# Nightmare-n/GD-MAE

Measured on AMD Instinct MI355X. Metric: MAE pre-train frames/sec (Waymo-shape, 180k pts, 75% mask), higher is better.
Workload: dtype bf16

## Files before the change

gd-mae_amd/csrc/conv_tiles.hip:

```cpp
#include "conv_tiles.h"

typedef float f32x16 __attribute__((ext_vector_type(16)));
typedef __bf16 bf16x8 __attribute__((ext_vector_type(8)));
typedef _Float16 f16x8 __attribute__((ext_vector_type(8)));
union CtFrag {
  uint4 q;
  bf16x8 v;
  f16x8 h;
};

#define CT_C 128
#define CT_SITE_PITCH 272
#ifndef CT_CH
#define CT_CH 128
#endif
#ifndef CT_RING
#define CT_RING 8
#endif
#define CT_HALVES (CT_C / CT_CH)
#define CT_KS (CT_CH / 16)
#define CT_NSTEP (9 * CT_KS)
#define CT_CPS (CT_CH / 8)
#define CT_PSITE (CT_CH * 2 + 16)
#define CT_ROW_PITCH (CT_CH == 128 ? 2944 : 1664)
#define CT_TILE_PITCH (10 * CT_ROW_PITCH)
#ifndef CT_TPW
#define CT_TPW 2
#endif
#define CT_THREADS (CT_TPW * 128)
#define CT_NWAVES (CT_TPW * 2)
#define CT_STAGE_PITCH 17408
#define CT_RED_OFF (CT_TPW * CT_STAGE_PITCH)
#define CT_EPI_BYTES (CT_RED_OFF + CT_TPW * CT_NWAVES * 2 * CT_C * 4)
#define CT_PATCH_BYTES (CT_TPW * CT_TILE_PITCH)
#define CT_LDS_BYTES (CT_PATCH_BYTES > CT_EPI_BYTES ? CT_PATCH_BYTES : CT_EPI_BYTES)
#define CT_SPP (CT_THREADS / CT_CPS)
#define CT_NPASS ((100 * CT_TPW + CT_SPP - 1) / CT_SPP)
#define CT_ESPP (CT_THREADS / 16)
#define CT_MAX_SRC 3
#define CT_NRED 256

__device__ inline float ct_bf2f(unsigned short h) { return __uint_as_float(((unsigned)h) << 16); }
__device__ inline unsigned short ct_f2bf(float f) { return gd_to_bf16(f); }
__device__ inline unsigned ct_pack2(float lo, float hi) { return gd_pack_bf16(lo, hi); }
__device__ inline float ct_f16r(float f) {
  const unsigned p = gd_pack_f16(f, 0.f);
  return (float)__builtin_bit_cast(_Float16, (unsigned short)(p & 0xFFFFu));
}
__device__ inline void ct_unpack8(const uint4& u, float (&f)[8]) {
  const unsigned w[4] = {u.x, u.y, u.z, u.w};
#pragma unroll
  for (int k = 0; k < 4; ++k) {
    f[2 * k] = __uint_as_float(w[k] << 16);
    f[2 * k + 1] = __uint_as_float(w[k] & 0xFFFF0000u);
  }
}

struct CtMaps {
  const int* map[CT_MAX_SRC];
  int ls[CT_MAX_SRC];
  int k;
};

__global__ __launch_bounds__(256) void k_ct_tile_flags(CtMaps Mp, int B, int H, int W, int TH, int TW, int* __restrict__ flag) {
  const int lane = threadIdx.x & 63;
  const int t = blockIdx.x * 4 + (threadIdx.x >> 6);
  if (t >= B * TH * TW) return;
  const int tx = t % TW, r = t / TW, ty = r % TH, b = r / TH;
  bool act = false;
  for (int e = lane; e < 100; e += 64) {
    const int y = ty * 8 - 1 + e / 10, x = tx * 8 - 1 + e % 10;
    if (y < 0 || y >= H || x < 0 || x >= W) continue;
    for (int g = 0; g < Mp.k; ++g) {
      const int ls = Mp.ls[g];
      act |= Mp.map[g][(b * (H >> ls) + (y >> ls)) * (W >> ls) + (x >> ls)] >= 0;
    }
  }
  const unsigned long long m = __ballot(act);
  if (lane == 0) flag[t] = m != 0ull;
}

struct CtFlagLoad {
  const int* flag;
  __device__ int operator()(long long i) const { return flag[i]; }
};
struct CtSlotStore {
  int* slot;
  int* list;
  __device__ void operator()(long long i, int ex, int v) const {
    slot[i] = v ? ex : -1;
    if (v) list[ex] = (int)i;
  }
};

extern "C" size_t gdmae_decoder_tiles_workspace_bytes(int B, int H, int W) {
  const long long nt = (long long)B * ((H + 7) / 8) * ((W + 7) / 8);
  return gd_align(sizeof(int) * nt) + gd_align(sizeof(int) * (gd_scan_ws_elems(nt) + 2)) + 256;
}

extern "C" int gdmae_decoder_tiles(const int* const* maps, const int* strides, int k, int B, int H, int W, int* tile_slot,
                                   int* tile_list, int* n_act, void* workspace, void* stream) {
  GD_REQUIRE(k >= 1 && k <= CT_MAX_SRC, "decoder_tiles: 1..3 source stages");
  GD_REQUIRE(H >= 2 && W >= 2 && B >= 1, "decoder_tiles: map too small");
  hipStream_t st = (hipStream_t)stream;
  CtMaps Mp;
  Mp.k = k;
  for (int g = 0; g < k; ++g) {
    const int s = strides[g];
    GD_REQUIRE(s == 1 || s == 2 || s == 4 || s == 8, "decoder_tiles: stride must be 1, 2, 4 or 8");
    GD_REQUIRE(H % s == 0 && W % s == 0, "decoder_tiles: stride must divide the map");
    Mp.map[g] = maps[g];
    Mp.ls[g] = s == 1 ? 0 : (s == 2 ? 1 : (s == 4 ? 2 : 3));
  }
  const int TH = (H + 7) / 8, TW = (W + 7) / 8;
  const long long nt = (long long)B * TH * TW;
  GdArena A(workspace, gdmae_decoder_tiles_workspace_bytes(B, H, W));
  int* flag = A.take<int>(nt);
  int* scan_ws = A.take<int>(gd_scan_ws_elems(nt) + 2);
  hipLaunchKernelGGL(k_ct_tile_flags, dim3(gd_div_up(nt, 4)), dim3(256), 0, st, Mp, B, H, W, TH, TW, flag);
  GD_LAUNCH_CHECK();
  return gd_device_scan<int>(nt, CtFlagLoad{flag}, CtSlotStore{tile_slot, tile_list}, n_act, scan_ws, st);
}

size_t gd_decoder_tiles_lb_state_bytes(long long nt) { return gd_scan_lb_state_bytes<int>(nt); }
int gd_decoder_tiles_lb(const int* const* maps, const int* strides, int k, int B, int H, int W, int* tile_slot, int* tile_list, int* n_act,
                        int* flag, void* lb_state, hipStream_t st) {
  GD_REQUIRE(k >= 1 && k <= CT_MAX_SRC, "decoder_tiles: 1..3 source stages");
  CtMaps Mp;
  Mp.k = k;
  for (int g = 0; g < k; ++g) {
    const int s = strides[g];
    GD_REQUIRE((s == 1 || s == 2 || s == 4 || s == 8) && H % s == 0 && W % s == 0, "decoder_tiles: stride must be 1, 2, 4 or 8 and divide the map");
    Mp.map[g] = maps[g];
    Mp.ls[g] = s == 1 ? 0 : (s == 2 ? 1 : (s == 4 ? 2 : 3));
  }
  const int TH = (H + 7) / 8, TW = (W + 7) / 8;
  const long long nt = (long long)B * TH * TW;
  hipLaunchKernelGGL(k_ct_tile_flags, dim3(gd_div_up(nt, 4)), dim3(256), 0, st, Mp, B, H, W, TH, TW, flag);
  GD_LAUNCH_CHECK();
  return gd_device_scan_lb<int>(nt, CtFlagLoad{flag}, CtSlotStore{tile_slot, tile_list}, GdNoTotal{}, n_act, lb_state, st);
}

__global__ __launch_bounds__(256) void k_ct_pack_weights(const float* __restrict__ w, int Cin, int nsteps, uint4* __restrict__ Wp) {
  const int i = blockIdx.x * blockDim.x + threadIdx.x;
  if (i >= nsteps * 4 * 64) return;
  const int lane = i & 63, wv = (i >> 6) & 3, st = i >> 8;
  const int ks = st & 7, tap = (st >> 3) % 9, g = (st >> 3) / 9;
  const int o = 32 * wv + (lane & 31);
  const int ci = g * CT_C + ks * 16 + (lane >> 5) * 8;
  float f[8];
#pragma unroll
  for (int j = 0; j < 8; ++j) f[j] = w[((long long)o * Cin + ci + j) * 9 + tap];
  uint4 q;
  q.x = gd_pack_f16(f[0], f[1]);
  q.y = gd_pack_f16(f[2], f[3]);
  q.z = gd_pack_f16(f[4], f[5]);
  q.w = gd_pack_f16(f[6], f[7]);
  Wp[i] = q;
}

struct CtBPtrs {
  const float* b[CT_MAX_SRC];
};

__global__ __launch_bounds__(256) void k_ct_class_consts(const float* __restrict__ w, CtBPtrs Bp, int Cin, int C2,
                                                         unsigned short* __restrict__ bgz, unsigned short* __restrict__ ybg) {
  __shared__ double sh[9][256];
  const int o = blockIdx.x;
  double t[9];
#pragma unroll
  for (int k = 0; k < 9; ++k) t[k] = 0.0;
  for (int c = threadIdx.x; c < Cin; c += 256) {
    const float bv = Bp.b[c / CT_C][c % CT_C];
    if (o == 0) bgz[c] = ct_f2bf(bv > 0.f ? bv : 0.f);
    const double bg = (double)ct_f16r(bv > 0.f ? bv : 0.f);
#pragma unroll
    for (int k = 0; k < 9; ++k) t[k] += (double)ct_f16r(w[((long long)o * Cin + c) * 9 + k]) * bg;
  }
#pragma unroll
  for (int k = 0; k < 9; ++k) sh[k][threadIdx.x] = t[k];
  __syncthreads();
  if (threadIdx.x < 9) {
    double s = 0.0;
    for (int i = 0; i < 256; ++i) s += sh[threadIdx.x][i];
    sh[threadIdx.x][0] = s;
  }
  __syncthreads();
  if (threadIdx.x < 9) {
    const int cy = threadIdx.x / 3, cx = threadIdx.x % 3;
    double s = 0.0;
    for (int ky = 0; ky < 3; ++ky) {
      if ((cy == 0 && ky == 0) || (cy == 2 && ky == 2)) continue;
      for (int kx = 0; kx < 3; ++kx) {
        if ((cx == 0 && kx == 0) || (cx == 2 && kx == 2)) continue;
        s += sh[ky * 3 + kx][0];
      }
    }
    ybg[threadIdx.x * C2 + o] = ct_f2bf((float)s);
  }
}

extern "C" size_t gdmae_conv3x3_tiles_packed_bytes(int k) { return (size_t)k * 72 * 4 * 64 * 16; }

extern "C" int gdmae_conv3x3_tiles_pack(const float* conv_w, int C2, int Cin, const float* const* b, int k, void* Wp, void* bgz,
                                        void* ybg, void* stream) {
  GD_REQUIRE(C2 == CT_C && k >= 1 && k <= CT_MAX_SRC && Cin == CT_C * k, "conv3x3_tiles: 128 output channels, 128 per source");
  hipStream_t st = (hipStream_t)stream;
  const int nsteps = k * 72;
  hipLaunchKernelGGL(k_ct_pack_weights, dim3(nsteps), dim3(256), 0, st, conv_w, Cin, nsteps, (uint4*)Wp);
  GD_LAUNCH_CHECK();
  CtBPtrs Bp;
  for (int g = 0; g < CT_MAX_SRC; ++g) Bp.b[g] = g < k ? b[g] : nullptr;
  hipLaunchKernelGGL(k_ct_class_consts, dim3(C2), dim3(256), 0, st, conv_w, Bp, Cin, C2, (unsigned short*)bgz, (unsigned short*)ybg);
  GD_LAUNCH_CHECK();
  return 0;
}

struct CtSrc {
  const unsigned short* P;
  const int* map;
  const float* a;
  const float* b;
  int ls;
};
struct CtArgs {
  CtSrc src[CT_MAX_SRC];
  int k;
  const uint4* Wp;
  const int* tile_list;
  int n_act, H, W, TH, TW;
  unsigned short* Yc;
  float* part;
};

#define CT_MFMA(a, b, c) __builtin_amdgcn_mfma_f32_32x32x16_f16((a), (b), (c), 0, 0, 0)

#define CT_OFF(st) ((((st) / CT_KS) / 3) * CT_ROW_PITCH + (((st) / CT_KS) % 3) * CT_PSITE + ((st) % CT_KS) * 32)
#define CT_WSTEP(st, hf) ((((st) / CT_KS) * 8 + (hf) * CT_KS + ((st) % CT_KS)) * 256)

__global__ __launch_bounds__(CT_THREADS, CT_TPW == 2 ? (CT_CH == 64 ? 3 : 2) : 1) void k_conv3x3_tiles(CtArgs A) {
  extern __shared__ __align__(16) unsigned char lds[];
  const int tid = threadIdx.x, lane = tid & 63, wvg = tid >> 6;
  const int wv = wvg & 3;
  const int tg = wvg >> 2;
  const int slot0 = blockIdx.x * CT_TPW;
  int tb[CT_TPW], ty0[CT_TPW], tx0[CT_TPW];
  bool have[CT_TPW];
#pragma unroll
  for (int t = 0; t < CT_TPW; ++t) {
    have[t] = slot0 + t < A.n_act;
    const int tile = have[t] ? A.tile_list[slot0 + t] : 0;
    tx0[t] = (tile % A.TW) * 8;
    const int r = tile / A.TW;
    ty0[t] = (r % A.TH) * 8;
    tb[t] = r / A.TH;
  }
  const int lc = tid % CT_CPS;
  const int lsg = tid / CT_CPS;
  const unsigned char* lb = lds + tg * 2 * CT_TILE_PITCH + ((lane & 31) >> 3) * CT_ROW_PITCH + (lane & 7) * CT_PSITE + (lane >> 5) * 16;
  f32x16 acc0, acc1, acc2, acc3;
#pragma unroll
  for (int i = 0; i < 16; ++i) acc0[i] = acc1[i] = acc2[i] = acc3[i] = 0.f;

  for (int g = 0; g < A.k; ++g) {
    const CtSrc S = A.src[g];
    const int ls = S.ls, sm = (1 << ls) - 1;
    const int Hs = A.H >> ls, Ws = A.W >> ls;
    int code[CT_NPASS];
    {
      int tokv[CT_NPASS];
#pragma unroll
      for (int p = 0; p < CT_NPASS; ++p) {
        const int e = p * CT_SPP + lsg;
        const int t = e / 100 < CT_TPW ? e / 100 : CT_TPW - 1;
        const int r = e - 100 * (e / 100);
        const int py = r / 10, px = r - py * 10;
        const int y = ty0[t] + py - 1, x = tx0[t] + px - 1;
        const bool inb = e < 100 * CT_TPW && have[t] && y >= 0 && y < A.H && x >= 0 && x < A.W;
        tokv[p] = S.map[inb ? (tb[t] * Hs + (y >> ls)) * Ws + (x >> ls) : 0];
      }
#pragma unroll
      for (int p = 0; p < CT_NPASS; ++p) {
        const int e = p * CT_SPP + lsg;
        int c = -3;
        if (e < 100 * CT_TPW) {
          const int t = e / 100;
          const int r = e - 100 * t;
          const int py = r / 10, px = r - py * 10;
          if (have[t]) {
            const int y = ty0[t] + py - 1, x = tx0[t] + px - 1;
            c = -2;
            if (y >= 0 && y < A.H && x >= 0 && x < A.W) {
              const int tok = tokv[p];
              c = tok < 0 ? -1 : (((tok << ls) + (y & sm)) << ls) + (x & sm);
            }
          }
        }
        code[p] = c;
      }
    }
    const unsigned short* __restrict__ Prows = S.P ? S.P : (const unsigned short*)S.a;
#pragma unroll 1
    for (int hf = 0; hf < CT_HALVES; ++hf) {
      {
        const int c0 = hf * CT_CH + lc * 8;
        float av[8], bv[8];
        {
          const float4 a0 = *(const float4*)(S.a + c0), a1 = *(const float4*)(S.a + c0 + 4);
          const float4 b0 = *(const float4*)(S.b + c0), b1 = *(const float4*)(S.b + c0 + 4);
          av[0] = a0.x; av[1] = a0.y; av[2] = a0.z; av[3] = a0.w; av[4] = a1.x; av[5] = a1.y; av[6] = a1.z; av[7] = a1.w;
          bv[0] = b0.x; bv[1] = b0.y; bv[2] = b0.z; bv[3] = b0.w; bv[4] = b1.x; bv[5] = b1.y; bv[6] = b1.z; bv[7] = b1.w;
        }
        uint4 bgq;
        {
          float r[8];
#pragma unroll
          for (int j = 0; j < 8; ++j) r[j] = bv[j];
          bgq.x = gd_pack_f16_relu(r[0], r[1]); bgq.y = gd_pack_f16_relu(r[2], r[3]); bgq.z = gd_pack_f16_relu(r[4], r[5]); bgq.w = gd_pack_f16_relu(r[6], r[7]);
        }
        uint4 q[CT_NPASS];
#pragma unroll
        for (int p = 0; p < CT_NPASS; ++p) q[p] = *(const uint4*)(Prows + (long long)(code[p] >= 0 ? code[p] : 0) * CT_C + c0);
#pragma unroll
        for (int p = 0; p < CT_NPASS; ++p) {
          if (code[p] == -3) continue;
          const int e = p * CT_SPP + lsg;
          const int t = e / 100;
          const int r = e - 100 * t;
          const int py = r / 10, px = r - py * 10;
          uint4 o;
          if (code[p] >= 0) {
            float f[8];
            ct_unpack8(q[p], f);
#pragma unroll
            for (int j = 0; j < 8; ++j) f[j] = fmaf(av[j], f[j], bv[j]);
            o.x = gd_pack_f16_relu(f[0], f[1]); o.y = gd_pack_f16_relu(f[2], f[3]); o.z = gd_pack_f16_relu(f[4], f[5]); o.w = gd_pack_f16_relu(f[6], f[7]);
          } else if (code[p] == -1) {
            o = bgq;
          } else {
            o = make_uint4(0u, 0u, 0u, 0u);
          }
          *(uint4*)(lds + t * CT_TILE_PITCH + py * CT_ROW_PITCH + px * CT_PSITE + lc * 16) = o;
        }
      }
      __syncthreads();
      {
        const uint4* __restrict__ wp = A.Wp + ((size_t)g * 72 * 4 + wv) * 64 + lane + (size_t)hf * CT_KS * 256;
        CtFrag wr[CT_RING + 1], sf[2][4];
#pragma unroll
        for (int st = 0; st < CT_RING; ++st) wr[st].q = wp[CT_WSTEP(st, 0)];
        sf[0][0].q = *(const uint4*)(lb);
        sf[0][1].q = *(const uint4*)(lb + 4 * CT_ROW_PITCH);
        sf[0][2].q = *(const uint4*)(lb + CT_TILE_PITCH);
        sf[0][3].q = *(const uint4*)(lb + CT_TILE_PITCH + 4 * CT_ROW_PITCH);
#pragma unroll
        for (int st = 0; st < CT_NSTEP; ++st) {
          if (st + CT_RING < CT_NSTEP) wr[(st + CT_RING) % (CT_RING + 1)].q = wp[CT_WSTEP(st + CT_RING, 0)];
          if (st + 1 < CT_NSTEP) {
            sf[(st + 1) & 1][0].q = *(const uint4*)(lb + CT_OFF(st + 1));
            sf[(st + 1) & 1][1].q = *(const uint4*)(lb + 4 * CT_ROW_PITCH + CT_OFF(st + 1));
            sf[(st + 1) & 1][2].q = *(const uint4*)(lb + CT_TILE_PITCH + CT_OFF(st + 1));
            sf[(st + 1) & 1][3].q = *(const uint4*)(lb + CT_TILE_PITCH + 4 * CT_ROW_PITCH + CT_OFF(st + 1));
          }
          acc0 = CT_MFMA(wr[st % (CT_RING + 1)].h, sf[st & 1][0].h, acc0);
          acc1 = CT_MFMA(wr[st % (CT_RING + 1)].h, sf[st & 1][1].h, acc1);
          acc2 = CT_MFMA(wr[st % (CT_RING + 1)].h, sf[st & 1][2].h, acc2);
          acc3 = CT_MFMA(wr[st % (CT_RING + 1)].h, sf[st & 1][3].h, acc3);
          __builtin_amdgcn_sched_barrier(0);
        }
      }
      __syncthreads();
    }
  }

  {
    const int n = lane & 31;
    const int cb = wv * 32 + 4 * (lane >> 5);
#define CT_STAGE(acc, sb)                                                                                              \
  _Pragma("unroll") for (int j = 0; j < 4; ++j) {                                                                      \
    uint2 o;                                                                                                           \
    o.x = ct_pack2(acc[4 * j], acc[4 * j + 1]);                                                                        \
    o.y = ct_pack2(acc[4 * j + 2], acc[4 * j + 3]);                                                                    \
    *(uint2*)(lds + (tg * 2 + ((sb) >> 1)) * CT_STAGE_PITCH + (((sb) & 1) * 32 + n) * CT_SITE_PITCH + (cb + 8 * j) * 2) = o; \
  }
    CT_STAGE(acc0, 0)
    CT_STAGE(acc1, 1)
    CT_STAGE(acc2, 2)
    CT_STAGE(acc3, 3)
#undef CT_STAGE
  }
  __syncthreads();
  float* red = (float*)(lds + CT_RED_OFF);
  const int elc = tid & 15, elsg = tid >> 4;
#pragma unroll
  for (int t = 0; t < CT_TPW; ++t) {
    if (!have[t]) continue;
    float s[8], q2[8];
#pragma unroll
    for (int j = 0; j < 8; ++j) s[j] = q2[j] = 0.f;
#pragma unroll
    for (int p = 0; p < 64 / CT_ESPP; ++p) {
      const int site = p * CT_ESPP + elsg;
      const uint4 v = *(const uint4*)(lds + t * CT_STAGE_PITCH + site * CT_SITE_PITCH + elc * 16);
      *(uint4*)(A.Yc + ((long long)(slot0 + t) * GD_TILE_SITES + site) * CT_C + elc * 8) = v;
      if (ty0[t] + (site >> 3) < A.H && tx0[t] + (site & 7) < A.W) {
        float f[8];
        ct_unpack8(v, f);
#pragma unroll
        for (int j = 0; j < 8; ++j) {
          s[j] += f[j];
          q2[j] = fmaf(f[j], f[j], q2[j]);
        }
      }
    }
#pragma unroll
    for (int j = 0; j < 8; ++j) {
      s[j] += __shfl_xor(s[j], 16, 64);
      s[j] += __shfl_xor(s[j], 32, 64);
      q2[j] += __shfl_xor(q2[j], 16, 64);
      q2[j] += __shfl_xor(q2[j], 32, 64);
    }
    if (lane < 16) {
#pragma unroll
      for (int j = 0; j < 8; ++j) {
        red[((t * CT_NWAVES + wvg) * 2 + 0) * CT_C + elc * 8 + j] = s[j];
        red[((t * CT_NWAVES + wvg) * 2 + 1) * CT_C + elc * 8 + j] = q2[j];
      }
    }
  }
  __syncthreads();
#pragma unroll
  for (int t = 0; t < CT_TPW; ++t) {
    if (!have[t] || tid >= 256) continue;
    const int stat = tid >> 7, ch = tid & 127;
    float v = 0.f;
#pragma unroll
    for (int w = 0; w < CT_NWAVES; ++w) v += red[((t * CT_NWAVES + w) * 2 + stat) * CT_C + ch];
    A.part[(long long)(slot0 + t) * 256 + tid] = v;
  }
}

__global__ __launch_bounds__(256) void k_ct_stats_reduce(const float* __restrict__ part, int n_act, const int* __restrict__ tile_list,
                                                         const unsigned short* __restrict__ ybg, int B, int H, int W, int TH, int TW,
                                                         float* __restrict__ red) {
  const int tid = threadIdx.x;
  if ((int)blockIdx.x < CT_NRED) {
    const int chunk = (n_act + CT_NRED - 1) / CT_NRED;
    const int r0 = blockIdx.x * chunk, r1 = r0 + chunk < n_act ? r0 + chunk : n_act;
    float a0 = 0.f, a1 = 0.f, a2 = 0.f, a3 = 0.f;
    int r = r0;
    for (; r + 15 < r1; r += 16) {
      float v[16];
#pragma unroll
      for (int u = 0; u < 16; ++u) v[u] = part[(long long)(r + u) * 256 + tid];
#pragma unroll
      for (int u = 0; u < 16; u += 4) {
        a0 += v[u];
        a1 += v[u + 1];
        a2 += v[u + 2];
        a3 += v[u + 3];
      }
    }
    for (; r + 3 < r1; r += 4) {
      a0 += part[(long long)r * 256 + tid];
      a1 += part[(long long)(r + 1) * 256 + tid];
      a2 += part[(long long)(r + 2) * 256 + tid];
      a3 += part[(long long)(r + 3) * 256 + tid];
    }
    for (; r < r1; ++r) a0 += part[(long long)r * 256 + tid];
    red[(long long)blockIdx.x * 256 + tid] = (a0 + a1) + (a2 + a3);
    return;
  }
  __shared__ int cnt[9];
  if (tid < 9) cnt[tid] = 0;
  __syncthreads();
  int c[9];
#pragma unroll
  for (int k = 0; k < 9; ++k) c[k] = 0;
  for (int i0 = tid; i0 < n_act; i0 += 8 * 256) {
   int tl[8];
#pragma unroll
   for (int u = 0; u < 8; ++u) tl[u] = tile_list[i0 + u * 256 < n_act ? i0 + u * 256 : n_act - 1];
#pragma unroll
   for (int u = 0; u < 8; ++u) {
    if (i0 + u * 256 >= n_act) continue;
    const int tile = tl[u];
    const int tx = tile % TW, ty = (tile / TW) % TH;
    const int y0 = ty * 8, y1 = y0 + 8 < H ? y0 + 8 : H, x0 = tx * 8, x1 = x0 + 8 < W ? x0 + 8 : W;
    const int ry[3] = {y0 == 0 ? 1 : 0, 0, y1 == H ? 1 : 0};
    const int rx[3] = {x0 == 0 ? 1 : 0, 0, x1 == W ? 1 : 0};
    const int my = (y1 - y0) - ry[0] - ry[2], mx = (x1 - x0) - rx[0] - rx[2];
#pragma unroll
    for (int cy = 0; cy < 3; ++cy)
#pragma unroll
      for (int cx = 0; cx < 3; ++cx) c[cy * 3 + cx] += (cy == 1 ? my : ry[cy]) * (cx == 1 ? mx : rx[cx]);
   }
  }
#pragma unroll
  for (int k = 0; k < 9; ++k)
    if (c[k]) atomicAdd(&cnt[k], c[k]);
  __syncthreads();
  const int stat = tid >> 7, ch = tid & 127;
  double acc = 0.0;
#pragma unroll
  for (int cy = 0; cy < 3; ++cy)
#pragma unroll
    for (int cx = 0; cx < 3; ++cx) {
      const long long total = (long long)B * (cy == 1 ? H - 2 : 1) * (cx == 1 ? W - 2 : 1);
      const double n = (double)(total - cnt[cy * 3 + cx]);
      const double v = (double)ct_bf2f(ybg[(cy * 3 + cx) * CT_C + ch]);
      acc += n * (stat ? v * v : v);
    }
  const float hi = (float)acc;
  red[(long long)CT_NRED * 256 + tid] = hi;
  red[(long long)(CT_NRED + 1) * 256 + tid] = (float)(acc - (double)hi);
}

int gd_bn_fold_from_partials(hipStream_t st, const float* part, int nblk, int C, double count, const float* gamma,
                             const float* beta, double eps, double momentum, float* running_mean, float* running_var,
                             long long* num_batches, double* stats, float* ab, float* mv);

extern "C" size_t gdmae_conv3x3_tiles_workspace_bytes(int n_act) {
  return gd_align((size_t)(n_act > 0 ? n_act : 1) * 256 * sizeof(float)) + gd_align((size_t)(CT_NRED + 2) * 256 * sizeof(float));
}

extern "C" int gdmae_conv3x3_tiles_fwd(const void* const* P, const int* const* maps, const float* const* a, const float* const* b,
                                       const int* strides, int k, const void* Wp, const void* ybg, const int* tile_list, int n_act,
                                       int B, int H, int W, void* Yc, const float* gamma, const float* beta, double eps,
                                       double momentum, float* running_mean, float* running_var, long long* num_batches,
                                       double* stats, float* ab, float* mv, void* workspace, void* stream) {
  GD_REQUIRE(k >= 1 && k <= CT_MAX_SRC, "conv3x3_tiles: 1..3 source stages");
  GD_REQUIRE(H >= 2 && W >= 2, "conv3x3_tiles: map too small");
  hipStream_t st = (hipStream_t)stream;
  CtArgs A;
  A.k = k;
  for (int g = 0; g < CT_MAX_SRC; ++g) {
    if (g < k) {
      const int s = strides[g];
      GD_REQUIRE((s == 1 || s == 2 || s == 4 || s == 8) && H % s == 0 && W % s == 0, "conv3x3_tiles: stride");
      A.src[g].P = (const unsigned short*)P[g];
      A.src[g].map = maps[g];
      A.src[g].a = a[g];
      A.src[g].b = b[g];
      A.src[g].ls = s == 1 ? 0 : (s == 2 ? 1 : (s == 4 ? 2 : 3));
    } else {
      A.src[g].P = nullptr; A.src[g].map = nullptr; A.src[g].a = nullptr; A.src[g].b = nullptr; A.src[g].ls = 0;
    }
  }
  A.Wp = (const uint4*)Wp;
  A.tile_list = tile_list;
  A.n_act = n_act;
  A.H = H; A.W = W; A.TH = (H + 7) / 8; A.TW = (W + 7) / 8;
  A.Yc = (unsigned short*)Yc;
  GdArena ar(workspace, gdmae_conv3x3_tiles_workspace_bytes(n_act));
  float* part = ar.take<float>((size_t)(n_act > 0 ? n_act : 1) * 256);
  float* red = ar.take<float>((size_t)(CT_NRED + 2) * 256);
  A.part = part;
  if (n_act > 0) {
    static bool once = false;
    if (!once) {
      GD_CHECK(hipFuncSetAttribute((const void*)k_conv3x3_tiles, hipFuncAttributeMaxDynamicSharedMemorySize, CT_LDS_BYTES));
      once = true;
    }
    hipLaunchKernelGGL(k_conv3x3_tiles, dim3((n_act + CT_TPW - 1) / CT_TPW), dim3(CT_THREADS), CT_LDS_BYTES, st, A);
    GD_LAUNCH_CHECK();
  }
  hipLaunchKernelGGL(k_ct_stats_reduce, dim3(CT_NRED + 1), dim3(256), 0, st, (const float*)part, n_act, tile_list,
                     (const unsigned short*)ybg, B, H, W, A.TH, A.TW, red);
  GD_LAUNCH_CHECK();
  return gd_bn_fold_from_partials(st, red, CT_NRED + 2, CT_C, (double)B * H * W, gamma, beta, eps, momentum, running_mean,
                                  running_var, num_batches, stats, ab, mv);
}

template <int ES>
__global__ __launch_bounds__(256) void k_tiles_gather_rows(const void* __restrict__ Yc, GdTiles T, const int* __restrict__ cell,
                                                           long long n, int H, int W, int C, uint4* __restrict__ out) {
  const int cv = C * ES / 16;
  const long long total = n * cv;
  for (long long i = blockIdx.x * (long long)blockDim.x + threadIdx.x; i < total; i += (long long)gridDim.x * blockDim.x) {
    const long long r = total < (1ll << 31) ? (long long)((unsigned)i / (unsigned)cv) : i / cv;
    const int v = (int)(i - r * cv);
    const int s = cell[r];
    const int x = s % W, q = s / W, y = q % H, b = q / H;
    out[i] = ((const uint4*)gd_y_row<ES>(Yc, T, b, y, x, H, W, C))[v];
  }
}

extern "C" int gdmae_tiles_gather_rows(const void* Yc, const int* tile_slot, const void* ybg, const int* cell, long long n, int H,
                                       int W, int C, int elem_bytes, void* out, void* stream) {
  GD_REQUIRE(tile_slot != nullptr && (elem_bytes == 2 || elem_bytes == 4) && (C * elem_bytes) % 16 == 0, "tiles_gather_rows");
  if (n <= 0) return 0;
  GdTiles T{tile_slot, ybg, (H + 7) / 8, (W + 7) / 8};
  long long g = (n * (C * elem_bytes / 16) + 255) / 256;
  if (g > 16384) g = 16384;
  if (elem_bytes == 2) hipLaunchKernelGGL(k_tiles_gather_rows<2>, dim3((int)g), dim3(256), 0, (hipStream_t)stream, Yc, T, cell, n, H, W, C, (uint4*)out);
  else hipLaunchKernelGGL(k_tiles_gather_rows<4>, dim3((int)g), dim3(256), 0, (hipStream_t)stream, Yc, T, cell, n, H, W, C, (uint4*)out);
  GD_LAUNCH_CHECK();
  return 0;
}

__global__ __launch_bounds__(256) void k_tiles_gather_rows_affine_relu(const void* __restrict__ Yc, GdTiles T, const int* __restrict__ cell,
                                                                       long long n, int H, int W, int C, const float* __restrict__ a,
                                                                       const float* __restrict__ b, uint4* __restrict__ yrows,
                                                                       float4* __restrict__ out) {
  const int cv = C / 8;
  const long long total = n * cv;
  for (long long i = blockIdx.x * (long long)blockDim.x + threadIdx.x; i < total; i += (long long)gridDim.x * blockDim.x) {
    const long long r = total < (1ll << 31) ? (long long)((unsigned)i / (unsigned)cv) : i / cv;
    const int v = (int)(i - r * cv);
    const int s = cell[r];
    const int x = s % W, q = s / W, y = q % H, bb = q / H;
    const uint4 yq = ((const uint4*)gd_y_row<2>(Yc, T, bb, y, x, H, W, C))[v];
    const float4 a0 = ((const float4*)a)[2 * v], a1 = ((const float4*)a)[2 * v + 1];
    const float4 b0 = ((const float4*)b)[2 * v], b1 = ((const float4*)b)[2 * v + 1];
    const unsigned w4[4] = {yq.x, yq.y, yq.z, yq.w};
    const float av[8] = {a0.x, a0.y, a0.z, a0.w, a1.x, a1.y, a1.z, a1.w};
    const float bv[8] = {b0.x, b0.y, b0.z, b0.w, b1.x, b1.y, b1.z, b1.w};
    float o[8];
#pragma unroll
    for (int j = 0; j < 4; ++j) {
      const float h0 = fmaf(av[2 * j], __uint_as_float(w4[j] << 16), bv[2 * j]);
      const float h1 = fmaf(av[2 * j + 1], __uint_as_float(w4[j] & 0xFFFF0000u), bv[2 * j + 1]);
      o[2 * j] = h0 > 0.f ? h0 : 0.f;
      o[2 * j + 1] = h1 > 0.f ? h1 : 0.f;
    }
    yrows[i] = yq;
    out[2 * i] = make_float4(o[0], o[1], o[2], o[3]);
    out[2 * i + 1] = make_float4(o[4], o[5], o[6], o[7]);
  }
}

extern "C" int gdmae_tiles_gather_rows_affine_relu(const void* Yc, const int* tile_slot, const void* ybg, const int* cell, long long n,
                                                   int H, int W, int C, const float* a, const float* b, void* yrows, float* out,
                                                   void* stream) {
  GD_REQUIRE(tile_slot != nullptr && C % 8 == 0 && a != nullptr && b != nullptr, "tiles_gather_rows_affine_relu: bf16 rows, C % 8 == 0");
  if (n <= 0) return 0;
  GdTiles T{tile_slot, ybg, (H + 7) / 8, (W + 7) / 8};
  long long g = (n * (C / 8) + 255) / 256;
  if (g > 16384) g = 16384;
  hipLaunchKernelGGL(k_tiles_gather_rows_affine_relu, dim3((int)g), dim3(256), 0, (hipStream_t)stream, Yc, T, cell, n, H, W, C, a, b,
                     (uint4*)yrows, (float4*)out);
  GD_LAUNCH_CHECK();
  return 0;
}

template <int ES>
__global__ __launch_bounds__(256) void k_tiles_to_dense(const void* __restrict__ Yc, GdTiles T, int B, int H, int W, int C,
                                                        uint4* __restrict__ out) {
  const int cv = C * ES / 16;
  const long long total = (long long)B * H * W * cv;
  for (long long i = blockIdx.x * (long long)blockDim.x + threadIdx.x; i < total; i += (long long)gridDim.x * blockDim.x) {
    const long long s = i / cv;
    const int v = (int)(i % cv);
    const int x = (int)(s % W);
    const long long q = s / W;
    const int y = (int)(q % H), b = (int)(q / H);
    out[i] = ((const uint4*)gd_y_row<ES>(Yc, T, b, y, x, H, W, C))[v];
  }
}

__global__ __launch_bounds__(256) void k_tiles_to_dense_affine_relu(const void* __restrict__ Yc, GdTiles T, int B, int H, int W, int C,
                                                                    const float* __restrict__ a, const float* __restrict__ bsh,
                                                                    float* __restrict__ out) {
  const int cv = C / 8;
  const long long total = (long long)B * H * W * cv;
  const unsigned total32 = (unsigned)total, ucv = (unsigned)cv, uW = (unsigned)W, uH = (unsigned)H;
  for (unsigned i = blockIdx.x * blockDim.x + threadIdx.x; i < total32; i += gridDim.x * blockDim.x) {
    const unsigned s32 = i / ucv;
    const int v = (int)(i - s32 * ucv);
    const unsigned q32 = s32 / uW;
    const int x = (int)(s32 - q32 * uW);
    const unsigned b32 = q32 / uH;
    const int y = (int)(q32 - b32 * uH), b = (int)b32;
    const long long s = s32;
    const uint4 u = ((const uint4*)gd_y_row<2>(Yc, T, b, y, x, H, W, C))[v];
    float f[8];
    ct_unpack8(u, f);
    const float4 a0 = *(const float4*)(a + 8 * v), a1 = *(const float4*)(a + 8 * v + 4);
    const float4 b0 = *(const float4*)(bsh + 8 * v), b1 = *(const float4*)(bsh + 8 * v + 4);
    float4 o0, o1;
    o0.x = fmaxf(fmaf(a0.x, f[0], b0.x), 0.f); o0.y = fmaxf(fmaf(a0.y, f[1], b0.y), 0.f);
    o0.z = fmaxf(fmaf(a0.z, f[2], b0.z), 0.f); o0.w = fmaxf(fmaf(a0.w, f[3], b0.w), 0.f);
    o1.x = fmaxf(fmaf(a1.x, f[4], b1.x), 0.f); o1.y = fmaxf(fmaf(a1.y, f[5], b1.y), 0.f);
    o1.z = fmaxf(fmaf(a1.z, f[6], b1.z), 0.f); o1.w = fmaxf(fmaf(a1.w, f[7], b1.w), 0.f);
    typedef float f4v __attribute__((ext_vector_type(4)));
    __builtin_nontemporal_store(f4v{o0.x, o0.y, o0.z, o0.w}, (f4v*)(out + s * C + 8 * v));
    __builtin_nontemporal_store(f4v{o1.x, o1.y, o1.z, o1.w}, (f4v*)(out + s * C + 8 * v + 4));
  }
}

extern "C" int gdmae_tiles_to_dense_affine_relu(const void* Yc, const int* tile_slot, const void* ybg, int B, int H, int W, int C, const float* a,
                                                const float* b, float* out, void* stream) {
  GD_REQUIRE(tile_slot != nullptr && C % 8 == 0 && a != nullptr && b != nullptr, "tiles_to_dense_affine_relu");
  GD_REQUIRE((long long)B * H * W * (C / 8) < (1ll << 31), "tiles_to_dense_affine_relu: B H W C / 8 must fit 31 bits");
  GdTiles T{tile_slot, ybg, (H + 7) / 8, (W + 7) / 8};
  hipLaunchKernelGGL(k_tiles_to_dense_affine_relu, dim3(16384), dim3(256), 0, (hipStream_t)stream, Yc, T, B, H, W, C, a, b, out);
  GD_LAUNCH_CHECK();
  return 0;
}

extern "C" int gdmae_tiles_to_dense(const void* Yc, const int* tile_slot, const void* ybg, int B, int H, int W, int C, int elem_bytes,
                                    void* out, void* stream) {
  GD_REQUIRE(tile_slot != nullptr && (elem_bytes == 2 || elem_bytes == 4) && (C * elem_bytes) % 16 == 0, "tiles_to_dense");
  GdTiles T{tile_slot, ybg, (H + 7) / 8, (W + 7) / 8};
  if (elem_bytes == 2) hipLaunchKernelGGL(k_tiles_to_dense<2>, dim3(16384), dim3(256), 0, (hipStream_t)stream, Yc, T, B, H, W, C, (uint4*)out);
  else hipLaunchKernelGGL(k_tiles_to_dense<4>, dim3(16384), dim3(256), 0, (hipStream_t)stream, Yc, T, B, H, W, C, (uint4*)out);
  GD_LAUNCH_CHECK();
  return 0;
}
```

gd-mae_amd/csrc/plan.hip:

```cpp
#include "../../include/gdmae_hip.h"
#include "common.h"
#include <string.h>

int gd_voxelize_impl(const float* points, long long n_points, int n_cols, const float* lo, const float* vs, const int* grid_xyz,
                     int batch_size, float* points_out, long long* point_coords, long long* inverse, int* inverse32,
                     long long* voxel_coords, int* pillar_cell, int* pillar_pt_off, int* pillar_pts, int* point_rank,
                     int* sample_pillar_off, float* pillar_mean, int* cell2pillar_out, int* counts, void* workspace, size_t workspace_bytes,
                     void* lb_state, float* points_pm, int* row_pillar, hipStream_t st);
size_t gd_voxelize_lb_state_bytes(long long n_points, long long cells);
size_t gd_plan_scan_state_bytes(long long n);
size_t gd_plan_win_state_bytes(long long n);
int gd_plan_visible_tokens(const float* mask, const int* cell2pillar, long long n_cells, int* tok_pillar, int* tok_cell, int* map,
                           int* n_tok, void* lb_state, hipStream_t st);
int gd_plan_downsample(const int* map_in, int B, int Yi, int Xi, int* tok_cell_out, int* map_out, int* n_out, void* lb_state,
                       hipStream_t st);
struct Dims {
  int B, Y, X;
};
struct PlanJob {
  const int* n_tok;
  const int* tok_cell;
  Dims dt, dm;
  const int* map;
  int mode, s;
  int* nbr;
  int* nbr_rev;
};
constexpr int kPlanMaxJobs = 16;
struct PlanJobs {
  PlanJob j[kPlanMaxJobs];
  int count;
};
int gd_plan_jobs(const PlanJobs& J, long long cap_max, hipStream_t st);
size_t gd_plan_windows_ws_bytes(int B, int Y, int X, int wx, int wy);
long long gd_plan_n_windows(int B, int Y, int X, int wx, int wy);
struct GdWinStage {
  const int* map;
  int B, Y, X, wx, wy, nlev;
  const int *drop_lo, *drop_hi, *max_tokens;
  int* out[2][7];
  int* counts[2];
  void* workspace;
  void* lb_state;
};
int gd_plan_windows_all(const GdWinStage* stages, int n_stages, hipStream_t st);
size_t gd_decoder_tiles_lb_state_bytes(long long nt);
int gd_decoder_tiles_lb(const int* const* maps, const int* strides, int k, int B, int H, int W, int* tile_slot, int* tile_list, int* n_act,
                        int* flag, void* lb_state, hipStream_t st);
int gd_decoder_site_rulebook(const int* site, const int* n_dev, int sites_per_tok, long long cap_sites, const int* tile_slot, int H, int W,
                             int* nbr, hipStream_t st);

namespace {

struct StageGeo {
  int Y, X;
  long long cap;
  long long cap_in;
  int up_s;
  long long n_win;
};

struct Layout {
  gdmae_plan_buffer* table;
  int max_entries, n;
  size_t off;
  bool ok;
  long long add(const char* name, size_t bytes) {
    const size_t o = off;
    if (table) {
      if (n >= max_entries) {
        ok = false;
        return -1;
      }
      strncpy(table[n].name, name, sizeof(table[n].name) - 1);
      table[n].name[sizeof(table[n].name) - 1] = 0;
      table[n].offset = (long long)o;
      table[n].bytes = (long long)bytes;
    }
    ++n;
    off += gd_align(bytes);
    return (long long)o;
  }
};

struct Offsets {
  long long lb_state, counts, points, point_coords, inverse, inverse32, voxel_coords, pillar_cell, pt_off, pillar_pts, point_rank,
      sample_off, pillar_mean, cell2pillar, points_pm, row_pillar, vox_ws, mask, len_keep, tok_pillar;
  long long vis_tok_cell, vis_map;
  long long vfe_row_tok, vfe_vis_rows, vfe_vis_tok, vfe_tok_row_off;
  struct {
    long long tok_cell, map, nbr_subm, nbr_subm_t, nbr_down, nbr_down_t, up_sites, win_ws;
    long long w[2][7];
  } s[GDMAE_PLAN_MAX_STAGES];
  long long dec_slot, dec_list, dec_flag, dec_nbr[3];
  size_t lb_bytes, vox_ws_bytes;
  int n_counts;
  bool dec;
  StageGeo geo[GDMAE_PLAN_MAX_STAGES];
  long long cap_pts, m_cap, cells;
};

constexpr int kTokScanThreads = 1024, kTokScanItems = 4;
__global__ __launch_bounds__(kTokScanThreads) void k_vfe_tok_row_off(const int* __restrict__ n_tok_p, const int* __restrict__ tok_pillar,
                                                                     const int* __restrict__ pt_off, int* __restrict__ tok_row_off,
                                                                     int* __restrict__ n_rows) {
  __shared__ int s_wave[kTokScanThreads / 64];
  const int n = *n_tok_p, lane = threadIdx.x & 63, wave = threadIdx.x >> 6;
  int base = 0;
  for (int t0 = 0; t0 < n; t0 += kTokScanThreads * kTokScanItems) {
    const int t = t0 + (int)threadIdx.x * kTokScanItems;
    int c[kTokScanItems], sum = 0;
#pragma unroll
    for (int k = 0; k < kTokScanItems; ++k) {
      c[k] = 0;
      if (t + k < n) {
        const int p = tok_pillar[t + k];
        c[k] = pt_off[p + 1] - pt_off[p];
      }
      sum += c[k];
    }
    int incl = sum;
#pragma unroll
    for (int d = 1; d < 64; d <<= 1) {
      const int o = __shfl_up(incl, d, 64);
      if (lane >= d) incl += o;
    }
    if (lane == 63) s_wave[wave] = incl;
    __syncthreads();
    int before = 0, all = 0;
#pragma unroll
    for (int w = 0; w < kTokScanThreads / 64; ++w) {
      before += w < wave ? s_wave[w] : 0;
      all += s_wave[w];
    }
    int run = base + before + incl - sum;
#pragma unroll
    for (int k = 0; k < kTokScanItems; ++k) {
      if (t + k < n) tok_row_off[t + k] = run;
      run += c[k];
    }
    base += all;
    __syncthreads();
  }
  if (threadIdx.x == 0) {
    tok_row_off[n] = base;
    *n_rows = base;
  }
}
__global__ __launch_bounds__(256) void k_vfe_vis_rows(const int* __restrict__ counts, const int* __restrict__ row_pillar,
                                                      const int* __restrict__ pillar_cell, const int* __restrict__ map,
                                                      const int* __restrict__ pt_off, const int* __restrict__ tok_row_off,
                                                      int* __restrict__ row_tok, int* __restrict__ vis_rows, int* __restrict__ vis_tok) {
  const int N = counts[0];
  for (int r = blockIdx.x * 256 + threadIdx.x; r < N; r += gridDim.x * 256) {
    const int p = row_pillar[r];
    const int t = map[pillar_cell[p]];
    row_tok[r] = t;
    if (t >= 0) {
      const int rc = tok_row_off[t] + (r - pt_off[p]);
      vis_rows[rc] = r;
      vis_tok[rc] = t;
    }
  }
}

int check(const gdmae_plan_params* p) {
  GD_REQUIRE(p != nullptr, "geometry plan: null parameters");
  GD_REQUIRE(p->n_points >= 0 && p->n_points < (1ll << 31) && p->n_cols >= 4 && p->n_cols <= 65 && p->batch_size >= 1,
             "geometry plan: bad point buffer");
  GD_REQUIRE(p->grid[0] >= 1 && p->grid[1] >= 1 && p->grid[2] == 1, "geometry plan: single-layer pillar grids (spt_backbone_mae.py:94)");
  GD_REQUIRE(p->n_stages >= 1 && p->n_stages <= GDMAE_PLAN_MAX_STAGES, "geometry plan: 1..4 stages");
  for (int i = 0; i < p->n_stages; ++i) {
    GD_REQUIRE(p->stride[i] == 1 || p->stride[i] == 2, "geometry plan: conv_down stride 1 or 2 (k3 s2 p1)");
    GD_REQUIRE(i == 0 || p->stride[i] == 2, "geometry plan: only the first stage may keep the resolution");
    GD_REQUIRE(p->win_x[i] >= 1 && p->win_y[i] >= 1 && p->win_x[i] * p->win_y[i] <= 64, "geometry plan: window must fit one wavefront");
    GD_REQUIRE(p->n_levels[i] >= 1 && p->n_levels[i] <= 3, "geometry plan: 1..3 drop levels");
  }
  GD_REQUIRE(p->n_dec >= 0 && p->n_dec <= 3, "geometry plan: at most 3 decoder source stages");
  for (int g = 0; g < p->n_dec; ++g) GD_REQUIRE(p->dec_sources[g] >= 0 && p->dec_sources[g] < p->n_stages, "geometry plan: decoder source");
  return 0;
}

int layout(const gdmae_plan_params* p, gdmae_plan_buffer* table, int max_entries, Offsets& O, size_t* total, int* n_entries) {
  if (int rc = check(p)) return rc;
  Layout L{table, max_entries, 0, 0, true};
  const int B = p->batch_size, gx = p->grid[0], gy = p->grid[1], F = p->n_cols - 1;
  const long long n0 = p->cap_points > p->n_points ? p->cap_points : p->n_points;
  O.cells = (long long)B * gx * gy;
  GD_REQUIRE(O.cells < (1ll << 31), "geometry plan: B*Y*X must fit int32");
  O.cap_pts = n0 > 0 ? n0 : 1;
  O.m_cap = n0 < O.cells ? n0 : O.cells;
  if (O.m_cap < 1) O.m_cap = 1;
  const long long cap = O.cap_pts;
  int Y = gy, X = gx;
  long long c = O.m_cap;
  for (int i = 0; i < p->n_stages; ++i) {
    StageGeo& g = O.geo[i];
    g.cap_in = c;
    if (p->stride[i] == 2) {
      Y = (Y - 1) / 2 + 1;
      X = (X - 1) / 2 + 1;
      c = 4 * c < (long long)B * Y * X ? 4 * c : (long long)B * Y * X;
    }
    g.Y = Y; g.X = X; g.cap = c;
    const int us = gy / Y;
    g.up_s = (us >= 1 && us * Y == gy && us * X == gx) ? us : 0;
    g.n_win = gd_plan_n_windows(B, Y, X, p->win_x[i], p->win_y[i]);
    GD_REQUIRE(g.n_win < (1 << 21), "geometry plan: window grid too large for the packed scan");
    GD_REQUIRE(g.cap < (1 << 21), "geometry plan: stage token capacity must stay below 2^21 (21-bit fields of the packed window scan)");
  }
  O.dec = p->n_dec > 0;
  for (int g = 0; g < p->n_dec; ++g) {
    const int us = O.geo[p->dec_sources[g]].up_s;
    O.dec = O.dec && (us == 1 || us == 2 || us == 4 || us == 8);
  }
  const long long nt = (long long)B * ((gy + 7) / 8) * ((gx + 7) / 8);
  size_t lb = gd_voxelize_lb_state_bytes(n0, O.cells) + gd_plan_scan_state_bytes(O.cells);
  for (int i = 0; i < p->n_stages; ++i) {
    if (p->stride[i] == 2) lb += gd_plan_scan_state_bytes((long long)B * O.geo[i].Y * O.geo[i].X);
    lb += 2 * gd_plan_win_state_bytes(O.geo[i].n_win);
  }
  if (O.dec) lb += gd_decoder_tiles_lb_state_bytes(nt);
  O.lb_bytes = lb;
  O.lb_state = L.add("lb_state", lb);
  O.n_counts = 2 + p->n_stages + 16 * p->n_stages + 1 + 1 + 1;
  O.counts = L.add("counts", sizeof(int) * O.n_counts);
  O.points = L.add("points", sizeof(float) * cap * p->n_cols);
  O.point_coords = L.add("point_coords", sizeof(long long) * cap * 4);
  O.inverse = L.add("inverse", sizeof(long long) * cap);
  O.inverse32 = L.add("inverse32", sizeof(int) * cap);
  O.voxel_coords = L.add("voxel_coords", sizeof(long long) * cap * 4);
  O.pillar_cell = L.add("pillar_cell", sizeof(int) * cap);
  O.pt_off = L.add("pt_off", sizeof(int) * (cap + 1));
  O.pillar_pts = L.add("pillar_pts", sizeof(int) * cap);
  O.point_rank = L.add("point_rank", sizeof(int) * cap);
  O.sample_off = L.add("sample_off", sizeof(int) * (B + 1));
  O.pillar_mean = L.add("pillar_mean", sizeof(float) * cap * F);
  O.cell2pillar = L.add("cell2pillar", sizeof(int) * O.cells);
  O.points_pm = L.add("points_pm", sizeof(float) * cap * p->n_cols);
  O.row_pillar = L.add("row_pillar", sizeof(int) * cap);
  O.vox_ws_bytes = gdmae_voxelize_workspace_bytes(n0, B, gx, gy, 1);
  O.vox_ws = L.add("vox_ws", O.vox_ws_bytes);
  O.mask = L.add("mask", sizeof(float) * O.m_cap);
  O.len_keep = L.add("len_keep", sizeof(int) * B);
  O.tok_pillar = L.add("tok_pillar", sizeof(int) * O.m_cap);
  O.vis_tok_cell = O.vis_map = -1;
  if (p->stride[0] == 2) {
    O.vis_tok_cell = L.add("vis.tok_cell", sizeof(int) * O.m_cap);
    O.vis_map = L.add("vis.map", sizeof(int) * O.cells);
  }
  O.vfe_row_tok = O.vfe_vis_rows = O.vfe_vis_tok = O.vfe_tok_row_off = -1;
  if (p->masked && p->want_pm) {
    O.vfe_row_tok = L.add("vfe.row_tok", sizeof(int) * cap);
    O.vfe_vis_rows = L.add("vfe.vis_rows", sizeof(int) * cap);
    O.vfe_vis_tok = L.add("vfe.vis_tok", sizeof(int) * cap);
    O.vfe_tok_row_off = L.add("vfe.tok_row_off", sizeof(int) * (O.m_cap + 1));
  }
  char nm[40];
  static const char* const kWin[7] = {"tok_win", "tok_level", "tok_slot", "tok_pos", "csr_tok", "win_start", "win_len"};
  for (int i = 0; i < p->n_stages; ++i) {
    const StageGeo& g = O.geo[i];
    auto name = [&](const char* s) { snprintf(nm, sizeof(nm), "s%d.%s", i, s); return (const char*)nm; };
    O.s[i].tok_cell = L.add(name("tok_cell"), sizeof(int) * g.cap);
    O.s[i].map = L.add(name("map"), sizeof(int) * (long long)B * g.Y * g.X);
    O.s[i].nbr_subm = L.add(name("nbr_subm"), sizeof(int) * g.cap * 9);
    O.s[i].nbr_subm_t = L.add(name("nbr_subm_t"), sizeof(int) * g.cap * 9);
    O.s[i].nbr_down = O.s[i].nbr_down_t = O.s[i].up_sites = -1;
    if (p->stride[i] == 2) {
      O.s[i].nbr_down = L.add(name("nbr_down"), sizeof(int) * g.cap * 9);
      O.s[i].nbr_down_t = L.add(name("nbr_down_t"), sizeof(int) * g.cap_in * 9);
    }
    if (g.up_s > 1) O.s[i].up_sites = L.add(name("up_sites"), sizeof(int) * g.cap * g.up_s * g.up_s);
    O.s[i].win_ws = L.add(name("win_ws"), gd_plan_windows_ws_bytes(B, g.Y, g.X, p->win_x[i], p->win_y[i]));
    const long long wcap = g.n_win < g.cap ? g.n_win : g.cap;
    for (int sh = 0; sh < 2; ++sh)
      for (int k = 0; k < 7; ++k) {
        snprintf(nm, sizeof(nm), "s%d.w%d.%s", i, sh, kWin[k]);
        O.s[i].w[sh][k] = L.add(nm, sizeof(int) * (k < 5 ? g.cap : wcap));
      }
  }
  O.dec_slot = O.dec_list = O.dec_flag = -1;
  if (O.dec) {
    O.dec_slot = L.add("dec.tile_slot", sizeof(int) * nt);
    O.dec_list = L.add("dec.tile_list", sizeof(int) * nt);
    O.dec_flag = L.add("dec.flag", sizeof(int) * nt);
    for (int g = 0; g < p->n_dec; ++g) {
      const StageGeo& sg = O.geo[p->dec_sources[g]];
      snprintf(nm, sizeof(nm), "dec.nbr%d", g);
      O.dec_nbr[g] = L.add(nm, sizeof(int) * sg.cap * sg.up_s * sg.up_s * 9);
    }
  }
  GD_REQUIRE(L.ok, "geometry plan: buffer table too small");
  if (total) *total = L.off;
  if (n_entries) *n_entries = L.n;
  return 0;
}

}

extern "C" int gdmae_geometry_plan_layout(const gdmae_plan_params* p, gdmae_plan_buffer* table, int max_entries, int* n_entries,
                                          size_t* total_bytes) {
  Offsets O;
  return layout(p, table, max_entries, O, total_bytes, n_entries);
}

extern "C" int gdmae_geometry_plan(const gdmae_plan_params* p, const float* points, const float* noise, void* arena, size_t arena_bytes,
                                   void* stream) {
  Offsets O;
  size_t total = 0;
  if (int rc = layout(p, nullptr, 0, O, &total, nullptr)) return rc;
  GD_REQUIRE(arena != nullptr && arena_bytes >= total, "geometry plan: arena too small (gdmae_geometry_plan_layout)");
  GD_REQUIRE(!p->masked || noise != nullptr, "geometry plan: masking needs one noise value per pillar (capacity min(points, cells))");
  hipStream_t st = (hipStream_t)stream;
  char* A = (char*)arena;
  auto I = [&](long long off) { return off < 0 ? (int*)nullptr : (int*)(A + off); };
  const int B = p->batch_size, gx = p->grid[0], gy = p->grid[1], ns = p->n_stages;
  int* counts = I(O.counts);
  int* n_tok = counts + 2;
  int* win_counts = counts + 2 + ns;
  int* n_act = counts + 2 + ns + 16 * ns;
  int* n_vis = n_act + 1;
  GD_CHECK(hipMemsetAsync(A + O.lb_state, 0, (size_t)(O.counts - O.lb_state) + gd_align(sizeof(int) * O.n_counts), st));
  char* lb = A + O.lb_state;
  {
    int rc = gd_voxelize_impl(points, p->n_points, p->n_cols, p->lo, p->vs, p->grid, B, (float*)(A + O.points), (long long*)(A + O.point_coords),
                              (long long*)(A + O.inverse), I(O.inverse32), (long long*)(A + O.voxel_coords), I(O.pillar_cell), I(O.pt_off),
                              I(O.pillar_pts), I(O.point_rank), I(O.sample_off), (float*)(A + O.pillar_mean), I(O.cell2pillar), counts,
                              A + O.vox_ws, O.vox_ws_bytes, lb, p->want_pm ? (float*)(A + O.points_pm) : nullptr,
                              p->want_pm ? I(O.row_pillar) : nullptr, st);
    if (rc) return rc;
    lb += gd_voxelize_lb_state_bytes(p->n_points, O.cells);
  }
  float* mask = (float*)(A + O.mask);
  if (p->masked) {
    int rc = gdmae_random_mask(noise, I(O.sample_off), B, p->keep_frac, mask, I(O.len_keep), stream);
    if (rc) return rc;
  } else {
    GD_CHECK(hipMemsetAsync(mask, 0, sizeof(float) * O.m_cap, st));
  }
  const bool first_strided = p->stride[0] == 2;
  int* cur_cell = first_strided ? I(O.vis_tok_cell) : I(O.s[0].tok_cell);
  int* cur_map = first_strided ? I(O.vis_map) : I(O.s[0].map);
  int* cur_n = first_strided ? n_vis : n_tok;
  {
    int rc = gd_plan_visible_tokens(mask, I(O.cell2pillar), O.cells, I(O.tok_pillar), cur_cell, cur_map, cur_n, lb, st);
    if (rc) return rc;
    lb += gd_plan_scan_state_bytes(O.cells);
  }
  if (O.vfe_row_tok >= 0) {
    hipLaunchKernelGGL(k_vfe_tok_row_off, dim3(1), dim3(kTokScanThreads), 0, st, (const int*)cur_n, (const int*)I(O.tok_pillar),
                       (const int*)I(O.pt_off), I(O.vfe_tok_row_off), n_vis + 1);
    GD_LAUNCH_CHECK();
    const long long blocks = (O.cap_pts + 255) / 256;
    hipLaunchKernelGGL(k_vfe_vis_rows, dim3((unsigned)(blocks < 2048 ? blocks : 2048)), dim3(256), 0, st, (const int*)counts,
                       (const int*)I(O.row_pillar), (const int*)I(O.pillar_cell), (const int*)cur_map, (const int*)I(O.pt_off),
                       (const int*)I(O.vfe_tok_row_off), I(O.vfe_row_tok), I(O.vfe_vis_rows), I(O.vfe_vis_tok));
    GD_LAUNCH_CHECK();
  }
  int Yp = gy, Xp = gx;
  PlanJobs J;
  J.count = 0;
  long long cap_max = 1;
  GdWinStage W[4];
  GD_REQUIRE(ns <= 4, "geometry plan: at most four stages");
  for (int i = 0; i < ns; ++i) {
    const StageGeo& g = O.geo[i];
    GD_REQUIRE(J.count + 4 <= kPlanMaxJobs, "geometry plan: job table full");
    if (g.cap > cap_max) cap_max = g.cap;
    if (p->stride[i] == 2) {
      int rc = gd_plan_downsample(cur_map, B, Yp, Xp, I(O.s[i].tok_cell), I(O.s[i].map), n_tok + i, lb, st);
      if (rc) return rc;
      lb += gd_plan_scan_state_bytes((long long)B * g.Y * g.X);
      J.j[J.count++] = PlanJob{n_tok + i, I(O.s[i].tok_cell), Dims{B, g.Y, g.X}, Dims{B, Yp, Xp}, cur_map, 1, 0, I(O.s[i].nbr_down), nullptr};
      J.j[J.count++] = PlanJob{cur_n, cur_cell, Dims{B, Yp, Xp}, Dims{B, g.Y, g.X}, I(O.s[i].map), 2, 0, I(O.s[i].nbr_down_t), nullptr};
      if (g.cap_in > cap_max) cap_max = g.cap_in;
      cur_cell = I(O.s[i].tok_cell);
      cur_map = I(O.s[i].map);
      cur_n = n_tok + i;
      Yp = g.Y;
      Xp = g.X;
    }
    J.j[J.count++] = PlanJob{cur_n, cur_cell, Dims{B, g.Y, g.X}, Dims{B, g.Y, g.X}, cur_map, 0, 0, I(O.s[i].nbr_subm), I(O.s[i].nbr_subm_t)};
    if (g.up_s > 1) {
      J.j[J.count++] = PlanJob{cur_n, cur_cell, Dims{B, g.Y, g.X}, Dims{B, g.Y, g.X}, nullptr, 3, g.up_s, I(O.s[i].up_sites), nullptr};
      if (g.cap * g.up_s * g.up_s / 9 + 1 > cap_max) cap_max = g.cap * g.up_s * g.up_s / 9 + 1;
    }
    GdWinStage& w = W[i];
    w.map = cur_map;
    w.B = B; w.Y = g.Y; w.X = g.X; w.wx = p->win_x[i]; w.wy = p->win_y[i]; w.nlev = p->n_levels[i];
    w.drop_lo = p->drop_lo[i]; w.drop_hi = p->drop_hi[i]; w.max_tokens = p->max_tokens[i];
    w.counts[0] = win_counts + 16 * i;
    w.counts[1] = win_counts + 16 * i + 8;
    for (int sh = 0; sh < 2; ++sh)
      for (int k = 0; k < 7; ++k) w.out[sh][k] = I(O.s[i].w[sh][k]);
    w.workspace = A + O.s[i].win_ws;
    w.lb_state = lb;
    lb += 2 * gd_plan_win_state_bytes(g.n_win);
  }
  {
    int rc = gd_plan_jobs(J, cap_max, st);
    if (rc) return rc;
    rc = gd_plan_windows_all(W, ns, st);
    if (rc) return rc;
  }
  if (O.dec) {
    const int* maps[3];
    int ups[3];
    for (int g = 0; g < p->n_dec; ++g) {
      maps[g] = I(O.s[p->dec_sources[g]].map);
      ups[g] = O.geo[p->dec_sources[g]].up_s;
    }
    int rc = gd_decoder_tiles_lb(maps, ups, p->n_dec, B, gy, gx, I(O.dec_slot), I(O.dec_list), n_act, I(O.dec_flag), lb, st);
    if (rc) return rc;
    for (int g = 0; g < p->n_dec; ++g) {
      const int si = p->dec_sources[g];
      const StageGeo& sg = O.geo[si];
      const int* sites = sg.up_s > 1 ? I(O.s[si].up_sites) : I(O.s[si].tok_cell);
      rc = gd_decoder_site_rulebook(sites, n_tok + si, sg.up_s * sg.up_s, sg.cap * sg.up_s * sg.up_s, I(O.dec_slot), gy, gx, I(O.dec_nbr[g]), st);
      if (rc) return rc;
    }
  }
  return 0;
}
```

gd-mae_amd/gdmae_hip/decoder.py:

```python
from __future__ import annotations

import os
from collections import namedtuple
from dataclasses import dataclass
from types import SimpleNamespace
from typing import Optional

import torch
import torch.nn.functional as F

from . import bn as gbn
from . import lib as L
from . import ops, packing
from . import plan as gplan
from . import timing

CONV_BWD = os.environ.get("GDMAE_DEC_BWD", "implicit")
BLOCK_BWD = os.environ.get("GDMAE_DEC_BLOCK", "1")
DY_ROWS = os.environ.get("GDMAE_DEC_DY_ROWS", "1") != "0"
GATHER_FUSED = os.environ.get("GDMAE_DEC_GATHER_FUSED", "1") != "0"



def colstats(x2d: torch.Tensor):
    R, C = x2d.shape
    assert x2d.is_contiguous() and x2d.dtype in (torch.float32, torch.bfloat16)
    out = torch.empty(2 * C, dtype=torch.float64, device=x2d.device)
    ws = torch.empty(L.load().gdmae_colstats_workspace_bytes(C), dtype=torch.uint8, device=x2d.device)
    L.call("gdmae_colstats", L.ptr(x2d), R, C, int(x2d.dtype == torch.bfloat16), L.ptr(out), L.ptr(ws), L.stream())
    return out[:C], out[C:]


def _gather_slice(table2d, idx, col0, ncol):
    es = table2d.element_size()
    out = torch.empty(idx.numel(), ncol, dtype=table2d.dtype, device=table2d.device)
    L.call("gdmae_gather_rows_strided", L.ptr(table2d), L.ptr(idx), idx.numel(), ncol * es, table2d.shape[1] * es,
           col0 * es, L.ptr(out), L.stream())
    return out


def _scatter_slice(src2d, idx, table2d, col0):
    es = table2d.element_size()
    src2d = src2d.contiguous()
    assert src2d.dtype == table2d.dtype
    L.call("gdmae_scatter_rows_strided", L.ptr(src2d), L.ptr(idx), idx.numel(), src2d.shape[1] * es,
           table2d.shape[1] * es, col0 * es, L.ptr(table2d), L.stream())


def _bf(t):
    return int(t.dtype == torch.bfloat16)


_TAP_REGION = torch.zeros(9, 9, dtype=torch.float64)
for _ky in (-1, 0, 1):
    for _kx in (-1, 0, 1):
        _k = (_ky + 1) * 3 + (_kx + 1)
        _TAP_REGION[_k, 0] = 1
        if _ky:
            _TAP_REGION[_k, 1 if _ky < 0 else 2] = -1
        if _kx:
            _TAP_REGION[_k, 3 if _kx < 0 else 4] = -1
        if _ky and _kx:
            _TAP_REGION[_k, 5 + (0 if _ky < 0 else 2) + (0 if _kx < 0 else 1)] = 1


_REGION_CONSTS = {}


def _region_consts(dev, B, H, W):
    key = (dev, B, H, W)
    if key not in _REGION_CONSTS:
        R = B * H * W
        cnt = torch.tensor([R, B * W, B * W, B * H, B * H, B, B, B, B], dtype=torch.float64)
        _REGION_CONSTS[key] = (_TAP_REGION.to(dev), cnt.to(dev))
    return _REGION_CONSTS[key]


@dataclass(frozen=True, eq=False)
class TileConv:
    tiles: gplan.DecoderTiles
    maps: list
    ups: list


@dataclass(frozen=True, eq=False)
class DecoderGeom:
    B: int
    H: int
    W: int
    eps1: float
    eps2: float
    cdt: torch.dtype
    tile_conv: Optional[TileConv] = None


_Forward = namedtuple("_Forward", "y2 yrows stats2 ab2 mv2 Z tile_slot ybg bgz out", defaults=(None,))


def _forward_tiles(geom, pre_conv_hook, conv_w, gamma2, beta2, pillar_cell, Ps, widths, ab_l, bn2):
    B, H, W, cdt, tc = geom.B, geom.H, geom.W, geom.cdt, geom.tile_conv
    dt, k, dev = tc.tiles, len(Ps), Ps[0].device
    lib = L.load()
    Cin = sum(widths)
    C2 = 128
    Wp = torch.empty(lib.gdmae_conv3x3_tiles_packed_bytes(k), dtype=torch.uint8, device=dev)
    bgz = torch.empty(Cin, dtype=cdt, device=dev)
    ybg = torch.empty(9, C2, dtype=cdt, device=dev)
    a_l, b_l = [ab[:w] for ab, w in zip(ab_l, widths)], [ab[w:] for ab, w in zip(ab_l, widths)]
    L.call("gdmae_conv3x3_tiles_pack", L.ptr(conv_w), C2, Cin, L.host_ptrs(b_l), k, L.ptr(Wp), L.ptr(bgz), L.ptr(ybg),
           L.stream())
    y2 = torch.empty(max(dt.n_act, 1) * 64, C2, dtype=cdt, device=dev)
    stats2 = torch.empty(2 * C2, dtype=torch.float64, device=dev)
    ab2 = torch.empty(2 * C2, dtype=torch.float32, device=dev)
    mv2 = torch.empty(2 * C2, dtype=torch.float32, device=dev)
    ws = torch.empty(lib.gdmae_conv3x3_tiles_workspace_bytes(dt.n_act), dtype=torch.uint8, device=dev)
    rm, rv, nb, mom = gbn.running_stats(bn2)
    flops = 2.0 * dt.n_act * 64 * C2 * 9 * Cin
    if pre_conv_hook is not None:
        pre_conv_hook()
    with timing.kernel("k_conv3x3_tiles", dt.n_act * 64 * (Cin + C2) * 2, flops,
                       {"dense_equivalent_TFLOPs_per_launch": round(2.0 * B * H * W * C2 * 9 * Cin / 1e12, 4), "active_tiles": dt.n_act}):
        L.call("gdmae_conv3x3_tiles_fwd", L.host_ptrs([P.contiguous() for P in Ps]), L.host_ptrs(tc.maps), L.host_ptrs(a_l),
               L.host_ptrs(b_l), L.host_i32(tc.ups), k, L.ptr(Wp), L.ptr(ybg), L.ptr(dt.tile_list), dt.n_act, B, H, W,
               L.ptr(y2), L.ptr(gamma2), L.ptr(beta2), float(geom.eps2), mom, L.ptr(rm), L.ptr(rv), L.ptr(nb), L.ptr(stats2),
               L.ptr(ab2), L.ptr(mv2), L.ptr(ws), L.stream())
    M = pillar_cell.numel()
    yrows = torch.empty(M, C2, dtype=cdt, device=dev)
    out = None
    if GATHER_FUSED:
        out = torch.empty(M, C2, dtype=torch.float32, device=dev)
        L.call("gdmae_tiles_gather_rows_affine_relu", L.ptr(y2), L.ptr(dt.tile_slot), L.ptr(ybg), L.ptr(pillar_cell), M, H, W, C2,
               L.ptr(ab2), L.ptr(ab2[C2:]), L.ptr(yrows), L.ptr(out), L.stream())
    else:
        L.call("gdmae_tiles_gather_rows", L.ptr(y2), L.ptr(dt.tile_slot), L.ptr(ybg), L.ptr(pillar_cell), M, H, W, C2, 2,
               L.ptr(yrows), L.stream())
    return _Forward(y2, yrows, stats2, ab2, mv2, None, dt.tile_slot, ybg, bgz, out)


def _forward_dense_map(geom, conv_w, gamma2, beta2, pillar_cell, sites, Ps, widths, ab_l, bn2):
    B, H, W, cdt = geom.B, geom.H, geom.W, geom.cdt
    R = B * H * W
    bgz = torch.relu(torch.cat([ab[w:] for ab, w in zip(ab_l, widths)])).to(cdt)
    Z = torch.empty(R, sum(widths), dtype=cdt, device=Ps[0].device)
    L.call("gdmae_fill_rows", L.ptr(bgz), R, Z.shape[1], Z.element_size(), L.ptr(Z), L.stream())
    col = 0
    for P, st, ab, w in zip(Ps, sites, ab_l, widths):
        L.call("gdmae_rows_affine_relu_scatter", L.ptr(P), _bf(P), L.ptr(st), P.shape[0], w, L.ptr(ab), L.ptr(ab[w:]), L.ptr(Z), _bf(Z),
               Z.shape[1], col, L.stream())
        col += w
    from . import dense as gdense
    C2o = conv_w.shape[0]
    if cdt == torch.bfloat16 and Z.shape[1] % 64 == 0 and conv_w.dtype == torch.float32:
        y2 = gdense.Conv3x3Dense.apply(Z.view(B, H, W, -1).permute(0, 3, 1, 2), conv_w.detach(), None, 1, None).permute(0, 2, 3, 1)
    elif cdt == torch.float32 and Z.shape[1] % 64 == 0:
        y2 = gdense.conv3x3_f32_rows(Z.view(B, H, W, -1), conv_w.detach().float().contiguous(), None, 1)[..., :C2o]
    else:
        wc = ops.shadow(conv_w, cdt)
        with torch.autocast("cuda", enabled=False):
            y2 = F.conv2d(Z.view(B, H, W, -1).permute(0, 3, 1, 2), wc, None, 1, 1).permute(0, 2, 3, 1)
    if not y2.is_contiguous():
        y2 = y2.contiguous()
    y2 = y2.view(R, -1)
    stats2, ab2, mv2 = gbn.fold(y2, R, gamma2, beta2, geom.eps2, bn2)
    yrows = ops.gather_rows_raw(y2, pillar_cell)
    return _Forward(y2, yrows, stats2, ab2, mv2, Z, None, None, bgz)


def _backward_schedule(geom, conv_w, sites, Ps, widths, fwd):
    C2 = fwd.y2.shape[1]
    native = conv_w.dtype == torch.float32 and conv_w.is_contiguous() and C2 % 8 == 0
    tc = geom.tile_conv
    if not (CONV_BWD == "implicit" and fwd.tile_slot is not None and fwd.y2.dtype == torch.bfloat16 and native and C2 == 128
            and all(w == 128 for w in widths) and tc is not None):
        return native, ["taps"] * len(widths)
    stage_bwd = []
    for P, st, u in zip(Ps, sites, tc.ups):
        n, u = P.shape[0], int(u)
        block = (BLOCK_BWD != "0" and u in (2, 4) and P.dtype == torch.bfloat16 and P.is_contiguous() and st.numel() >= n
                 and int(L.load().gdmae_decoder_block_dw_workspace_bytes(n, u)) > 0)
        stage_bwd.append("block" if block else "rulebook")
    return native, stage_bwd


def _save(ctx, **named):
    ctx.saved_names = [(name, len(v) if isinstance(v, (list, tuple)) else None) for name, v in named.items()]
    ctx.save_for_backward(*[t for v in named.values() for t in (v if isinstance(v, (list, tuple)) else (v,))])


def _saved(ctx) -> SimpleNamespace:
    sv, out, j = ctx.saved_tensors, SimpleNamespace(), 0
    for name, n in ctx.saved_names:
        setattr(out, name, sv[j] if n is None else sv[j:j + n])
        j += 1 if n is None else n
    return out


def _bn2_backward(s, dout, R, direct):
    yrows, ab2 = s.yrows, s.ab2
    M, C2 = yrows.shape
    dev = yrows.device
    dout = dout.float().contiguous()
    st2 = torch.empty(3 * C2, dtype=torch.float64, device=dev)
    ws = torch.empty(L.load().gdmae_rows_bwd_stats_workspace_bytes(C2), dtype=torch.uint8, device=dev)
    L.call("gdmae_rows_bwd_stats", L.ptr(yrows), _bf(yrows), None, M, C2, L.ptr(ab2), L.ptr(ab2[C2:]), L.ptr(dout), 0, C2, 0,
           L.ptr(st2), L.ptr(ws), L.stream())
    dgamma2, dbeta2, k01 = gbn.bwd_coeffs(st2, 3, s.stats2, ab2, s.gamma2, R, None, direct)
    return dout, st2, k01, dgamma2, dbeta2


def _pillar_rows(s, dout):
    yrows, ab2 = s.yrows, s.ab2
    M, C2 = yrows.shape
    zero = torch.zeros(2 * C2, dtype=torch.float32, device=yrows.device)
    rows = torch.empty(M, C2, dtype=torch.float32, device=yrows.device)
    L.call("gdmae_rows_bwd", L.ptr(yrows), _bf(yrows), None, M, C2, L.ptr(ab2), L.ptr(ab2[C2:]), L.ptr(zero), L.ptr(zero[C2:]),
           L.ptr(dout), 0, C2, 0, L.ptr(rows), 0, L.stream())
    return rows


def _region_sums(s, rows, dout, B, H, W):
    y2 = s.y2
    C2 = y2.shape[1]
    reg = torch.empty(16, C2, dtype=torch.float64, device=y2.device)
    ws = torch.empty(L.load().gdmae_border_sums_workspace_bytes(B, C2), dtype=torch.uint8, device=y2.device)
    if rows is None:
        L.call("gdmae_border_sums_rows", L.ptr(y2), _bf(y2), L.ptr(s.tile_slot), L.ptr(s.ybg), L.ptr(dout), L.ptr(s.yrows), L.ptr(s.ab2),
               L.ptr(s.ab2[C2:]), L.ptr(s.pillar_cell), dout.shape[0], B, H, W, C2, L.ptr(reg), L.ptr(ws), L.stream())
    else:
        L.call("gdmae_border_sums", L.ptr(y2), _bf(y2), L.ptr(s.tile_slot), L.ptr(s.ybg), L.ptr(rows), L.ptr(s.pillar_cell),
               rows.shape[0], B, H, W, C2, L.ptr(reg), L.ptr(ws), L.stream())
    return reg



def region_algebra_native(stats2, ab2, st2, k01, reg, tap_region, cnt, R, conv_w, bgz, cdt):
    C2, Cin, dev = conv_w.shape[0], bgz.numel(), conv_w.device
    S = torch.empty(9, C2, dtype=torch.float64, device=dev)
    tot = torch.empty(Cin, dtype=torch.float64, device=dev)
    dWk = torch.empty(9, C2, Cin, dtype=torch.float32, device=dev)
    Wd = torch.empty(9, C2, Cin, dtype=cdt, device=dev)
    ws = torch.empty(L.load().gdmae_decoder_region_workspace_bytes(C2, Cin), dtype=torch.uint8, device=dev)
    L.call("gdmae_decoder_region_algebra", L.ptr(stats2), L.ptr(ab2), L.ptr(st2), L.ptr(k01), L.ptr(reg),
           L.ptr(tap_region), L.ptr(cnt), float(R), C2, Cin, L.ptr(conv_w), L.ptr(bgz), _bf(Wd), L.ptr(S), L.ptr(tot),
           L.ptr(dWk), L.ptr(Wd), L.ptr(ws), L.stream())
    return S, tot, dWk, Wd


def region_algebra_torch(stats2, ab2, st2, k01, reg, tap_region, cnt, R, conv_w, bgz, cdt):
    C2, Cin = conv_w.shape[0], bgz.numel()
    k0, k1 = k01[:C2].double(), k01[C2:].double()
    regY = torch.cat([(stats2[:C2] * R)[None], reg[:8]])
    regR = torch.cat([(ab2[:C2].double() * st2[:C2])[None], reg[8:]])
    regD = cnt[:, None] * k0[None, :] + regY * k1[None, :] + regR
    S = tap_region @ regD
    Wk = conv_w.permute(2, 3, 0, 1).reshape(9, C2, Cin)
    tot = torch.einsum('ko,koi->i', S, Wk.double()).contiguous()
    dWk = (S[:, :, None] * bgz.double()[None, None, :]).to(torch.promote_types(torch.float32, conv_w.dtype))
    Wd = Wk.to(cdt)
    return S, tot, dWk, Wd


def _stage_dx_spconv(b, i, col):
    n, w, C2 = b.Ps[i].shape[0], b.widths[i], b.y2.shape[1]
    nbr = b.tiles.nbr[i]
    assert nbr.shape[0] == n, (nbr.shape, n)
    dX = torch.empty(n, w, dtype=b.cdt, device=b.y2.device)
    L.call("gdmae_spconv", L.ptr(b.dYc), 0, L.ptr(nbr), b.packed.data_ptr() + i * 9 * w * C2 * 2, n, C2, w, L.ptr(dX), 8, L.stream())
    return dX


def _stage_grads_block(b, i, col):
    dX = _stage_dx_spconv(b, i, col)
    P, ab, w, u = b.Ps[i], b.ab_l[i], b.widths[i], int(b.ups[i])
    n = P.shape[0]
    ws = torch.empty(int(L.load().gdmae_decoder_block_dw_workspace_bytes(n, u)), dtype=torch.uint8, device=P.device)
    L.call("gdmae_decoder_block_dw", L.ptr(P), L.ptr(ab), L.ptr(ab[w:]), L.ptr(b.bgz[col:col + w]), L.ptr(b.sites[i]), n, u, L.ptr(b.dYc),
           L.ptr(b.tile_slot), b.H, b.W, L.ptr(b.dWk), b.bgz.numel(), col, L.ptr(ws), L.stream())
    return dX, None
# ... 130 lines not shown
            col += w
        dWk = b.dWk
        if dW_rows:
            dWk = dWk + torch.cat(dW_rows, dim=1).view(dWk.shape)
        dW = dWk.permute(1, 2, 0).reshape(b.conv_w.shape[0], b.conv_w.shape[1], 3, 3)
        if ctx.direct_w is not None:
            ctx.direct_w.add_(dW)
        else:
            grads[2] = dW.to(b.conv_w.dtype)
        grads[3], grads[4] = dgamma2, dbeta2
        return tuple(grads)


class DeconvRowsFn(torch.autograd.Function):

    @staticmethod
    def forward(ctx, x, weight, direct):
        cin, cout, s, _ = weight.shape
        n = x.shape[0]
        dev = x.device
        x = x.contiguous()
        nb = L.load().gdmae_deconv_rows_packed_bytes(cin, cout, s)
        pf = torch.empty(nb, dtype=torch.uint8, device=dev)
        pb = torch.empty(nb, dtype=torch.uint8, device=dev)
        L.call("gdmae_deconv_rows_pack", L.ptr(weight), cin, cout, s, L.ptr(pf), L.ptr(pb), L.stream())
        P = torch.empty(n * s * s, cout, dtype=torch.bfloat16, device=dev)
        L.call("gdmae_deconv_rows_fwd", L.ptr(x), n, cin, cout, s, L.ptr(pf), L.ptr(P), L.stream())
        ctx.save_for_backward(x, pb)
        ctx.meta = (cin, cout, s, direct)
        return P

    @staticmethod
    def backward(ctx, dP):
        x, pb = ctx.saved_tensors
        cin, cout, s, direct = ctx.meta
        n = x.shape[0]
        dP = dP.contiguous()
        if dP.dtype != torch.bfloat16:
            dP = dP.to(torch.bfloat16)
        dx = None
        if ctx.needs_input_grad[0]:
            dx = torch.empty(n, cin, dtype=torch.bfloat16, device=x.device)
            L.call("gdmae_deconv_rows_bwd_input", L.ptr(dP), n, cin, cout, s, L.ptr(pb), L.ptr(dx), L.stream())
        ws = torch.empty(L.load().gdmae_deconv_rows_dw_workspace_bytes(n, cin, cout, s), dtype=torch.uint8, device=x.device)
        L.call("gdmae_deconv_rows_bwd_weight", L.ptr(x), L.ptr(dP), n, cin, cout, s, L.ptr(direct), L.ptr(ws), L.stream())
        return dx, None, None


DECONV_ROWS = os.environ.get("GDMAE_DECONV_ROWS", "1") != "0"


def deconv_rows(x, deconv):
    w = deconv.weight
    s = int(deconv.stride[0])
    cin, cout = w.shape[0], w.shape[1]
    direct = ops.direct_grad(w)
    if (DECONV_ROWS and x.is_cuda and torch.is_autocast_enabled() and x.dtype == torch.bfloat16 and direct is not None and w.dtype == torch.float32
            and w.is_contiguous() and cin in (128, 256) and cout == 128 and s in (1, 2, 4) and x.shape[0] > 0):
        return DeconvRowsFn.apply(x, w, direct)
    wmat = w.permute(0, 2, 3, 1).reshape(cin, s * s * cout)
    return ops.linear(x, wmat.t()).view(-1, cout)


class PredHeadFn(torch.autograd.Function):

    @staticmethod
    def forward(ctx, x, weight, bias, direct):
        n, n_out = x.shape[0], weight.shape[0]
        x = x.contiguous()
        packed = torch.empty(L.load().gdmae_pred_head_packed_bytes(), dtype=torch.uint8, device=x.device)
        L.call("gdmae_pred_head_pack", L.ptr(weight), None if bias is None else L.ptr(bias), weight.shape[1], n_out, L.ptr(packed), L.stream())
        xb = torch.empty(n, x.shape[1], dtype=torch.bfloat16, device=x.device)
        y = torch.empty(n, n_out, dtype=torch.float32, device=x.device)
        L.call("gdmae_pred_head_fwd", L.ptr(x), n, n_out, L.ptr(packed), None, L.ptr(xb), L.ptr(y), L.stream())
        ctx.save_for_backward(xb, packed)
        ctx.meta = (n_out, direct, weight.shape, None if bias is None else bias.shape)
        return y

    @staticmethod
    def backward(ctx, dy):
        x, packed = ctx.saved_tensors
        n_out, direct, wshape, bshape = ctx.meta
        n = x.shape[0]
        dy = dy.contiguous()
        if dy.dtype not in (torch.bfloat16, torch.float32):
            dy = dy.float()
        f32 = dy.dtype == torch.float32
        dyb = torch.empty(dy.shape, dtype=torch.bfloat16, device=x.device) if f32 else None
        dx = torch.empty(x.shape, dtype=torch.float32, device=x.device) if ctx.needs_input_grad[0] else None
        if direct is not None:
            dW, db = direct
            ret = (None, None)
        else:
            dW = torch.zeros(wshape, dtype=torch.float32, device=x.device)
            db = None if bshape is None else torch.zeros(bshape, dtype=torch.float32, device=x.device)
            ret = (dW, db)
        ws = torch.empty(L.load().gdmae_pred_head_bwd_workspace_bytes(n), dtype=torch.uint8, device=x.device)
        scale = ops.LAZY_SCALE.pop(dy.data_ptr(), None) if f32 else None
        if scale is None and ops.LAZY_SCALE:
            raise RuntimeError("an unscaled Chamfer gradient was handed over (ops.LAZY_SCALE) but did not arrive here as the same tensor")
        L.call("gdmae_pred_head_bwd", L.ptr(dy), int(f32), None if dyb is None else L.ptr(dyb), None if scale is None else L.ptr(scale[0]),
               None if scale is None else L.ptr(scale[1]), L.ptr(x), n, n_out, L.ptr(packed),
               None if dx is None else L.ptr(dx), L.ptr(dW), None if db is None else L.ptr(db), L.ptr(ws), L.stream())
        return (dx, *ret, None)


def pred_head(x, linear):
    w, b = linear.weight, linear.bias
    if (DECONV_ROWS and x.is_cuda and torch.is_autocast_enabled() and x.dtype == torch.float32 and w.dtype == torch.float32 and w.is_contiguous()
            and w.shape[1] == 128 and 8 <= w.shape[0] <= 64 and w.shape[0] % 8 == 0 and x.shape[0] > 0):
        dw, db = ops.direct_grad(w), (ops.direct_grad(b) if b is not None else None)
        direct = (dw, db) if (dw is not None and (b is None or db is not None)) else None
        y = PredHeadFn.apply(x, w, b, direct)
        y._gd_pred_head = True
        return y
    return ops.linear(x, w, b)


def upsampled_sites(stage_plan, s: int, Y: int, X: int) -> torch.Tensor:
    if s == 1:
        return stage_plan.tok_cell
    pre = getattr(stage_plan, "_up_sites", None)
    if pre is not None and pre[0] == s and stage_plan.Y * s == Y and stage_plan.X * s == X:
        return pre[1]
    return gplan.upsample_cells(stage_plan.tok_cell, stage_plan.Y, stage_plan.X, s).reshape(-1).contiguous()


def expand_dense(y2, ybg, tiles, a2, b2, B, Y, X):
    R = B * Y * X
    C2 = y2.shape[1]
    compact = ybg is not None
    assert y2.shape[0] == (max(tiles.n_act, 1) * 64 if compact else R), (y2.shape, R, compact)
    if compact and y2.dtype == torch.bfloat16 and C2 % 8 == 0:
        dmap = torch.empty(R, C2, dtype=torch.float32, device=y2.device)
        L.call("gdmae_tiles_to_dense_affine_relu", L.ptr(y2), L.ptr(tiles.tile_slot), L.ptr(ybg), B, Y, X, C2,
               L.ptr(a2), L.ptr(b2), L.ptr(dmap), L.stream())
        return dmap.view(B, Y, X, -1).permute(0, 3, 1, 2)
    if compact:
        yd = torch.empty(R, C2, dtype=y2.dtype, device=y2.device)
        L.call("gdmae_tiles_to_dense", L.ptr(y2), L.ptr(tiles.tile_slot), L.ptr(ybg), B, Y, X, C2, y2.element_size(),
               L.ptr(yd), L.stream())
        y2 = yd
    return torch.relu(y2.float() * a2 + b2).view(B, Y, X, -1).permute(0, 3, 1, 2)


def sparse_decoder(model_cfg, deblocks, conv_out, hidden, pillar_cell, cell2pillar, B, Y, X, want_dense=False, conv_impl='tiles', pre_conv_hook=None):
    args, bns = [], []
    cdt = torch.bfloat16 if torch.is_autocast_enabled() else torch.float32
    src_idx = [int(src[-1]) - 1 for src in model_cfg.FEATURES_SOURCE]
    tile_conv = None
    if cdt == torch.bfloat16 and conv_impl == 'tiles':
        ep = hidden[0]._plan
        tile_conv = TileConv(gplan.decoder_tiles(ep, src_idx, Y, X), [hidden[i].stage_plan.map for i in src_idx],
                             [Y // hidden[i].stage_plan.Y for i in src_idx])
    for i, src in enumerate(model_cfg.FEATURES_SOURCE):
        h = hidden[int(src[-1]) - 1]
        sp = h.stage_plan
        deconv, bn = deblocks[i][0], deblocks[i][1]
        s = int(deconv.stride[0])
        assert deconv.kernel_size == (s, s) and sp.Y * s == Y and sp.X * s == X and deconv.bias is None
        P = deconv_rows(h.features, deconv)
        args += [upsampled_sites(sp, s, Y, X), P, bn.weight, bn.bias]
        bns.append(bn)
    conv, bn2 = conv_out[0], conv_out[1]
    outs = DecoderHead.apply(DecoderGeom(B, Y, X, bns[0].eps, bn2.eps, cdt, tile_conv), pre_conv_hook, conv.weight, bn2.weight, bn2.bias,
                             pillar_cell, cell2pillar, tuple(bns) + (bn2,), *args)
    out, y2, mean2, var2 = outs[:4]
    dense = None
    if want_dense:
        with torch.no_grad():
            a2 = (bn2.weight * torch.rsqrt(var2 + bn2.eps)).float().contiguous()
            b2 = (bn2.bias - a2 * mean2).float().contiguous()
            dense = expand_dense(y2, outs[-1], None if tile_conv is None else tile_conv.tiles, a2, b2, B, Y, X)
    return out, dense
```

gd-mae_amd/gdmae_hip/lib.py:

```python
from __future__ import annotations

import ctypes as C
import os

import torch

_HERE = os.path.dirname(os.path.abspath(__file__))
LIB_PATH = os.path.abspath(os.path.join(_HERE, "..", "csrc", "libgdmae_hip.so"))
if os.environ.get("GDMAE_LIB"):
    LIB_PATH = os.path.abspath(os.environ["GDMAE_LIB"])


class GdmaeHipError(RuntimeError):
    pass


_P, _I, _L, _F, _D, _Z = C.c_void_p, C.c_int, C.c_longlong, C.c_float, C.c_double, C.c_size_t

SIGNATURES = {
    "gdmae_abi_version": (_I, []),
    "gdmae_target_arch": (C.c_char_p, []),
    "gdmae_last_error": (C.c_char_p, []),
    "gdmae_voxelize_workspace_bytes": (_Z, [_L, _I, _I, _I, _I]),
    "gdmae_voxelize": (_I, [_P, _L, _I, _P, _P, _P, _I, _P, _P, _P, _P, _P, _P, _P, _P, _P, _P, _P, _P, _P, _P, _Z, _P]),
    "gdmae_decorate_points": (_I, [_P, _P, _P, _P, _L, _I, _P, _P, _P, _P]),
    "gdmae_vfe_infer": (_I, [_P, _P, _P, _P, _L, _L, _I, _P, _P, _P, _P, _I, _P, _P, _I, _P, _P]),
    "gdmae_vfe_point_layer_workspace_bytes": (_Z, [_I]),
    "gdmae_pillar_major_rows": (_I, [_P, _I, _P, _P, _P, _L, _P, _P, _P]),
    "gdmae_vfe_point_layer_fwd": (_I, [_P, _P, _P, _P, _I, _L, _I, _P, _P, _P, _I, _P, _P, _D, _D, _P, _P, _P, _P, _P, _P, _P, _I, _P, _P]),
    "gdmae_vfe_point_layer_bwd": (_I, [_P, _P, _P, _P, _I, _L, _I, _P, _P, _P, _I, _P, _P, _P, _P, _I, _P, _P, _P, _I, _P, _P]),
    "gdmae_vfe_max_layer_workspace_bytes": (_Z, []),
    "gdmae_vfe_max_layer_fwd": (_I, [_P, _L, _P, _P, _P, _I, _P, _P, _D, _D, _P, _P, _P, _P, _P, _P, _P, _P, _P, _P]),
    "gdmae_vfe_max_layer_bwd": (_I, [_P, _L, _P, _P, _I, _P, _P, _P, _P, _P, _P, _P, _P, _P, _P, _P, _I, _P, _P]),
    "gdmae_vfe_max_layer_fwd_f16": (_I, [_P, _L, _P, _P, _P, _I, _P, _P, _D, _D, _P, _P, _P, _P, _P, _P, _P, _P, _P, _P]),
    "gdmae_vfe_max_layer_bwd_f16": (_I, [_P, _L, _P, _P, _I, _P, _P, _P, _P, _P, _P, _P, _P, _P, _P, _P, _I, _P, _P]),
    "gdmae_vfe_max_layer_vis_fwd": (_I, [_P, _L, _P, _P, _P, _L, _I, _P, _P, _D, _D, _P, _P, _P, _P, _P, _P, _P, _P, _P, _P]),
    "gdmae_vfe_max_layer_vis_fwd_f16": (_I, [_P, _L, _P, _P, _P, _L, _I, _P, _P, _D, _D, _P, _P, _P, _P, _P, _P, _P, _P, _P, _P]),
    "gdmae_vfe_max_layer_vis_bwd": (_I, [_P, _L, _P, _P, _P, _I, _I, _P, _P, _P, _P, _P, _P, _P, _P, _P, _P, _P, _I, _P, _P]),
    "gdmae_vfe_max_layer_vis_bwd_f16": (_I, [_P, _L, _P, _P, _P, _I, _I, _P, _P, _P, _P, _P, _P, _P, _P, _P, _P, _P, _I, _P, _P]),
    "gdmae_fill_rows": (_I, [_P, _L, _I, _I, _P, _P]),
    "gdmae_weighted_mean_finish": (_I, [_P, _P, _L, _P, _P]),
    "gdmae_decoder_region_workspace_bytes": (_Z, [_I, _I]),
    "gdmae_decoder_region_algebra": (_I, [_P, _P, _P, _P, _P, _P, _P, _D, _I, _I, _P, _P, _I, _P, _P, _P, _P, _P, _P]),
    "gdmae_segment_max": (_I, [_P, _P, _P, _I, _I, _P, _P, _P]),
    "gdmae_segment_max_bwd": (_I, [_P, _P, _P, _L, _I, _P, _P]),
    "gdmae_random_mask": (_I, [_P, _P, _I, _D, _P, _P, _P]),
    "gdmae_visible_tokens": (_I, [_P, _P, _P, _L, _L, _P, _P, _P, _P, _P, _P]),
    "gdmae_downsample_tokens": (_I, [_P, _P, _L, _I, _I, _I, _P, _P, _P, _P, _P, _P]),
    "gdmae_rulebook": (_I, [_P, _P, _L, _I, _I, _I, _I, _I, _P, _I, _P, _P]),
    "gdmae_window_workspace_bytes": (_Z, [_I, _I, _I, _I, _I]),
    "gdmae_window_partition": (_I, [_P, _I, _I, _I, _I, _I, _I, _I, _P, _P, _P, _P, _P, _P, _P, _P, _P, _P, _P, _P, _Z, _P]),
    "gdmae_gather_rows": (_I, [_P, _P, _L, _I, _P, _P]),
    "gdmae_scatter_rows": (_I, [_P, _P, _L, _I, _P, _P]),
    "gdmae_gather_rows_strided": (_I, [_P, _P, _L, _I, _I, _I, _P, _P]),
    "gdmae_scatter_rows_strided": (_I, [_P, _P, _L, _I, _I, _I, _P, _P]),
    "gdmae_colstats_workspace_bytes": (_Z, [_I]),
    "gdmae_colstats": (_I, [_P, _L, _I, _I, _P, _P, _P]),
    "gdmae_rows_affine_relu_scatter": (_I, [_P, _I, _P, _L, _I, _P, _P, _P, _I, _I, _I, _P]),
    "gdmae_rows_affine_relu_sub": (_I, [_P, _I, _P, _L, _I, _P, _P, _P, _P, _I, _I, _I, _P]),
    "gdmae_rows_affine_relu_add": (_I, [_P, _I, _L, _I, _P, _P, _P, _P, _I, _P]),
    "gdmae_rows_bwd_stats_workspace_bytes": (_Z, [_I]),
    "gdmae_rows_bwd_stats": (_I, [_P, _I, _P, _L, _I, _P, _P, _P, _I, _I, _I, _P, _P, _P]),
    "gdmae_bn_fold": (_I, [_P, _L, _I, _I, _D, _P, _P, _D, _D, _P, _P, _P, _P, _P, _P, _P, _P]),
    "gdmae_bn_bwd_coeffs": (_I, [_P, _I, _P, _P, _P, _I, _D, _P, _P, _P, _I, _P, _P]),
    "gdmae_rows_bwd_stats_rows": (_I, [_L]),
    "gdmae_bn_bwd_coeffs_rows": (_I, [_P, _I, _I, _P, _P, _P, _I, _D, _P, _P, _P, _I, _P, _P]),
    "gdmae_border_sums_workspace_bytes": (_Z, [_I, _I]),
    "gdmae_border_sums": (_I, [_P, _I, _P, _P, _P, _P, _I, _I, _I, _I, _I, _P, _P, _P]),
    "gdmae_border_sums_rows": (_I, [_P, _I, _P, _P, _P, _P, _P, _P, _P, _I, _I, _I, _I, _I, _P, _P, _P]),
    "gdmae_conv3x3_grad_taps": (_I, [_P, _I, _P, _P, _P, _P, _P, _P, _P, _L, _I, _I, _I, _P, _P]),
    "gdmae_decoder_tiles_workspace_bytes": (_Z, [_I, _I, _I]),
    "gdmae_decoder_tiles": (_I, [_P, _P, _I, _I, _I, _I, _P, _P, _P, _P, _P]),
    "gdmae_conv3x3_tiles_packed_bytes": (_Z, [_I]),
    "gdmae_conv3x3_tiles_pack": (_I, [_P, _I, _I, _P, _I, _P, _P, _P, _P]),
    "gdmae_conv3x3_tiles_workspace_bytes": (_Z, [_I]),
    "gdmae_conv3x3_tiles_fwd": (_I, [_P, _P, _P, _P, _P, _I, _P, _P, _P, _I, _I, _I, _I, _P, _P, _P, _D, _D, _P, _P, _P, _P, _P, _P,
                                     _P, _P]),
    "gdmae_tiles_gather_rows": (_I, [_P, _P, _P, _P, _L, _I, _I, _I, _I, _P, _P]),
    "gdmae_tiles_gather_rows_affine_relu": (_I, [_P, _P, _P, _P, _L, _I, _I, _I, _P, _P, _P, _P, _P]),
    "gdmae_tiles_to_dense": (_I, [_P, _P, _P, _I, _I, _I, _I, _I, _P, _P]),
    "gdmae_tiles_to_dense_affine_relu": (_I, [_P, _P, _P, _I, _I, _I, _I, _P, _P, _P, _P]),
    "gdmae_rows_bwd": (_I, [_P, _I, _P, _L, _I, _P, _P, _P, _P, _P, _I, _I, _I, _P, _I, _P]),
    "gdmae_segment_max_affine": (_I, [_P, _I, _P, _P, _I, _I, _P, _P, _P, _P, _P]),
    "gdmae_segmax_bwd_stats": (_I, [_P, _I, _P, _P, _P, _L, _I, _P, _P, _P, _P, _P]),
    "gdmae_segmax_bn_bwd": (_I, [_P, _I, _P, _P, _P, _P, _L, _I, _P, _P, _P, _P, _I, _P]),
    "gdmae_window_attention_fwd": (_I, [_P, _P, _P, _I, _P, _P, _P, _I, _I, _I, _I, _P, _F, _P]),
    "gdmae_window_attention_bwd": (_I, [_P, _P, _P, _P, _P, _I, _P, _P, _P, _P, _I, _I, _I, _I, _P, _F, _P]),
    "gdmae_window_attention_levels_writes_lse": (_I, [_I, _I, _P, _I, _I]),
    "gdmae_window_attention_levels_fwd": (_I, [_P, _P, _P, _I, _P, _P, _P, _I, _P, _P, _I, _I, _P, _F, _P, _P]),
    "gdmae_window_attention_levels_bwd": (_I, [_P, _P, _P, _P, _P, _I, _P, _P, _P, _P, _I, _P, _P, _I, _I, _P, _F, _P, _P, _P]),
    "gdmae_conv3x3_dense_packed_bytes": (_Z, [_I, _I]),
    "gdmae_conv3x3_dense_pack": (_I, [_P, _I, _I, _I, _I, _P, _P]),
    "gdmae_conv3x3_dense": (_I, [_P, _I, _I, _I, _I, _I, _I, _P, _P, _P, _P]),
    "gdmae_conv3x3_dense_add": (_I, [_P, _I, _I, _I, _I, _I, _I, _P, _P, _P, _P, _P]),
    "gdmae_conv3x3_dense_relu": (_I, [_P, _I, _I, _I, _I, _I, _I, _P, _P, _P, _P, _P]),
    "gdmae_conv3x3_dense_stats_workspace_bytes": (_Z, [_I, _I, _I, _I]),
    "gdmae_conv3x3_dense_stat_rows": (_I, []),
    "gdmae_conv3x3_dense_stats": (_I, [_P, _I, _I, _I, _I, _I, _I, _P, _P, _P, _P, _P, _P]),
    "gdmae_bn_fold_partials": (_I, [_P, _I, _I, _D, _P, _P, _D, _D, _P, _P, _P, _P, _P, _P, _P]),
    "gdmae_conv3x3_dense_f32out": (_I, [_P, _I, _I, _I, _I, _I, _I, _P, _P, _P, _I, _P]),
    "gdmae_conv3x3_dense_dw_workspace_bytes": (_Z, [_I, _I, _I, _I, _I]),
    "gdmae_conv3x3_dense_bwd_weight": (_I, [_P, _P, _I, _I, _I, _I, _I, _I, _I, _I, _P, _P, _P]),
    "gdmae_attention_timing": (_I, [_I]),
    "gdmae_attention_timing_read": (_I, [_I, _P, _P]),
    "gdmae_kernel_timing": (_I, [_I]),
    "gdmae_kernel_timing_slots": (_I, []),
    "gdmae_kernel_timing_name": (C.c_char_p, [_I]),
    "gdmae_kernel_timing_read": (_I, [_I, _P, _P, _P, _P]),
    "gdmae_kernel_timing_read_side": (_I, [_I, _P]),
    "gdmae_add_layernorm_workspace_bytes": (_Z, [_I]),
    "gdmae_add_layernorm_fwd": (_I, [_P, _P, _I, _P, _P, _L, _I, _F, _P, _P, _P, _P]),
    "gdmae_add_layernorm_bwd": (_I, [_P, _P, _I, _P, _P, _P, _P, _I, _L, _I, _P, _P, _P, _P, _P]),
    "gdmae_prep_tokens": (_I, [_P, _P, _P, _L, _I, _P, _P, _I, _P]),
    "gdmae_sum_bf16": (_I, [_P, _I, _L, _P, _P]),
    "gdmae_add3": (_I, [_P, _P, _I, _P, _I, _L, _P, _P]),
    "gdmae_add3_to": (_I, [_P, _P, _I, _P, _I, _L, _P, _I, _P]),
    "gdmae_set_attention_impl": (_I, [_I]),
    "gdmae_sum_partials": (_I, [_P, _L, _F, _P, _I, _P]),
    "gdmae_sum_partials_gated": (_I, [_P, _L, _F, _P, _P, _F, _P]),
    "gdmae_gemm_workspace_bytes": (_Z, []),
    "gdmae_gemm_stats": (_I, [_P]),
    "gdmae_gemm_tuning": (_I, [_I]),
    "gdmae_gemm": (_I, [_P, _P, _P, _L, _L, _L, _I, _I, _I, _I, _P, _P, _P]),
    "gdmae_gemm_tn_splitk_workspace_bytes": (_Z, [_L, _I, _I]),
    "gdmae_gemm_tn_splitk": (_I, [_P, _P, _P, _L, _I, _I, _I, _I, _P, _P]),
    "gdmae_conv_block_scratch_bytes": (_Z, [_L, _L, _I, _I, _I]),
    "gdmae_spconv_packed_bytes": (_Z, [_I, _I]),
    "gdmae_spconv_pack_jobs": (_I, [_P, _I, _I, _I, _P, _P]),
    "gdmae_spconv": (_I, [_P, _I, _P, _P, _L, _I, _I, _P, _I, _P]),
    "gdmae_spconv_bias_relu": (_I, [_P, _I, _P, _P, _P, _L, _I, _I, _P, _P]),
    "gdmae_spconv_stat_rows": (_I, [_I, _I, _I]),
    "gdmae_spconv_stats": (_I, [_P, _I, _P, _P, _L, _I, _I, _P, _P, _P]),
    "gdmae_decoder_dy": (_I, [_P, _P, _I, _P, _P, _P, _P, _I, _I, _I, _P, _P]),
    "gdmae_decoder_dy_rows": (_I, [_P, _P, _I, _P, _P, _P, _P, _P, _P, _I, _I, _I, _P, _P]),
    "gdmae_decoder_site_rulebook": (_I, [_P, _P, _I, _L, _P, _I, _I, _P, _P]),
    "gdmae_tap_dw_rows": (_L, [_L, _I, _I]),
    "gdmae_tap_dw_workspace_bytes": (_Z, [_L, _I, _I]),
    "gdmae_tap_dw": (_I, [_P, _L, _L, _I, _P, _P, _I, _P, _I, _I, _P, _P]),
    "gdmae_decoder_block_dw_workspace_bytes": (_Z, [_L, _I]),
    "gdmae_decoder_block_dw": (_I, [_P, _P, _P, _P, _P, _L, _I, _P, _P, _I, _I, _P, _I, _I, _P, _P]),
    "gdmae_conv_block_fwd": (_I, [_P, _P]),
    "gdmae_conv_block_bwd": (_I, [_P, _P]),
    "gdmae_encoder_layer_bytes": (_I, [_L, _I, _I, _I, _I, _P, _P, _P]),
    "gdmae_dw_gemm_workspace_bytes": (_Z, [_L, _I, _I]),
    "gdmae_dw_gemm": (_I, [_P, _P, _L, _I, _I, _P, _P, _P, _P]),
    "gdmae_layer_packed_bytes": (_Z, [_I, _I]),
    "gdmae_layer_pack_jobs": (_I, [_P, _P, _P, _P, _I, _I, _P, _P]),
    "gdmae_layer_pack_job_count": (_I, [_I, _I]),
    "gdmae_tok_gemm_pack": (_I, [_P, _I, _P]),
    "gdmae_tok_gemm": (_I, [_P, _P, _P, _L, _L, _I, _I, _I, _P, _P, _P, _P, _P, _P, _F, _P, _P, _P, _P, _P, _P, _P]),
    "gdmae_tok_gemm_qkv": (_I, [_P, _P, _P, _P, _P, _L, _I, _P, _P, _P]),
    "gdmae_tok_gemm_ffn": (_I, [_P, _P, _P, _P, _P, _L, _L, _I, _P, _P, _P, _P, _F, _P, _P, _P, _P, _P, _P, _P, _P]),
    "gdmae_tok_gemm_ln_bwd_rows": (_I, [_I]),
    "gdmae_tok_gemm_ln_bwd": (_I, [_P, _P, _L, _L, _I, _I, _P, _P, _P, _P, _P, _P, _P, _P, _P, _P]),
    "gdmae_encoder_layer_fwd": (_I, [_P, _P]),
    "gdmae_encoder_layer_bwd": (_I, [_P, _P]),
    "gdmae_encoder_stage_fwd": (_I, [_P, _I, _P]),
    "gdmae_encoder_stage_bwd": (_I, [_P, _I, _P]),
    "gdmae_deconv_rows_packed_bytes": (_Z, [_I, _I, _I]),
    "gdmae_deconv_rows_pack": (_I, [_P, _I, _I, _I, _P, _P, _P]),
    "gdmae_deconv_rows_fwd": (_I, [_P, _L, _I, _I, _I, _P, _P, _P]),
    "gdmae_deconv_rows_bwd_input": (_I, [_P, _L, _I, _I, _I, _P, _P, _P]),
    "gdmae_deconv_rows_dw_workspace_bytes": (_Z, [_L, _I, _I, _I]),
    "gdmae_deconv_rows_bwd_weight": (_I, [_P, _P, _L, _I, _I, _I, _P, _P, _P]),
    "gdmae_pred_head_packed_bytes": (_Z, []),
    "gdmae_pred_head_pack": (_I, [_P, _P, _I, _I, _P, _P]),
    "gdmae_pred_head_fwd": (_I, [_P, _L, _I, _P, _P, _P, _P, _P]),
    "gdmae_pred_head_bwd_workspace_bytes": (_Z, [_L]),
    "gdmae_pred_head_bwd": (_I, [_P, _I, _P, _P, _P, _P, _L, _I, _P, _P, _P, _P, _P, _P]),
    "gdmae_encoder_set_layer_path": (_I, [_I]),
    "gdmae_encoder_stage_fused": (_I, [_P, _I]),
    "gdmae_group_gt_points": (_I, [_P, _I, _P, _P, _P, _I, _I, _P, _P, _P, _P, _P]),
    "gdmae_chamfer": (_I, [_P, _P, _P, _I, _I, _I, _P, _P, _P]),
    "gdmae_chamfer_points": (_I, [_P, _P, _I, _P, _P, _P, _P, _P, _P, _I, _I, _I, _P, _P, _P]),
    "gdmae_augment_collate_workspace_bytes": (_Z, [_L]),
    "gdmae_augment_collate": (_I, [_P, _L, _I, _P, _I, _P, _P, _P, _P, _P, _P]),
    "gdmae_gt_sample_workspace_bytes": (_Z, [_L]),
    "gdmae_gt_sample_select": (_I, [_P, _P, _P, _P, _I, _I, _P, _P, _P, _I, _I, _P, _P, _P, _P, _P, _P]),
    "gdmae_gt_sample_collate": (_I, [_P, _P, _I, _P, _I, _L, _I, _P, _P, _P, _P, _P, _P, _P, _P, _P, _P]),
    "gdmae_group_workspace_bytes": (_Z, [_L, _L]),
    "gdmae_ingroup_inds": (_I, [_P, _L, _L, _P, _P, _Z, _P]),
    "gdmae_group_inner_inds": (_I, [_P, _L, _L, _I, _P, _P, _Z, _P]),
    "gdmae_center_head_targets_workspace_bytes": (_Z, [_I, _I]),
    "gdmae_center_head_targets": (_I, [_P, _I, _I, _I, _P, _I, _I, _P, _P, _F, _I, _I, _I, _D, _I, _P, _P, _P, _P, _P, _P]),
    "gdmae_center_head_targets_iou": (_I, [_P, _I, _I, _I, _P, _I, _I, _P, _P, _F, _I, _I, _I, _D, _I, _P, _P, _P, _P, _P, _P, _P]),
    "gdmae_focal_loss_rows": (_I, []),
    "gdmae_focal_loss_fwd": (_I, [_P, _I, _P, _P, _I, _I, _I, _I, _P, _P, _P, _P]),
    "gdmae_focal_loss_bwd": (_I, [_P, _I, _P, _P, _I, _I, _I, _I, _P, _P, _P, _I, _P]),
    "gdmae_center_head_decode": (_I, [_P, _P, _P, _P, _P, _P, _P, _P, _I, _I, _I, _I, _P, _P, _F, _P, _F, _I, _P, _P, _P, _P, _P]),
    "gdmae_center_head_detect_workspace_bytes": (_Z, [_I, _I, _I]),
    "gdmae_center_head_detect": (_I, [_P] * 8 + [_I] * 4 + [_P, _P, _F, _P, _F, _I, _I, _P, _P, _P, _P, _P, _I, _I] + [_P] * 6),
    "gdmae_anchor_targets_workspace_bytes": (_Z, [_I, _I, _I]),
    "gdmae_anchor_targets": (_I, [_P, _I, _I, _I, _I, _I, _I, _I, _I, _P, _P, _P, _P, _P, _P, _P, _P, _P, _F, _I, _P, _P, _P, _P, _P, _P, _P]),
    "gdmae_anchor_loss_rows": (_I, []),
    "gdmae_anchor_loss_fwd": (_I, [_P, _I, _I, _I, _I, _I, _I, _I, _P, _P, _P, _P, _P, _P, _P, _P, _P]),
    "gdmae_anchor_loss_bwd": (_I, [_P, _I, _I, _I, _I, _I, _I, _I, _P, _P, _P, _P, _P, _P, _P, _P, _P]),
    "gdmae_anchor_decode": (_I, [_P, _I, _I, _I, _I, _I, _I, _I, _I, _P, _P, _P, _F, _F, _P, _P, _P]),
    "gdmae_anchor_select": (_I, [_P, _I, _I, _I, _I, _F, _P, _P, _P, _P, _P]),
    "gdmae_anchor_head_infer_packed_bytes": (_Z, [_I]),
    "gdmae_anchor_head_infer_pack": (_I, [_P, _P, _P, _P, _P, _P, _I, _I, _I, _I, _P, _P]),
    "gdmae_anchor_head_infer_workspace_bytes": (_Z, [_I, _I, _I, _I]),
    "gdmae_anchor_head_infer": (_I, [_P, _I, _I, _I, _I, _I, _I, _I, _P, _P, _P, _P, _F, _F, _F, _P, _P, _P, _P, _P, _P, _P, _P]),
    "gdmae_anchor_detect_workspace_bytes": (_Z, [_I, _I]),
    "gdmae_anchor_detect": (_I, [_P, _P, _P, _P, _I, _I, _I, _I, _F, _I, _P, _P, _P, _P, _P, _P]),
    "gdmae_boxes_bev_pairs": (_I, [_P, _I, _P, _I, _I, _P, _P]),
    "gdmae_nms_workspace_bytes": (_Z, [_I]),
    "gdmae_nms_bev": (_I, [_P, _I, _F, _I, _P, _P, _P, _P]),
    "gdmae_geometry_plan_layout": (_I, [_P, _P, _I, _P, _P]),
    "gdmae_geometry_plan": (_I, [_P, _P, _P, _P, _Z, _P]),
    "gdmae_grad_sq_norm": (_I, [_P, _L, _P, _P, _P]),
    "gdmae_adam_step": (_I, [_P, _P, _P, _P, _P, _I, _F, _F, _F, _F, _F, _I, _F, _F, _P, _P]),
    "gdmae_adam_step_shadow": (_I, [_P, _P, _P, _P, _P, _I, _F, _F, _F, _F, _F, _I, _F, _F, _P, _P, _P]),
    "gdmae_roi_dfvs_pool_workspace_bytes": (_Z, [_L, _I, _I, _I, _I]),
    "gdmae_roi_dfvs_pool": (_I, [_P, _L, _I, _P, _I, _I, _I, _P, _P, _I, _I, _P, _I, _I, _I, _F, _F, _I, _I, _P, _P, _P, _P, _P, _Z, _P]),
    "gdmae_roi_targets_workspace_bytes": (_Z, [_I, _I]),
    "gdmae_roi_targets": (_I, [_P, _P, _P, _I, _I, _I, _P, _I, _P, _P, _P, _I, _I, _F, _F, _F, _F, _I, _I, _P, _P, _P, _P, _P, _P, _P, _P, _P, _P, _Z, _P]),
    "gdmae_recall_record": (_I, [_P, _P, _I, _I, _I, _P, _P, _I, _I, _P, _I, _I, _P, _I, _P, _P, _P]),
    "gdmae_kitti_eval_frames_per_chunk": (_I, []),
    "gdmae_kitti_eval_workspace_bytes": (_Z, [_I, _I]),
    "gdmae_kitti_eval": (_I, [_I, _I, _I] + [_P] * 21 + [_I] + [_P] * 9 + [_Z, _P]),
    "gdmae_kitti_annos": (_I, [_P, _I, _P, _P, _P, _P, _P, _I, _I, _I, _P, _I, _P, _I, _P, _P, _P, _P, _P, _P, _P, _P]),
    "gdmae_once_eval_frames_per_chunk": (_I, []),
    "gdmae_once_eval_workspace_bytes": (_Z, [_I, _I]),
    "gdmae_once_eval": (_I, [_I] * 6 + [_P] * 22 + [_Z, _P]),
    "gdmae_roi_graph_folded_floats": (_Z, []),
    "gdmae_roi_graph_packed_bytes": (_Z, []),
    "gdmae_roi_graph_workspace_bytes": (_Z, [_L]),
    "gdmae_roi_graph_pack": (_I, [_P, _P, _P]),
    "gdmae_roi_graph_forward": (_I, [_P, _P, _P, _I, _P, _I, _I, _I, _P, _P, _P, _P, _P, _P, _P, _Z, _P]),
}
# ... 95 lines not shown
```

gd-mae_amd/gdmae_hip/plan.py:

```python
from __future__ import annotations

from dataclasses import dataclass, field
from typing import List, Optional

import torch

from . import lib as L

I32 = torch.int32


def _empty(n, dtype, dev):
    return torch.empty(int(n), dtype=dtype, device=dev)


@dataclass
class VoxelPlan:
    batch_size: int
    grid: tuple
    lo: tuple
    vs: tuple
    n_cols: int
    N: int
    M: int
    points: torch.Tensor
    point_coords: torch.Tensor
    inverse: torch.Tensor
    inverse32: torch.Tensor
    voxel_coords: torch.Tensor
    pillar_cell: torch.Tensor
    pt_off: torch.Tensor
    pillar_pts: torch.Tensor
    point_rank: torch.Tensor
    sample_off: torch.Tensor
    pillar_mean: torch.Tensor
    cell2pillar: torch.Tensor
    counts: torch.Tensor
    points_pm: torch.Tensor = None
    row_pillar: torch.Tensor = None


def _voxelize_launch(points: torch.Tensor, point_cloud_range, voxel_size, grid_size, batch_size: int) -> dict:
    assert points.is_cuda and points.dtype == torch.float32 and points.dim() == 2
    points = points.contiguous()
    dev = points.device
    n0, ncols = points.shape
    gx, gy, gz = (int(g) for g in grid_size)
    cells = batch_size * gx * gy * gz
    lo = tuple(float(v) for v in point_cloud_range[:3])
    vs = tuple(float(v) for v in voxel_size)
    F = ncols - 1
    cap = max(n0, 1)
    r = dict(batch_size=batch_size, grid=(gx, gy, gz), lo=lo, vs=vs, ncols=ncols, n0=n0, src=points,
             pts_out=_empty(cap * ncols, torch.float32, dev), pcoords=_empty(cap * 4, torch.int64, dev),
             inverse=_empty(cap, torch.int64, dev), inverse32=_empty(cap, I32, dev), vcoords=_empty(cap * 4, torch.int64, dev),
             pillar_cell=_empty(cap, I32, dev), pt_off=_empty(cap + 1, I32, dev), pillar_pts=_empty(cap, I32, dev),
             prank=_empty(cap, I32, dev), sample_off=_empty(batch_size + 1, I32, dev), mean=_empty(cap * F, torch.float32, dev),
             cell2pillar=_empty(cells, I32, dev), counts=_empty(2, I32, dev))
    wsb = L.load().gdmae_voxelize_workspace_bytes(n0, batch_size, gx, gy, gz)
    r["ws"] = _empty(wsb, torch.uint8, dev)
    L.call("gdmae_voxelize", L.ptr(points), n0, ncols, L.host_f32(lo), L.host_f32(vs), L.host_i32((gx, gy, gz)),
           batch_size, L.ptr(r["pts_out"]), L.ptr(r["pcoords"]), L.ptr(r["inverse"]), L.ptr(r["inverse32"]), L.ptr(r["vcoords"]),
           L.ptr(r["pillar_cell"]), L.ptr(r["pt_off"]), L.ptr(r["pillar_pts"]), L.ptr(r["prank"]), L.ptr(r["sample_off"]),
           L.ptr(r["mean"]), L.ptr(r["cell2pillar"]), L.ptr(r["counts"]), L.ptr(r["ws"]), wsb, L.stream())
    r["pts_pm"] = _empty(cap * ncols, torch.float32, dev)
    r["row_pillar"] = _empty(cap, I32, dev)
    L.call("gdmae_pillar_major_rows", L.ptr(r["pts_out"]), ncols, L.ptr(r["pillar_pts"]), L.ptr(r["inverse32"]), L.ptr(r["counts"]),
           cap, L.ptr(r["pts_pm"]), L.ptr(r["row_pillar"]), L.stream())
    return r


def _voxelize_finalize(r: dict, N: int, M: int) -> VoxelPlan:
    ncols = r["ncols"]
    F = ncols - 1
    return VoxelPlan(r["batch_size"], r["grid"], r["lo"], r["vs"], ncols, N, M,
                     r["pts_out"][:N * ncols].view(N, ncols), r["pcoords"][:N * 4].view(N, 4), r["inverse"][:N],
                     r["inverse32"][:N], r["vcoords"][:M * 4].view(M, 4), r["pillar_cell"][:M], r["pt_off"][:M + 1],
                     r["pillar_pts"][:N], r["prank"][:N], r["sample_off"], r["mean"][:M * F].view(M, F), r["cell2pillar"],
                     r["counts"], r["pts_pm"][:N * ncols].view(N, ncols), r["row_pillar"][:N])


def voxelize(points: torch.Tensor, point_cloud_range, voxel_size, grid_size, batch_size: int) -> VoxelPlan:
    r = _voxelize_launch(points, point_cloud_range, voxel_size, grid_size, batch_size)
    N, M = (int(v) for v in r["counts"].tolist())
    return _voxelize_finalize(r, N, M)


@dataclass
class WindowPlan:
    tok_win: torch.Tensor
    tok_level: torch.Tensor
    tok_slot: torch.Tensor
    tok_pos: torch.Tensor
    csr_tok: torch.Tensor
    win_start: torch.Tensor
    win_len: torch.Tensor
    n_win: List[int] = field(default_factory=list)
    n_tok: List[int] = field(default_factory=list)
    max_tokens: List[int] = field(default_factory=list)


@dataclass
class StagePlan:
    B: int
    Y: int
    X: int
    n_tok: int
    tok_cell: torch.Tensor
    map: torch.Tensor
    nbr_subm: torch.Tensor
    nbr_down: Optional[torch.Tensor]
    nbr_down_t: Optional[torch.Tensor]
    windows: List[WindowPlan] = field(default_factory=list)

    def indices_byx(self) -> torch.Tensor:
        c = self.tok_cell.long()
        x = c % self.X
        r = c // self.X
        return torch.stack([r // self.Y, r % self.Y, x], dim=-1).int()


@dataclass
class DecoderTiles:
    sources: tuple
    B: int
    H: int
    W: int
    n_act: int
    tile_slot: torch.Tensor
    tile_list: torch.Tensor
    nbr: Optional[list] = None


@dataclass
class VfeVisible:
    n_rows: int
    row_tok: torch.Tensor
    vis_rows: torch.Tensor
    vis_tok: torch.Tensor
    tok_row_off: torch.Tensor
    tok_pillar: torch.Tensor
    n_pillars: int


@dataclass
class EncoderPlan:
    mask: Optional[torch.Tensor]
    tok_pillar: torch.Tensor
    stages: List[StagePlan]
    dec_tiles: Optional[DecoderTiles] = None
    vfe_vis: Optional[VfeVisible] = None


def upsample_cells(c: torch.Tensor, Ys: int, Xs: int, s: int) -> torch.Tensor:
    x = c % Xs
    r = torch.div(c, Xs, rounding_mode='floor')
    y = r % Ys
    b = torch.div(r, Ys, rounding_mode='floor')
    d = torch.arange(s, device=c.device, dtype=c.dtype)
    yy = (y * s).view(-1, 1, 1) + d.view(1, s, 1)
    xx = (x * s).view(-1, 1, 1) + d.view(1, 1, s)
    return ((b.view(-1, 1, 1) * (Ys * s) + yy) * (Xs * s) + xx).reshape(c.numel(), s * s)


def _drop_arrays(drop_info):
    d = {int(k): v for k, v in drop_info.items()}
    keys = sorted(d)
    assert keys == list(range(len(keys))) and len(keys) <= 3
    lo = [int(d[k]["drop_range"][0]) for k in keys]
    hi = [int(d[k]["drop_range"][1]) for k in keys]
    T = [int(d[k]["max_tokens"]) for k in keys]
    return lo, hi, T


def _decoder_tiles_launch(maps, ups, B, H, W, dev) -> dict:
    nt = B * ((H + 7) // 8) * ((W + 7) // 8)
    r = dict(tile_slot=_empty(nt, I32, dev), tile_list=_empty(nt, I32, dev), n_act=_empty(1, I32, dev), B=B, H=H, W=W)
    ws = _empty(L.load().gdmae_decoder_tiles_workspace_bytes(B, H, W), torch.uint8, dev)
    L.call("gdmae_decoder_tiles", L.host_ptrs(maps), L.host_i32(ups), len(maps), B, H, W, L.ptr(r["tile_slot"]),
           L.ptr(r["tile_list"]), L.ptr(r["n_act"]), L.ptr(ws), L.stream())
    r["_ws"] = ws
    return r


def decoder_tiles(ep: "EncoderPlan", sources, H: int, W: int) -> DecoderTiles:
    sources = tuple(int(v) for v in sources)
    dt = ep.dec_tiles
    if dt is not None and dt.sources == sources and dt.H == H and dt.W == W:
        return dt
    st = [ep.stages[i] for i in sources]
    B = st[0].B
    ups = [H // sp.Y for sp in st]
    assert all(sp.Y * u == H and sp.X * u == W for sp, u in zip(st, ups))
    r = _decoder_tiles_launch([sp.map for sp in st], ups, B, H, W, st[0].map.device)
    n = int(r["n_act"].item())
    ep.dec_tiles = DecoderTiles(sources, B, H, W, n, r["tile_slot"], r["tile_list"][:n])
    ep.dec_tiles.nbr = _site_rulebooks(ep.dec_tiles, st, ups)
    return ep.dec_tiles


def decoder_site_rulebooks(dt: "DecoderTiles", sites, ups, n_tok=None):
    out = []
    for g, (st, u) in enumerate(zip(sites, ups)):
        n_dev = torch.tensor([st.numel() // (u * u) if n_tok is None else n_tok[g]], dtype=I32, device=st.device)
        nbr = _empty(st.numel() * 9, I32, st.device)
        L.call("gdmae_decoder_site_rulebook", L.ptr(st.contiguous()), L.ptr(n_dev), u * u, st.numel(), L.ptr(dt.tile_slot), dt.H, dt.W,
               L.ptr(nbr), L.stream())
        out.append(nbr.view(-1, 9))
    return out


def _site_rulebooks(dt: "DecoderTiles", stages, ups):
    sites = (sp.tok_cell if u == 1 else (sp._up_sites[1] if getattr(sp, "_up_sites", None) is not None and sp._up_sites[0] == u
                                         else upsample_cells(sp.tok_cell, sp.Y, sp.X, u).reshape(-1).contiguous())
             for sp, u in zip(stages, ups))
    return decoder_site_rulebooks(dt, sites, ups, [sp.n_tok for sp in stages])


def _encoder_launch(vox, m_cap: int, strides, window_shapes, drop_infos, keep_frac, noise, dec_sources=None) -> dict:
    if isinstance(vox, dict):
        dev, grid, B = vox["src"].device, vox["grid"], vox["batch_size"]
        sample_off, pillar_cell, vcounts = vox["sample_off"], vox["pillar_cell"], vox["counts"]
    else:
        dev, grid, B = vox.points.device, vox.grid, vox.batch_size
        sample_off, pillar_cell, vcounts = vox.sample_off, vox.pillar_cell, vox.counts
    gx, gy, gz = grid
    assert gz == 1, "the SST backbone works on single-layer pillar grids (spt_backbone_mae.py:94)"
    lib = L.load()
    st = L.stream()
    M = m_cap
    scan_ws = _empty(8 * (max(B * gx * gy, M) // 4096 + 4), torch.int64, dev)

    if keep_frac is not None:
        if noise is None:
            noise = torch.rand(max(M, 1), device=dev, dtype=torch.float32)
        assert noise.numel() >= 1 and noise.dtype == torch.float32
        mask = _empty(max(M, 1), torch.float32, dev)
        len_keep = _empty(B, I32, dev)
        L.call("gdmae_random_mask", L.ptr(noise.contiguous()), L.ptr(sample_off), B, float(keep_frac), L.ptr(mask),
               L.ptr(len_keep), st)
    else:
        mask = torch.zeros(max(M, 1), dtype=torch.float32, device=dev)

    cap = max(M, 1)
    Y, X = gy, gx
    tok_pillar = _empty(cap, I32, dev)
    tok_cell = _empty(cap, I32, dev)
    smap = _empty(B * Y * X, I32, dev)
    n_tok = _empty(1, I32, dev)
    L.call("gdmae_visible_tokens", L.ptr(mask), L.ptr(pillar_cell), L.ptr(vcounts), M, B * Y * X,
           L.ptr(tok_pillar), L.ptr(tok_cell), L.ptr(smap), L.ptr(n_tok), L.ptr(scan_ws), st)

    raw = []
    for si, stride in enumerate(strides):
        if stride > 1:
            assert stride == 2, "only the k3 s2 p1 strided sparse conv of the shipped configs is implemented"
            Yi, Xi = Y, X
            Y, X = (Yi - 1) // 2 + 1, (Xi - 1) // 2 + 1
            cap_in = cap
            cap = min(4 * cap_in, B * Y * X)
            tok_cell_n = _empty(cap, I32, dev)
            smap_n = _empty(B * Y * X, I32, dev)
            n_tok_n = _empty(1, I32, dev)
            flag = _empty(B * Y * X, I32, dev)
            L.call("gdmae_downsample_tokens", L.ptr(n_tok), L.ptr(tok_cell), cap_in, B, Yi, Xi, L.ptr(tok_cell_n),
                   L.ptr(smap_n), L.ptr(n_tok_n), L.ptr(flag), L.ptr(scan_ws), st)
            nbr_down = _empty(cap * 9, I32, dev)
            L.call("gdmae_rulebook", L.ptr(n_tok_n), L.ptr(tok_cell_n), cap, B, Y, X, Yi, Xi, L.ptr(smap), 1,
                   L.ptr(nbr_down), st)
            nbr_down_t = _empty(cap_in * 9, I32, dev)
            L.call("gdmae_rulebook", L.ptr(n_tok), L.ptr(tok_cell), cap_in, B, Yi, Xi, Y, X, L.ptr(smap_n), 2,
                   L.ptr(nbr_down_t), st)
            tok_cell, smap, n_tok = tok_cell_n, smap_n, n_tok_n
        else:
            nbr_down = nbr_down_t = None
        nbr_subm = _empty(cap * 9, I32, dev)
        L.call("gdmae_rulebook", L.ptr(n_tok), L.ptr(tok_cell), cap, B, Y, X, Y, X, L.ptr(smap), 0, L.ptr(nbr_subm), st)
        wx, wy, wz = (int(v) for v in window_shapes[si])
        assert wz == 1
        dlo, dhi, dT = _drop_arrays(drop_infos[si])
        assert wx * wy <= max(dT), "token drop would not be the identity: unsupported (SURVEY header item 5)"
        wsb = lib.gdmae_window_workspace_bytes(B, Y, X, wx, wy)
        wins = []
        for shifted in (0, 1):
            nwin_cap = B * ((X + wx - 1) // wx + 1) * ((Y + wy - 1) // wy + 1)
            w = dict(tok_win=_empty(cap, I32, dev), tok_level=_empty(cap, I32, dev), tok_slot=_empty(cap, I32, dev),
                     tok_pos=_empty(cap, I32, dev), csr_tok=_empty(cap, I32, dev),
                     win_start=_empty(min(nwin_cap, cap), I32, dev), win_len=_empty(min(nwin_cap, cap), I32, dev),
                     counts=_empty(8, I32, dev), T=dT)
            ws = _empty(wsb, torch.uint8, dev)
            L.call("gdmae_window_partition", L.ptr(smap), B, Y, X, wx, wy, shifted, len(dT), L.host_i32(dlo),
                   L.host_i32(dhi), L.host_i32(dT), L.ptr(w["tok_win"]), L.ptr(w["tok_level"]), L.ptr(w["tok_slot"]),
                   L.ptr(w["tok_pos"]), L.ptr(w["csr_tok"]), L.ptr(w["win_start"]), L.ptr(w["win_len"]),
                   L.ptr(w["counts"]), L.ptr(ws), wsb, st)
            w["_ws"] = ws
            wins.append(w)
        nbr_subm_t = torch.flip(nbr_subm.view(cap, 9), dims=[1]).contiguous().view(-1)
        up_s = gy // Y
        up_sites = upsample_cells(tok_cell, Y, X, up_s) if (up_s > 1 and up_s * Y == gy and up_s * X == gx) else None
        raw.append(dict(B=B, Y=Y, X=X, cap=cap, tok_cell=tok_cell, map=smap, n_tok=n_tok, nbr_subm=nbr_subm,
                        nbr_subm_t=nbr_subm_t, up_s=up_s, up_sites=up_sites, nbr_down=nbr_down, nbr_down_t=nbr_down_t, wins=wins))
    dec = None
    if dec_sources is not None:
        srcs = [raw[int(i)] for i in dec_sources]
        if all(r["up_s"] * r["Y"] == gy and r["up_s"] * r["X"] == gx and r["up_s"] in (1, 2, 4, 8) for r in srcs):
            dec = _decoder_tiles_launch([r["map"] for r in srcs], [r["up_s"] for r in srcs], B, gy, gx, dev)
            dec["sources"] = tuple(int(i) for i in dec_sources)
    counts = torch.cat([r["n_tok"] for r in raw] + [w["counts"] for r in raw for w in r["wins"]]
                       + ([dec["n_act"]] if dec is not None else []))
    return dict(stages=raw, mask=mask, tok_pillar=tok_pillar, masked=keep_frac is not None, counts=counts,
                keep=(noise, scan_ws), dec=dec)


def _encoder_finalize(e: dict, allc, M: int) -> EncoderPlan:
    raw = e["stages"]
    ns = len(raw)
    stages = []
    for si, r in enumerate(raw):
        n = int(allc[si])
        wps = []
        for k, w in enumerate(r["wins"]):
            c = allc[ns + 8 * (2 * si + k): ns + 8 * (2 * si + k) + 8]
            assert c[7] == n, (c, n)
            nw = int(c[6])
            wps.append(WindowPlan(w["tok_win"][:n], w["tok_level"][:n], w["tok_slot"][:n], w["tok_pos"][:n],
                                  w["csr_tok"][:n], w["win_start"][:nw], w["win_len"][:nw],
                                  [int(v) for v in c[0:3]], [int(v) for v in c[3:6]], list(w["T"])))
        n_prev = int(allc[si - 1]) if r["nbr_down"] is not None else 0
        stages.append(StagePlan(r["B"], r["Y"], r["X"], n, r["tok_cell"][:n], r["map"],
                                r["nbr_subm"][:n * 9].view(n, 9),
                                None if r["nbr_down"] is None else r["nbr_down"][:n * 9].view(n, 9),
                                None if r["nbr_down_t"] is None else r["nbr_down_t"][:n_prev * 9].view(n_prev, 9),
                                wps))
        stages[-1]._nbr_subm_t = r["nbr_subm_t"][:n * 9].view(n, 9)
        stages[-1]._up_sites = None if r["up_sites"] is None else (r["up_s"], r["up_sites"][:n].reshape(-1))
    dec = e.get("dec", None)
    dt = None
    if dec is not None:
        n_act = int(allc[ns + 16 * ns])
        dt = DecoderTiles(dec["sources"], dec["B"], dec["H"], dec["W"], n_act, dec["tile_slot"], dec["tile_list"][:n_act])
    return EncoderPlan(e["mask"][:M] if e["masked"] else None, e["tok_pillar"][:stages[0].n_tok], stages, dt)


def encoder_plan(vox: VoxelPlan, strides, window_shapes, drop_infos, keep_frac: Optional[float] = None,
                 noise: Optional[torch.Tensor] = None, dec_sources=None) -> EncoderPlan:
    if noise is not None:
        assert noise.shape == (vox.M,)
    e = _encoder_launch(vox, vox.M, strides, window_shapes, drop_infos, keep_frac, noise, dec_sources)
    return _encoder_finalize(e, e["counts"].tolist(), vox.M)


import collections
import time as _time

EVENT_WAIT_S = 0.0

_PLAN_SHAPES = collections.OrderedDict()
_PLAN_SHAPES_MAX = 32
_PLAN_GRANULE = 16384
_PINNED = {}


def _plan_shape(n0, ncols, B, pcr, voxel_size, grid_size, strides, window_shapes, drop_infos, keep_frac, dec_sources):
    gx, gy, gz = (int(g) for g in grid_size)
    lo = tuple(float(v) for v in pcr[:3])
    vs = tuple(float(v) for v in voxel_size)
    drops = tuple(tuple(map(tuple, _drop_arrays(d))) for d in drop_infos)
    n_exact = n0
    n0 = max(1, (n0 + _PLAN_GRANULE - 1) // _PLAN_GRANULE) * _PLAN_GRANULE
    key = (n0, ncols, B, lo, vs, (gx, gy, gz), tuple(int(s) for s in strides), tuple(tuple(int(v) for v in w) for w in window_shapes),
           drops, None if keep_frac is None else float(keep_frac), None if dec_sources is None else tuple(int(i) for i in dec_sources))
    hit = _PLAN_SHAPES.get(key)
    if hit is not None:
        _PLAN_SHAPES.move_to_end(key)
        return hit
    del n_exact
    import ctypes as C
    ns = len(strides)
    assert gz == 1, "the SST backbone works on single-layer pillar grids (spt_backbone_mae.py:94)"
    assert 1 <= ns <= 4
    P = L.PlanParams()
    P.n_points, P.cap_points, P.n_cols, P.batch_size = n0, n0, ncols, B
    for i in range(3):
        P.lo[i], P.vs[i] = lo[i], vs[i]
        P.grid[i] = (gx, gy, gz)[i]
    P.n_stages = ns
    geo = []
    Y, X = gy, gx
    cap = max(1, min(n0, B * gx * gy))
    m_cap = cap
    for i in range(ns):
        wx, wy, wz = (int(v) for v in window_shapes[i])
        assert wz == 1
        dlo, dhi, dT = drops[i]
        assert wx * wy <= max(dT), "token drop would not be the identity: unsupported (SURVEY header item 5)"
        P.stride[i], P.win_x[i], P.win_y[i], P.n_levels[i] = int(strides[i]), wx, wy, len(dT)
        for l in range(len(dT)):
            P.drop_lo[i][l], P.drop_hi[i][l], P.max_tokens[i][l] = dlo[l], dhi[l], dT[l]
        cap_in = cap
        if int(strides[i]) > 1:
            assert int(strides[i]) == 2, "only the k3 s2 p1 strided sparse conv of the shipped configs is implemented"
            Y, X = (Y - 1) // 2 + 1, (X - 1) // 2 + 1
            cap = min(4 * cap, B * Y * X)
        us = gy // Y
        up_s = us if (us >= 1 and us * Y == gy and us * X == gx) else 0
        geo.append(dict(Y=Y, X=X, cap=cap, cap_in=cap_in, up_s=up_s, strided=int(strides[i]) > 1, T=list(dT)))
    P.masked = int(keep_frac is not None)
    P.keep_frac = float(keep_frac) if keep_frac is not None else 1.0
    P.n_dec = 0 if dec_sources is None else len(dec_sources)
    for g in range(P.n_dec):
        P.dec_sources[g] = int(dec_sources[g])
    P.want_pm = 1
    table = (L.PlanBuffer * 160)()
    n_ent, total = C.c_int(0), C.c_size_t(0)
    L.call("gdmae_geometry_plan_layout", C.byref(P), table, 160, C.byref(n_ent), C.byref(total))
    names = {table[i].name.decode(): (int(table[i].offset), int(table[i].bytes)) for i in range(n_ent.value)}
    hit = _PLAN_SHAPES[key] = (P, names, int(total.value), geo, m_cap, (lo, vs, (gx, gy, gz)))
    while len(_PLAN_SHAPES) > _PLAN_SHAPES_MAX:
        _PLAN_SHAPES.popitem(last=False)
    return hit


class _Arena:

    def __init__(self, raw, names):
        self.raw, self.names = raw, names
        self.base = {torch.int32: raw.view(torch.int32), torch.float32: raw.view(torch.float32), torch.int64: raw.view(torch.int64)}

    def has(self, name):
        return name in self.names

    def view(self, name, dtype, *shape):
        off, _ = self.names[name]
        es = 8 if dtype == torch.int64 else 4
        strides, acc = [], 1
        for d in reversed(shape):
            strides.append(acc)
            acc *= int(d)
        return self.base[dtype].as_strided(tuple(int(d) for d in shape), tuple(reversed(strides)), off // es)


class PlanPrefetch:

    _side = {}
    _arena_bytes = {}

    def __init__(self, points, point_cloud_range, voxel_size, grid_size, batch_size, strides, window_shapes, drop_infos,
                 keep_frac=None, noise=None, ready=None, dec_sources=None):
        import ctypes as C
        assert points.is_cuda and points.dtype == torch.float32 and points.dim() == 2
        points = points.contiguous()
        dev = points.device
        main = torch.cuda.current_stream(dev)
        side = PlanPrefetch._side.setdefault(dev.index, torch.cuda.Stream(device=dev))
        side.wait_stream(main)
        if ready is not None:
            side.wait_event(ready)
        points.record_stream(side)
        if noise is not None:
            noise.record_stream(side)
        n0, ncols = points.shape
        P, names, total, geo, m_cap, _ = self.shape = _plan_shape(n0, ncols, int(batch_size), point_cloud_range, voxel_size, grid_size,
                                                                    strides, window_shapes, drop_infos, keep_frac, dec_sources)
        self.masked, self.dec_sources, self.batch_size, self.ncols = keep_frac is not None, dec_sources, int(batch_size), ncols
        with torch.cuda.stream(side):
            cap = PlanPrefetch._arena_bytes.get(dev.index, 0)
            if total > cap:
                cap = PlanPrefetch._arena_bytes[dev.index] = -(-total // (64 << 20)) * (64 << 20)
            raw = torch.empty(cap, dtype=torch.uint8, device=dev)
            if self.masked and noise is None:
                noise = torch.rand(m_cap, device=dev, dtype=torch.float32)
            if noise is not None:
                assert noise.dtype == torch.float32 and noise.numel() >= 1
                noise = noise.contiguous()
            Pc = L.PlanParams.from_buffer_copy(P)
            Pc.n_points = n0
            L.call("gdmae_geometry_plan", C.byref(Pc), L.ptr(points), None if noise is None else L.ptr(noise), L.ptr(raw), total, L.stream())
            self.arena = _Arena(raw, names)
            nc = names["counts"][1] // 4
            assert nc <= 256
            free = _PINNED.setdefault(dev.index, [])
            self._pinned = free.pop() if free else torch.empty(256, dtype=torch.int32).pin_memory()
            self.host = self._pinned[:nc]
            self.host.copy_(self.arena.view("counts", torch.int32, nc), non_blocking=True)
            self.event = torch.cuda.Event()
            self.event.record(side)
        self.side, self.keep, self.points = side, noise, points
        self.serial = side == main

    def finish(self):
        assert self.serial or torch.cuda.current_stream() != self.side, "plan tensors must not be consumed on the plan stream"
        global EVENT_WAIT_S
        t_w = _time.perf_counter()
        self.event.synchronize()
        EVENT_WAIT_S += _time.perf_counter() - t_w
        torch.cuda.current_stream().wait_event(self.event)
        c = self.host.tolist()
        self.points_device = self.points.device
        self.host = None
        if self._pinned is not None:
            _PINNED.setdefault(self.points_device.index, []).append(self._pinned)
            self._pinned = None
        P, names, total, geo, m_cap, (lo, vs, grid) = self.shape
        A, V = self.arena, self.arena.view
        i32, f32, i64 = torch.int32, torch.float32, torch.int64
        B, ncols = self.batch_size, self.ncols
        F = ncols - 1
        N, M = int(c[0]), int(c[1])
        gx, gy, gz = grid
        vox = VoxelPlan(B, grid, lo, vs, ncols, N, M, V("points", f32, N, ncols), V("point_coords", i64, N, 4), V("inverse", i64, N),
                        V("inverse32", i32, N), V("voxel_coords", i64, M, 4), V("pillar_cell", i32, M), V("pt_off", i32, M + 1),
                        V("pillar_pts", i32, N), V("point_rank", i32, N), V("sample_off", i32, B + 1), V("pillar_mean", f32, M, F),
                        V("cell2pillar", i32, B * gx * gy * gz), V("counts", i32, 2), V("points_pm", f32, N, ncols), V("row_pillar", i32, N))
        vox._arena = A
        ns = len(geo)
        n_vis = int(c[2 + ns + 16 * ns + 1])
        stages = []
        for i, g in enumerate(geo):
            n = int(c[2 + i])
            pre = f"s{i}."
            wps = []
            for k in range(2):
                wc = c[2 + ns + 16 * i + 8 * k: 2 + ns + 16 * i + 8 * k + 8]
                assert wc[7] == n, (wc, n)
                nw = int(wc[6])
                wpre = f"{pre}w{k}."
                wps.append(WindowPlan(V(wpre + "tok_win", i32, n), V(wpre + "tok_level", i32, n), V(wpre + "tok_slot", i32, n),
                                      V(wpre + "tok_pos", i32, n), V(wpre + "csr_tok", i32, n), V(wpre + "win_start", i32, nw),
                                      V(wpre + "win_len", i32, nw), [int(v) for v in wc[0:3]], [int(v) for v in wc[3:6]], list(g["T"])))
            n_prev = (int(c[2 + i - 1]) if i > 0 else n_vis) if g["strided"] else 0
            sp = StagePlan(B, g["Y"], g["X"], n, V(pre + "tok_cell", i32, n), V(pre + "map", i32, B * g["Y"] * g["X"]),
                           V(pre + "nbr_subm", i32, n, 9), V(pre + "nbr_down", i32, n, 9) if g["strided"] else None,
                           V(pre + "nbr_down_t", i32, n_prev, 9) if g["strided"] else None, wps)
            sp._nbr_subm_t = V(pre + "nbr_subm_t", i32, n, 9)
            sp._up_sites = (g["up_s"], V(pre + "up_sites", i32, n * g["up_s"] * g["up_s"])) if g["up_s"] > 1 else None
            stages.append(sp)
        dt = None
        if A.has("dec.tile_slot"):
            n_act = int(c[2 + ns + 16 * ns])
            nt = B * ((gy + 7) // 8) * ((gx + 7) // 8)
            nbrs = [V(f"dec.nbr{g}", i32, stages[int(si)].n_tok * geo[int(si)]["up_s"] ** 2, 9) for g, si in enumerate(self.dec_sources)]
            dt = DecoderTiles(tuple(int(i) for i in self.dec_sources), B, gy, gx, n_act, V("dec.tile_slot", i32, nt), V("dec.tile_list", i32, n_act),
                              nbrs)
        ep = EncoderPlan(V("mask", f32, M) if self.masked else None, V("tok_pillar", i32, stages[0].n_tok if not geo[0]["strided"] else n_vis),
                         stages, dt)
        if self.masked and A.has("vfe.row_tok"):
            nt, nv = ep.tok_pillar.numel(), int(c[2 + ns + 16 * ns + 2])
            ep.vfe_vis = VfeVisible(nv, V("vfe.row_tok", i32, N), V("vfe.vis_rows", i32, nv), V("vfe.vis_tok", i32, nv),
                                    V("vfe.tok_row_off", i32, nt + 1), ep.tok_pillar, M)
        self.arena = self.points = self.keep = None
        return vox, ep


def _tensors_of(obj):
    out = []
    if isinstance(obj, torch.Tensor):
        if obj.is_cuda:
            out.append(obj)
    elif isinstance(obj, dict):
        for v in obj.values():
            out += _tensors_of(v)
    elif isinstance(obj, (list, tuple)):
        for v in obj:
            out += _tensors_of(v)
    return out
```

include/gdmae_hip.h:

```cpp
#ifndef GDMAE_HIP_H
#define GDMAE_HIP_H

#include <stddef.h>
#include <stdint.h>

#ifdef __cplusplus
extern "C" {
#endif

int gdmae_abi_version(void);
const char* gdmae_target_arch(void);
const char* gdmae_last_error(void);

size_t gdmae_voxelize_workspace_bytes(long long n_points, int batch_size, int gx, int gy, int gz);
int gdmae_voxelize(const float* points, long long n_points, int n_cols, const float* lo, const float* vs,
                   const int* grid_xyz, int batch_size, float* points_out, long long* point_coords,
                   long long* inverse, int* inverse32, long long* voxel_coords, int* pillar_cell,
                   int* pillar_pt_off, int* pillar_pts, int* point_rank, int* sample_pillar_off,
                   float* pillar_mean, int* cell2pillar, int* counts, void* workspace, size_t workspace_bytes,
                   void* stream);

int gdmae_decorate_points(const float* points, const long long* point_coords, const int* inverse32,
                          const float* pillar_mean, long long N, int n_cols, const float* lo, const float* vs,
                          float* out, void* stream);
int gdmae_pillar_major_rows(const float* points, int n_cols, const int* pillar_pts, const int* inverse32, const int* n_dev,
                            long long capacity, float* points_pm, int* row_pillar, void* stream);
int gdmae_vfe_infer(const float* points_pm, const long long* voxel_coords, const int* row_pillar, const float* pillar_mean,
                    long long N, long long M, int n_cols, const float* lo, const float* vs, const float* W1, const float* b1,
                    int c1, const float* W2, const float* b2, int c2, float* out, void* stream);
size_t gdmae_vfe_point_layer_workspace_bytes(int n_cols);
int gdmae_vfe_point_layer_fwd(const float* points, const long long* point_coords, const int* inverse32,
                              const float* pillar_mean, int coords_per_pillar, long long N, int n_cols, const float* lo,
                              const float* vs,
                              const float* W, int C, const float* gamma, const float* beta, double eps, double momentum,
                              float* running_mean, float* running_var, long long* num_batches, double* stats, float* ab,
                              float* mv, void* out, int out_bf16, void* workspace, void* stream);
int gdmae_vfe_point_layer_bwd(const float* points, const long long* point_coords, const int* inverse32,
                              const float* pillar_mean, int coords_per_pillar, long long N, int n_cols, const float* lo,
                              const float* vs,
                              const float* W, int C, const float* gamma, const double* stats, const float* ab,
                              const void* g, int g_bf16, float* dgamma, float* dbeta, float* dW, int accumulate,
                              void* workspace, void* stream);
size_t gdmae_vfe_max_layer_workspace_bytes(void);
int gdmae_vfe_max_layer_fwd(const void* y1, long long N, const void* W, const int* pillar_pt_off, const int* row_pillar,
                            int M, const float* gamma, const float* beta, double eps, double momentum,
                            float* running_mean, float* running_var, long long* num_batches, double* stats, float* ab,
                            float* mv, float* out, int* arg, void* workspace, void* stream);
int gdmae_vfe_max_layer_bwd(const void* y1, long long N, const void* W, const int* row_pillar, int M, const float* gamma,
                            const double* stats, const float* ab, const float* out, const int* arg, const float* g, void* gm,
                            void* dy1, float* dgamma, float* dbeta, float* dW, int accumulate,
                            void* workspace, void* stream);
int gdmae_vfe_max_layer_fwd_f16(const void* y1, long long N, const float* W, const int* pillar_pt_off, const int* row_pillar,
                                int M, const float* gamma, const float* beta, double eps, double momentum,
                                float* running_mean, float* running_var, long long* num_batches, double* stats, float* ab,
                                float* mv, float* out, int* arg, void* workspace, void* stream);
int gdmae_vfe_max_layer_bwd_f16(const void* y1, long long N, const float* W, const int* row_pillar, int M, const float* gamma,
                                const double* stats, const float* ab, const float* out, const int* arg, const float* g, void* gm,
                                void* dy1, float* dgamma, float* dbeta, float* dW, int accumulate,
                                void* workspace, void* stream);
int gdmae_vfe_max_layer_vis_fwd(const void* y1, long long N, const void* W, const int* vis_rows, const int* vis_tok, long long Nv,
                                int n_tok, const float* gamma, const float* beta, double eps, double momentum,
                                float* running_mean, float* running_var, long long* num_batches, double* stats, float* ab,
                                float* mv, float* out, int* arg, void* workspace, void* stream);
int gdmae_vfe_max_layer_vis_fwd_f16(const void* y1, long long N, const float* W, const int* vis_rows, const int* vis_tok, long long Nv,
                                    int n_tok, const float* gamma, const float* beta, double eps, double momentum,
                                    float* running_mean, float* running_var, long long* num_batches, double* stats, float* ab,
                                    float* mv, float* out, int* arg, void* workspace, void* stream);
int gdmae_vfe_max_layer_vis_bwd(const void* y1, long long N, const void* W, const int* row_tok, const int* tok_pillar, int n_tok, int M,
                                const float* gamma, const double* stats, const float* ab, const float* out, const int* arg,
                                const float* g, void* gm, void* dy1, float* dgamma, float* dbeta, float* dW, int accumulate,
                                void* workspace, void* stream);
int gdmae_vfe_max_layer_vis_bwd_f16(const void* y1, long long N, const float* W, const int* row_tok, const int* tok_pillar, int n_tok, int M,
                                    const float* gamma, const double* stats, const float* ab, const float* out, const int* arg,
                                    const float* g, void* gm, void* dy1, float* dgamma, float* dbeta, float* dW, int accumulate,
                                    void* workspace, void* stream);
int gdmae_segment_max(const float* x, const int* pillar_pt_off, const int* pillar_pts, int M, int C, float* out,
                      int* arg, void* stream);
int gdmae_segment_max_bwd(const float* dout, const int* arg, const int* inverse32, long long N, int C, float* dx,
                          void* stream);

int gdmae_random_mask(const float* noise, const int* sample_pillar_off, int batch_size, double keep_frac,
                      float* mask_out, int* len_keep_out, void* stream);

int gdmae_visible_tokens(const float* mask, const int* pillar_cell, const int* vox_counts, long long m_cap,
                         long long n_cells, int* tok_pillar, int* tok_cell, int* map, int* n_tok, void* scan_ws,
                         void* stream);
int gdmae_downsample_tokens(const int* n_in, const int* tok_cell_in, long long cap_in, int B, int Yi, int Xi,
                            int* tok_cell_out, int* map_out, int* n_out, int* flag_ws, void* scan_ws, void* stream);
int gdmae_rulebook(const int* n_tok, const int* tok_cell, long long cap, int B, int Yt, int Xt, int Ym, int Xm,
                   const int* map, int mode, int* nbr, void* stream);

size_t gdmae_window_workspace_bytes(int B, int Y, int X, int wx, int wy);
int gdmae_window_partition(const int* map, int B, int Y, int X, int wx, int wy, int shifted, int nlev,
                           const int* drop_lo, const int* drop_hi, const int* max_tokens, int* tok_win,
                           int* tok_level, int* tok_slot, int* tok_pos, int* csr_tok, int* win_start, int* win_len,
                           int* counts, void* workspace, size_t workspace_bytes, void* stream);

int gdmae_gather_rows(const void* src, const int* idx, long long n_slots, int row_bytes, void* out, void* stream);
int gdmae_scatter_rows(const void* src, const int* idx, long long n_rows, int row_bytes, void* dst, void* stream);

int gdmae_gather_rows_strided(const void* src, const int* idx, long long n_slots, int row_bytes, int table_row_bytes,
                              int table_col_bytes, void* out, void* stream);
int gdmae_scatter_rows_strided(const void* src, const int* idx, long long n_rows, int row_bytes, int table_row_bytes,
                               int table_col_bytes, void* dst, void* stream);
size_t gdmae_colstats_workspace_bytes(int C);
int gdmae_colstats(const void* x, long long R, int C, int is_bf16, double* out, void* workspace, void* stream);

size_t gdmae_decoder_region_workspace_bytes(int C2, int Cin);
int gdmae_decoder_region_algebra(const double* stats2, const float* ab2, const double* st2, const float* k01,
                                 const double* reg, const double* tap_region, const double* cnt, double R, int C2, int Cin,
                                 const float* conv_w, const void* bgz, int cdt_bf16, double* S, double* tot, float* dWk,
                                 void* Wd, void* workspace, void* stream);
int gdmae_fill_rows(const void* v, long long R, int C, int elem_bytes, void* Z, void* stream);
int gdmae_rows_affine_relu_scatter(const void* P, int p_bf16, const int* site, long long n, int C, const float* a,
                                   const float* b, void* Z, int z_bf16, int z_row_elems, int col0, void* stream);
int gdmae_rows_affine_relu_sub(const void* P, int p_bf16, const int* site, long long n, int C, const float* a, const float* b,
                               const void* sub, void* Z, int z_bf16, int z_row_elems, int col0, void* stream);
int gdmae_rows_affine_relu_add(const void* P, int p_bf16, long long n, int C, const float* a, const float* b, const void* R, void* Z,
                               int z_bf16, void* stream);
size_t gdmae_rows_bwd_stats_workspace_bytes(int C);
int gdmae_rows_bwd_stats(const void* P, int p_bf16, const int* site, long long n, int C, const float* a, const float* b,
                         const void* dZ, int z_bf16, int z_row_elems, int col0, double* out, void* workspace, void* stream);
int gdmae_rows_bwd(const void* P, int p_bf16, const int* site, long long n, int C, const float* a, const float* b,
                   const float* c0, const float* c1, const void* dZ, int z_bf16, int z_row_elems, int col0, void* dP,
                   int dp_bf16, void* stream);

int gdmae_bn_fold(const void* x, long long R, int C, int is_bf16, double count, const float* gamma, const float* beta,
                  double eps, double momentum, float* running_mean, float* running_var, long long* num_batches,
                  double* stats, float* ab, float* mv, void* workspace, void* stream);
int gdmae_bn_fold_partials(const float* part, int nblk, int C, double count, const float* gamma, const float* beta, double eps,
                           double momentum, float* running_mean, float* running_var, long long* num_batches, double* stats, float* ab,
                           float* mv, void* stream);
int gdmae_bn_bwd_coeffs(const double* st, int n_st, const double* stats, const float* ab, const float* gamma, int C,
                        double count, const double* tot, float* dgamma, float* dbeta, int accumulate, float* c01,
                        void* stream);
int gdmae_rows_bwd_stats_rows(long long n);
int gdmae_bn_bwd_coeffs_rows(const float* part, int nblk, int n_st, const double* stats, const float* ab, const float* gamma, int C,
                             double count, const double* tot, float* dgamma, float* dbeta, int accumulate, float* c01,
                             void* stream);

int gdmae_conv3x3_grad_taps(const void* Y, int y_bf16, const int* tile_slot, const void* ybg, const float* k0,
                            const float* k1, const float* rows, const int* cell2pillar, const int* site, long long n, int H,
                            int W, int C, void* out, void* stream);

size_t gdmae_border_sums_workspace_bytes(int B, int C);
int gdmae_border_sums(const void* Y, int y_bf16, const int* tile_slot, const void* ybg, const float* rows,
                      const int* pillar_cell, int M, int B, int H, int W, int C, double* out, void* workspace, void* stream);
int gdmae_border_sums_rows(const void* Y, int y_bf16, const int* tile_slot, const void* ybg, const float* dout, const void* yrows,
                           const float* a2, const float* b2, const int* pillar_cell, int M, int B, int H, int W, int C, double* out,
                           void* workspace, void* stream);

size_t gdmae_decoder_tiles_workspace_bytes(int B, int H, int W);
int gdmae_decoder_tiles(const int* const* maps, const int* strides, int k, int B, int H, int W, int* tile_slot, int* tile_list,
                        int* n_act, void* workspace, void* stream);
size_t gdmae_conv3x3_tiles_packed_bytes(int k);
int gdmae_conv3x3_tiles_pack(const float* conv_w, int C2, int Cin, const float* const* b, int k, void* Wp, void* bgz, void* ybg,
                             void* stream);
size_t gdmae_conv3x3_tiles_workspace_bytes(int n_act);
int gdmae_conv3x3_tiles_fwd(const void* const* P, const int* const* maps, const float* const* a, const float* const* b,
                            const int* strides, int k, const void* Wp, const void* ybg, const int* tile_list, int n_act, int B,
                            int H, int W, void* Yc, const float* gamma, const float* beta, double eps, double momentum,
                            float* running_mean, float* running_var, long long* num_batches, double* stats, float* ab,
                            float* mv, void* workspace, void* stream);
int gdmae_tiles_gather_rows(const void* Yc, const int* tile_slot, const void* ybg, const int* cell, long long n, int H, int W,
                            int C, int elem_bytes, void* out, void* stream);
int gdmae_tiles_gather_rows_affine_relu(const void* Yc, const int* tile_slot, const void* ybg, const int* cell, long long n, int H, int W,
                                        int C, const float* a, const float* b, void* yrows, float* out, void* stream);
int gdmae_tiles_to_dense(const void* Yc, const int* tile_slot, const void* ybg, int B, int H, int W, int C, int elem_bytes,
                         void* out, void* stream);
int gdmae_tiles_to_dense_affine_relu(const void* Yc, const int* tile_slot, const void* ybg, int B, int H, int W, int C, const float* a,
                                     const float* b, float* out, void* stream);

int gdmae_segment_max_affine(const void* x, int x_bf16, const int* pillar_pt_off, const int* pillar_pts, int M, int C,
                             const float* a, const float* b, float* out, int* arg, void* stream);
int gdmae_segmax_bwd_stats(const void* x, int x_bf16, const float* out, const int* arg, const float* dout, long long M,
                           int C, const float* a ,
                           const float* b, double* sums, void* workspace, void* stream);
int gdmae_segmax_bn_bwd(const void* x, int x_bf16, const float* out, const int* arg, const float* dout,
                        const int* inverse32, long long N, int C, const float* a, const float* c0, const float* c1,
                        void* dx, int dx_bf16, void* stream);

int gdmae_set_attention_impl(int impl);
int gdmae_window_attention_fwd(const void* qk, const void* v, void* out, int io_bf16, const int* csr_tok,
                               const int* win_start, const int* win_len, int n_win, int T, int d, int H,
                               const float* tau, float tau_min, void* stream);
int gdmae_window_attention_bwd(const void* qk, const void* v, const void* dout, void* dqk, void* dv, int io_bf16,
                               float* dtau_part, const int* csr_tok, const int* win_start, const int* win_len,
                               int n_win, int T, int d, int H, const float* tau, float tau_min, void* stream);
int gdmae_window_attention_levels_writes_lse(int io_bf16, int n_levels, const int* max_tokens, int d, int H);
int gdmae_window_attention_levels_fwd(const void* qk, const void* v, void* out, int io_bf16, const int* csr_tok,
                                      const int* win_start, const int* win_len, int n_levels, const int* n_win,
                                      const int* max_tokens, int d, int H, const float* tau, float tau_min, float* lse, void* stream);
int gdmae_window_attention_levels_bwd(const void* qk, const void* v, const void* dout, void* dqk, void* dv, int io_bf16,
                                      float* dtau_part, const int* csr_tok, const int* win_start, const int* win_len,
                                      int n_levels, const int* n_win, const int* max_tokens, int d, int H, const float* tau,
                                      float tau_min, const void* out, const float* lse, void* stream);
int gdmae_attention_timing(int on);
int gdmae_attention_timing_read(int which, double* total_ms, long long* calls);
int gdmae_kernel_timing(int on);
int gdmae_kernel_timing_slots(void);
const char* gdmae_kernel_timing_name(int slot);
int gdmae_kernel_timing_read(int slot, double* total_ms, long long* calls, double* bytes, double* flops);
int gdmae_kernel_timing_read_side(int slot, double* side_bytes);
int gdmae_weighted_mean_finish(const float* term, const float* weights, long long n, float* out, void* stream);
int gdmae_sum_partials(const float* part, long long n, float scale, float* out, int accumulate, void* stream);
int gdmae_sum_partials_gated(const float* part, long long n, float scale, float* out, const float* gate, float gate_min,
                             void* stream);

size_t gdmae_add_layernorm_workspace_bytes(int d);
int gdmae_add_layernorm_fwd(const float* a, const void* b, int b_is_bf16, const float* gamma, const float* beta,
                            long long n, int d, float eps, float* y, float* stats, void* y_bf16 ,
                            void* stream);
int gdmae_add_layernorm_bwd(const float* a, const void* b, int b_is_bf16, const float* gamma, const float* stats,
                            const float* dy, const void* dy2, int dy2_bf16, long long n, int d, float* dx, void* dx_bf16,
                            float* sums, void* workspace, void* stream);
int gdmae_prep_tokens(const float* x, const float* pos_table, const int* tok_pos, long long n, int d, void* x_out,
                      void* xpos_out, int out_bf16, void* stream);
int gdmae_sum_bf16(const void* const* src, int k, long long total, void* out, void* stream);
int gdmae_add3(const float* a, const void* b, int b_bf16, const void* c, int c_bf16, long long total, float* out, void* stream);
int gdmae_add3_to(const float* a, const void* b, int b_bf16, const void* c, int c_bf16, long long total, void* out, int out_bf16,
                  void* stream);

int gdmae_gemm_stats(long long* calls);
int gdmae_gemm_tuning(int mode);
size_t gdmae_gemm_workspace_bytes(void);
int gdmae_gemm(const void* A, const void* B, void* C, long long M, long long N, long long K, int trans_a, int trans_b,
               int ab_bf16, int c_f32, const void* bias, void* workspace, void* stream);
size_t gdmae_gemm_tn_splitk_workspace_bytes(long long K, int m, int n);
int gdmae_gemm_tn_splitk(const void* A, const void* B, float* C, long long K, int m, int n, int ab_bf16, int accumulate,
                         void* workspace, void* stream);

size_t gdmae_dw_gemm_workspace_bytes(long long rows, int M, int N);
int gdmae_dw_gemm(const void* G, const void* X, long long rows, int M, int N, float* dW, float* dbias, void* workspace,
                  void* stream);

typedef struct gdmae_conv_block_args {
  long long n_in, n_out;
  int cin, cout, bf16, x_f32, g_f32;
  float eps, momentum;
  const void* x;
  const int* nbr;
  const int* nbr_t;
  const void* W;
  const float *gamma, *beta;
  float *running_mean, *running_var;
  long long* num_batches;
  void* cols;
  void* y;
  double* stats;
  float* ab;
  float* mv;
  void* out;
  const void* g;
  void* dx;
  float *dW, *dgamma, *dbeta;
  void* scratch;
  const void* packed_fwd;
  const void* packed_bwd;
  int out_f32;
} gdmae_conv_block_args;
size_t gdmae_conv_block_scratch_bytes(long long n_in, long long n_out, int cin, int cout, int bf16);
size_t gdmae_spconv_packed_bytes(int cin, int cout);
int gdmae_spconv_pack_jobs(const float* W , int cin, int cout, int transposed, void* packed, long long* jobs);
int gdmae_spconv(const void* X, int x_f32, const int* nbr, const void* packed, long long n, int cin, int cout, void* Y,
                 int timing_slot , void* stream);
int gdmae_spconv_bias_relu(const void* X, int x_f32, const int* nbr, const void* packed, const float* bias, long long n, int cin, int cout,
                           void* Y, void* stream);
int gdmae_spconv_stat_rows(int cin, int cout, int x_f32);
int gdmae_spconv_stats(const void* X, int x_f32, const int* nbr, const void* packed, long long n, int cin, int cout, void* Y, float* part,
                       void* stream);
int gdmae_decoder_dy(const void* Yc, const int* tile_list, int n_act, const float* k0, const float* k1, const float* rows,
                     const int* cell2pillar, int H, int W, int C, void* dYc, void* stream);
int gdmae_decoder_dy_rows(const void* Yc, const int* tile_list, int n_act, const float* k0, const float* k1, const float* dout,
                          const float* a2, const float* b2, const int* cell2pillar, int H, int W, int C, void* dYc, void* stream);
int gdmae_decoder_site_rulebook(const int* site, const int* n_dev, int sites_per_tok, long long cap_sites, const int* tile_slot,
                                int H, int W, int* nbr, void* stream);
long long gdmae_tap_dw_rows(long long n, int M, int N);
size_t gdmae_tap_dw_workspace_bytes(long long n, int M, int N);
int gdmae_tap_dw(const void* G, long long n, long long n_pad, int M, const void* X, const int* nbr, int N, float* out, int ld_out,
                 int m_off, void* workspace, void* stream);
size_t gdmae_decoder_block_dw_workspace_bytes(long long n, int u);
int gdmae_decoder_block_dw(const void* P, const float* a, const float* b, const void* bg, const int* site, long long n, int u,
                           const void* dYc, const int* tile_slot, int H, int W, float* out, int ld_out, int m_off, void* workspace,
                           void* stream);
int gdmae_conv_block_fwd(const gdmae_conv_block_args* args , void* stream);
int gdmae_conv_block_bwd(const gdmae_conv_block_args* args , void* stream);

typedef struct gdmae_layer_args {
  long long n;
  int d, ff, nhead, bf16;
  float eps, tau_min;
  int n_levels;
  int n_win[4], max_tokens[4];
  const int* tok_pos;
  const int* csr_tok;
  const int* win_start;
  const int* win_len;
  const float* pos_table;
  const void *Win, *bin, *Wo, *bo, *W1, *b1, *W2, *b2;
  const float *g1, *be1, *g2, *be2, *tau;
  const float* x;
  float* y;
  const float* dy;
  float* dx;
  float *dWin, *dbin, *dtau, *dWo, *dbo, *dW1, *db1, *dW2, *db2, *dg1, *dbe1, *dg2, *dbe2;
  void* saved;
  void* scratch;
  const void* packed;
  int x_bf16;
  void* res_out;
  const void* dres;
  void* dx_bf16;
  int path;
} gdmae_layer_args;
size_t gdmae_layer_packed_bytes(int d, int ff);
int gdmae_layer_pack_jobs(const float* Win, const float* Wo, const float* W1, const float* W2, int d, int ff, void* packed,
// ... 249 lines not shown
```

Baseline: 1129.

## Skip empty source stages in tiled decoder conv via precomputed bias contributions

Tiles are classified by the first source stage that has any active cell in their halo, provided the tile lies fully inside the map. The conv kernel then starts from a precomputed per-channel constant (weights times relu(bias) for the empty earlier stages) and skips their MFMA work. Tiles are reordered by class so that the two tiles sharing a block have similar skip depth. This adds an ordering kernel, a single-block pass and the precompute blocks, and it depends on the assumption that inactive source cells equal relu(bias) exactly, which could shift numerics slightly.

```diff
diff --git a/gd-mae_amd/csrc/conv_tiles.hip b/gd-mae_amd/csrc/conv_tiles.hip
--- a/gd-mae_amd/csrc/conv_tiles.hip
+++ b/gd-mae_amd/csrc/conv_tiles.hip
@@ -67,23 +67,87 @@
   const int t = blockIdx.x * 4 + (threadIdx.x >> 6);
   if (t >= B * TH * TW) return;
   const int tx = t % TW, r = t / TW, ty = r % TH, b = r / TH;
-  bool act = false;
+  int tok = 0;
+  bool outside = false;
   for (int e = lane; e < 100; e += 64) {
     const int y = ty * 8 - 1 + e / 10, x = tx * 8 - 1 + e % 10;
-    if (y < 0 || y >= H || x < 0 || x >= W) continue;
+    if (y < 0 || y >= H || x < 0 || x >= W) {
+      outside = true;
+      continue;
+    }
     for (int g = 0; g < Mp.k; ++g) {
       const int ls = Mp.ls[g];
-      act |= Mp.map[g][(b * (H >> ls) + (y >> ls)) * (W >> ls) + (x >> ls)] >= 0;
-    }
-  }
-  const unsigned long long m = __ballot(act);
-  if (lane == 0) flag[t] = m != 0ull;
+      tok |= (Mp.map[g][(b * (H >> ls) + (y >> ls)) * (W >> ls) + (x >> ls)] >= 0) << g;
+    }
+  }
+  int any = 0;
+  for (int g = 0; g < Mp.k; ++g) any |= (__ballot((tok >> g) & 1) != 0ull) << g;
+  const bool out = __ballot(outside) != 0ull;
+  int cls = 0;
+  while (cls < Mp.k - 1 && !((any >> cls) & 1)) ++cls;
+  if (lane == 0) flag[t] = (any != 0) | ((out ? 0 : cls) << 1);
 }
 
 struct CtFlagLoad {
   const int* flag;
-  __device__ int operator()(long long i) const { return flag[i]; }
+  __device__ int operator()(long long i) const { return flag[i] & 1; }
 };
+
+#define CT_ORD_THREADS 1024
+__global__ __launch_bounds__(CT_ORD_THREADS) void k_ct_tile_order(const int* __restrict__ flag, const int* __restrict__ tile_list,
+                                                                  const int* __restrict__ n_act, int* __restrict__ tile_class,
+                                                                  int* __restrict__ tile_order) {
+  __shared__ int wcnt[CT_ORD_THREADS / 64][CT_MAX_SRC];
+  const int tid = threadIdx.x, lane = tid & 63, wv = tid >> 6;
+  const int n = *n_act;
+  int c[CT_MAX_SRC];
+#pragma unroll
+  for (int g = 0; g < CT_MAX_SRC; ++g) c[g] = 0;
+  for (int s = tid; s < n; s += CT_ORD_THREADS) {
+    const int cls = flag[tile_list[s]] >> 1;
+    tile_class[s] = cls;
+#pragma unroll
+    for (int g = 0; g < CT_MAX_SRC; ++g) c[g] += cls == g;
+  }
+#pragma unroll
+  for (int g = 0; g < CT_MAX_SRC; ++g) {
+    for (int o = 32; o > 0; o >>= 1) c[g] += __shfl_xor(c[g], o, 64);
+    if (lane == 0) wcnt[wv][g] = c[g];
+  }
+  __syncthreads();
+  int run[CT_MAX_SRC];
+  {
+    int tot[CT_MAX_SRC];
+#pragma unroll
+    for (int g = 0; g < CT_MAX_SRC; ++g) {
+      tot[g] = 0;
+      for (int w = 0; w < CT_ORD_THREADS / 64; ++w) tot[g] += wcnt[w][g];
+    }
+    run[0] = 0;
+#pragma unroll
+    for (int g = 1; g < CT_MAX_SRC; ++g) run[g] = run[g - 1] + tot[g - 1];
+  }
+  __syncthreads();
+  for (int s0 = 0; s0 < n; s0 += CT_ORD_THREADS) {
+    const int s = s0 + tid;
+    const int cls = s < n ? flag[tile_list[s]] >> 1 : -1;
+    int rank = 0;
+#pragma unroll
+    for (int g = 0; g < CT_MAX_SRC; ++g) {
+      const unsigned long long m = __ballot(cls == g);
+      if (cls == g) rank = __popcll(m & ((1ull << lane) - 1ull));
+      if (lane == 0) wcnt[wv][g] = __popcll(m);
+    }
+    __syncthreads();
+    int before = 0;
+    for (int w = 0; w < wv; ++w) before += cls >= 0 ? wcnt[w][cls] : 0;
+    if (cls >= 0) tile_order[run[cls] + before + rank] = s;
+#pragma unroll
+    for (int g = 0; g < CT_MAX_SRC; ++g)
+      for (int w = 0; w < CT_ORD_THREADS / 64; ++w) run[g] += wcnt[w][g];
+    __syncthreads();
+  }
+}
 struct CtSlotStore {
   int* slot;
   int* list;
@@ -98,8 +162,8 @@
   return gd_align(sizeof(int) * nt) + gd_align(sizeof(int) * (gd_scan_ws_elems(nt) + 2)) + 256;
 }
 
-extern "C" int gdmae_decoder_tiles(const int* const* maps, const int* strides, int k, int B, int H, int W, int* tile_slot,
-                                   int* tile_list, int* n_act, void* workspace, void* stream) {
+static int ct_decoder_tiles(const int* const* maps, const int* strides, int k, int B, int H, int W, int* tile_slot, int* tile_list,
+                            int* tile_class, int* tile_order, int* n_act, void* workspace, void* stream) {
   GD_REQUIRE(k >= 1 && k <= CT_MAX_SRC, "decoder_tiles: 1..3 source stages");
   GD_REQUIRE(H >= 2 && W >= 2 && B >= 1, "decoder_tiles: map too small");
   hipStream_t st = (hipStream_t)stream;
@@ -119,12 +183,29 @@
   int* scan_ws = A.take<int>(gd_scan_ws_elems(nt) + 2);
   hipLaunchKernelGGL(k_ct_tile_flags, dim3(gd_div_up(nt, 4)), dim3(256), 0, st, Mp, B, H, W, TH, TW, flag);
   GD_LAUNCH_CHECK();
-  return gd_device_scan<int>(nt, CtFlagLoad{flag}, CtSlotStore{tile_slot, tile_list}, n_act, scan_ws, st);
+  if (int rc = gd_device_scan<int>(nt, CtFlagLoad{flag}, CtSlotStore{tile_slot, tile_list}, n_act, scan_ws, st)) return rc;
+  if (tile_class) {
+    hipLaunchKernelGGL(k_ct_tile_order, dim3(1), dim3(CT_ORD_THREADS), 0, st, (const int*)flag, (const int*)tile_list, (const int*)n_act,
+                       tile_class, tile_order);
+    GD_LAUNCH_CHECK();
+  }
+  return 0;
+}
+
+extern "C" int gdmae_decoder_tiles(const int* const* maps, const int* strides, int k, int B, int H, int W, int* tile_slot,
+                                   int* tile_list, int* n_act, void* workspace, void* stream) {
+  return ct_decoder_tiles(maps, strides, k, B, H, W, tile_slot, tile_list, nullptr, nullptr, n_act, workspace, stream);
+}
+
+extern "C" int gdmae_decoder_tiles_classes(const int* const* maps, const int* strides, int k, int B, int H, int W, int* tile_slot,
+                                           int* tile_list, int* tile_class, int* tile_order, int* n_act, void* workspace, void* stream) {
+  GD_REQUIRE(tile_class != nullptr && tile_order != nullptr, "decoder_tiles_classes: tile_class and tile_order");
+  return ct_decoder_tiles(maps, strides, k, B, H, W, tile_slot, tile_list, tile_class, tile_order, n_act, workspace, stream);
 }
 
 size_t gd_decoder_tiles_lb_state_bytes(long long nt) { return gd_scan_lb_state_bytes<int>(nt); }
-int gd_decoder_tiles_lb(const int* const* maps, const int* strides, int k, int B, int H, int W, int* tile_slot, int* tile_list, int* n_act,
-                        int* flag, void* lb_state, hipStream_t st) {
+int gd_decoder_tiles_lb(const int* const* maps, const int* strides, int k, int B, int H, int W, int* tile_slot, int* tile_list,
+                        int* tile_class, int* tile_order, int* n_act, int* flag, void* lb_state, hipStream_t st) {
   GD_REQUIRE(k >= 1 && k <= CT_MAX_SRC, "decoder_tiles: 1..3 source stages");
   CtMaps Mp;
   Mp.k = k;
@@ -138,7 +219,13 @@
   const long long nt = (long long)B * TH * TW;
   hipLaunchKernelGGL(k_ct_tile_flags, dim3(gd_div_up(nt, 4)), dim3(256), 0, st, Mp, B, H, W, TH, TW, flag);
   GD_LAUNCH_CHECK();
-  return gd_device_scan_lb<int>(nt, CtFlagLoad{flag}, CtSlotStore{tile_slot, tile_list}, GdNoTotal{}, n_act, lb_state, st);
+  if (int rc = gd_device_scan_lb<int>(nt, CtFlagLoad{flag}, CtSlotStore{tile_slot, tile_list}, GdNoTotal{}, n_act, lb_state, st)) return rc;
+  if (tile_class && tile_order) {
+    hipLaunchKernelGGL(k_ct_tile_order, dim3(1), dim3(CT_ORD_THREADS), 0, st, (const int*)flag, (const int*)tile_list, (const int*)n_act,
+                       tile_class, tile_order);
+    GD_LAUNCH_CHECK();
+  }
+  return 0;
 }
 
 __global__ __launch_bounds__(256) void k_ct_pack_weights(const float* __restrict__ w, int Cin, int nsteps, uint4* __restrict__ Wp) {
@@ -163,10 +250,66 @@
   const float* b[CT_MAX_SRC];
 };
 
+#define CT_MFMA(a, b, c) __builtin_amdgcn_mfma_f32_32x32x16_f16((a), (b), (c), 0, 0, 0)
+#define CT_OFF(st) ((((st) / CT_KS) / 3) * CT_ROW_PITCH + (((st) / CT_KS) % 3) * CT_PSITE + ((st) % CT_KS) * 32)
+#define CT_WSTEP(st, hf) ((((st) / CT_KS) * 8 + (hf) * CT_KS + ((st) % CT_KS)) * 256)
+#define CT_SKIP_OK (CT_CH == 128 && CT_TPW == 2)
+
+#if CT_SKIP_OK
+#define CT_PRE_RING 36
+__device__ __forceinline__ void ct_pre_block(const uint4* __restrict__ Wp, const CtBPtrs& Bp, int k, float* __restrict__ pre, int wv) {
+  if (threadIdx.x >= 64) return;
+  const int lane = threadIdx.x;
+  const uint4* __restrict__ wp = Wp + wv * 64 + lane;
+  CtFrag wr[CT_PRE_RING];
+#pragma unroll
+  for (int s = 0; s < CT_PRE_RING; ++s) wr[s].q = wp[(s / CT_NSTEP) * CT_NSTEP * 256 + CT_WSTEP(s % CT_NSTEP, 0)];
+  CtFrag bg[CT_MAX_SRC - 1][CT_KS];
+#pragma unroll
+  for (int g = 0; g < CT_MAX_SRC - 1; ++g)
+#pragma unroll
+    for (int ks = 0; ks < CT_KS; ++ks) {
+      bg[g][ks].q = make_uint4(0u, 0u, 0u, 0u);
+      if (g + 1 < k) {
+        const float* b = Bp.b[g] + ks * 16 + (lane >> 5) * 8;
+        const float4 b0 = *(const float4*)b, b1 = *(const float4*)(b + 4);
+        bg[g][ks].q.x = gd_pack_f16_relu(b0.x, b0.y); bg[g][ks].q.y = gd_pack_f16_relu(b0.z, b0.w);
+        bg[g][ks].q.z = gd_pack_f16_relu(b1.x, b1.y); bg[g][ks].q.w = gd_pack_f16_relu(b1.z, b1.w);
+      }
+    }
+  f32x16 acc;
+#pragma unroll
+  for (int i = 0; i < 16; ++i) acc[i] = 0.f;
+#pragma unroll
+  for (int g = 0; g < CT_MAX_SRC - 1; ++g) {
+    if (g + 1 >= k) break;
+#pragma unroll
+    for (int st = 0; st < CT_NSTEP; ++st) {
+      const int s = g * CT_NSTEP + st, sn = s + CT_PRE_RING;
+      CtFrag a;
+      a.q = wr[s % CT_PRE_RING].q;
+      if (sn < (CT_MAX_SRC - 1) * CT_NSTEP) wr[s % CT_PRE_RING].q = wp[(sn / CT_NSTEP) * CT_NSTEP * 256 + CT_WSTEP(sn % CT_NSTEP, 0)];
+      acc = CT_MFMA(a.h, bg[g][st % CT_KS].h, acc);
+    }
+    if ((lane & 31) == 0) {
+#pragma unroll
+      for (int i = 0; i < 16; ++i) pre[g * CT_C + wv * 32 + 4 * (lane >> 5) + 8 * (i >> 2) + (i & 3)] = acc[i];
+    }
+  }
+}
+#endif
+
 __global__ __launch_bounds__(256) void k_ct_class_consts(const float* __restrict__ w, CtBPtrs Bp, int Cin, int C2,
-                                                         unsigned short* __restrict__ bgz, unsigned short* __restrict__ ybg) {
+                                                         unsigned short* __restrict__ bgz, unsigned short* __restrict__ ybg,
+                                                         const uint4* __restrict__ Wp, int k, float* __restrict__ pre) {
   __shared__ double sh[9][256];
   const int o = blockIdx.x;
+  if (o >= C2) {
+#if CT_SKIP_OK
+    ct_pre_block(Wp, Bp, k, pre, o - C2);
+#endif
+    return;
+  }
   double t[9];
 #pragma unroll
   for (int k = 0; k < 9; ++k) t[k] = 0.0;
@@ -202,8 +345,8 @@
 
 extern "C" size_t gdmae_conv3x3_tiles_packed_bytes(int k) { return (size_t)k * 72 * 4 * 64 * 16; }
 
-extern "C" int gdmae_conv3x3_tiles_pack(const float* conv_w, int C2, int Cin, const float* const* b, int k, void* Wp, void* bgz,
-                                        void* ybg, void* stream) {
+static int ct_pack(const float* conv_w, int C2, int Cin, const float* const* b, int k, void* Wp, void* bgz, void* ybg, float* pre,
+                   void* stream) {
   GD_REQUIRE(C2 == CT_C && k >= 1 && k <= CT_MAX_SRC && Cin == CT_C * k, "conv3x3_tiles: 128 output channels, 128 per source");
   hipStream_t st = (hipStream_t)stream;
   const int nsteps = k * 72;
@@ -211,9 +354,22 @@
   GD_LAUNCH_CHECK();
   CtBPtrs Bp;
   for (int g = 0; g < CT_MAX_SRC; ++g) Bp.b[g] = g < k ? b[g] : nullptr;
-  hipLaunchKernelGGL(k_ct_class_consts, dim3(C2), dim3(256), 0, st, conv_w, Bp, Cin, C2, (unsigned short*)bgz, (unsigned short*)ybg);
+  const bool with_pre = CT_SKIP_OK && pre != nullptr && k >= 2;
+  hipLaunchKernelGGL(k_ct_class_consts, dim3(C2 + (with_pre ? 4 : 0)), dim3(256), 0, st, conv_w, Bp, Cin, C2, (unsigned short*)bgz,
+                     (unsigned short*)ybg, (const uint4*)Wp, k, pre);
   GD_LAUNCH_CHECK();
   return 0;
+}
+
+extern "C" int gdmae_conv3x3_tiles_pack(const float* conv_w, int C2, int Cin, const float* const* b, int k, void* Wp, void* bgz,
+                                        void* ybg, void* stream) {
+  return ct_pack(conv_w, C2, Cin, b, k, Wp, bgz, ybg, nullptr, stream);
+}
+
+extern "C" int gdmae_conv3x3_tiles_pack_pre(const float* conv_w, int C2, int Cin, const float* const* b, int k, void* Wp, void* bgz,
+                                            void* ybg, float* pre, void* stream) {
+  GD_REQUIRE(pre != nullptr, "conv3x3_tiles_pack_pre: pre");
+  return ct_pack(conv_w, C2, Cin, b, k, Wp, bgz, ybg, pre, stream);
 }
 
 struct CtSrc {
@@ -231,38 +387,58 @@
   int n_act, H, W, TH, TW;
   unsigned short* Yc;
   float* part;
+  const int* tile_class;
+  const int* tile_order;
+  const float* pre;
 };
-
-#define CT_MFMA(a, b, c) __builtin_amdgcn_mfma_f32_32x32x16_f16((a), (b), (c), 0, 0, 0)
-
-#define CT_OFF(st) ((((st) / CT_KS) / 3) * CT_ROW_PITCH + (((st) / CT_KS) % 3) * CT_PSITE + ((st) % CT_KS) * 32)
-#define CT_WSTEP(st, hf) ((((st) / CT_KS) * 8 + (hf) * CT_KS + ((st) % CT_KS)) * 256)
 
 __global__ __launch_bounds__(CT_THREADS, CT_TPW == 2 ? (CT_CH == 64 ? 3 : 2) : 1) void k_conv3x3_tiles(CtArgs A) {
   extern __shared__ __align__(16) unsigned char lds[];
   const int tid = threadIdx.x, lane = tid & 63, wvg = tid >> 6;
   const int wv = wvg & 3;
   const int tg = wvg >> 2;
-  const int slot0 = blockIdx.x * CT_TPW;
-  int tb[CT_TPW], ty0[CT_TPW], tx0[CT_TPW];
+  const int pos0 = blockIdx.x * CT_TPW;
+  int slot[CT_TPW], tb[CT_TPW], ty0[CT_TPW], tx0[CT_TPW];
   bool have[CT_TPW];
 #pragma unroll
   for (int t = 0; t < CT_TPW; ++t) {
-    have[t] = slot0 + t < A.n_act;
-    const int tile = have[t] ? A.tile_list[slot0 + t] : 0;
+    have[t] = pos0 + t < A.n_act;
+    slot[t] = have[t] ? (A.tile_order ? A.tile_order[pos0 + t] : pos0 + t) : 0;
+    const int tile = have[t] ? A.tile_list[slot[t]] : 0;
     tx0[t] = (tile % A.TW) * 8;
     const int r = tile / A.TW;
     ty0[t] = (r % A.TH) * 8;
     tb[t] = r / A.TH;
   }
+  int lead = 0;
+#if CT_SKIP_OK
+  if (A.tile_class) {
+    lead = A.tile_class[slot[0]];
+    if (have[1]) {
+      const int l1 = A.tile_class[slot[1]];
+      lead = l1 < lead ? l1 : lead;
+    }
+  }
+#endif
   const int lc = tid % CT_CPS;
   const int lsg = tid / CT_CPS;
   const unsigned char* lb = lds + tg * 2 * CT_TILE_PITCH + ((lane & 31) >> 3) * CT_ROW_PITCH + (lane & 7) * CT_PSITE + (lane >> 5) * 16;
   f32x16 acc0, acc1, acc2, acc3;
 #pragma unroll
   for (int i = 0; i < 16; ++i) acc0[i] = acc1[i] = acc2[i] = acc3[i] = 0.f;
-
-  for (int g = 0; g < A.k; ++g) {
+#if CT_SKIP_OK
+  if (lead > 0) {
+    const float* pr = A.pre + (lead - 1) * CT_C + wv * 32 + 4 * (lane >> 5);
+#pragma unroll
+    for (int j = 0; j < 4; ++j) {
+      const float4 v = *(const float4*)(pr + 8 * j);
+      acc0[4 * j] = v.x; acc0[4 * j + 1] = v.y; acc0[4 * j + 2] = v.z; acc0[4 * j + 3] = v.w;
+    }
+    acc1 = acc2 = acc3 = acc0;
+  }
+#endif
+
+  for (int g = lead; g < A.k; ++g) {
     const CtSrc S = A.src[g];
     const int ls = S.ls, sm = (1 << ls) - 1;
     const int Hs = A.H >> ls, Ws = A.W >> ls;
@@ -402,7 +578,7 @@
     for (int p = 0; p < 64 / CT_ESPP; ++p) {
       const int site = p * CT_ESPP + elsg;
       const uint4 v = *(const uint4*)(lds + t * CT_STAGE_PITCH + site * CT_SITE_PITCH + elc * 16);
-      *(uint4*)(A.Yc + ((long long)(slot0 + t) * GD_TILE_SITES + site) * CT_C + elc * 8) = v;
+      *(uint4*)(A.Yc + ((long long)slot[t] * GD_TILE_SITES + site) * CT_C + elc * 8) = v;
       if (ty0[t] + (site >> 3) < A.H && tx0[t] + (site & 7) < A.W) {
         float f[8];
         ct_unpack8(v, f);
@@ -436,7 +612,7 @@
     float v = 0.f;
 #pragma unroll
     for (int w = 0; w < CT_NWAVES; ++w) v += red[((t * CT_NWAVES + w) * 2 + stat) * CT_C + ch];
-    A.part[(long long)(slot0 + t) * 256 + tid] = v;
+    A.part[(long long)slot[t] * 256 + tid] = v;
   }
 }
 
@@ -524,11 +700,11 @@
   return gd_align((size_t)(n_act > 0 ? n_act : 1) * 256 * sizeof(float)) + gd_align((size_t)(CT_NRED + 2) * 256 * sizeof(float));
 }
 
-extern "C" int gdmae_conv3x3_tiles_fwd(const void* const* P, const int* const* maps, const float* const* a, const float* const* b,
-                                       const int* strides, int k, const void* Wp, const void* ybg, const int* tile_list, int n_act,
-                                       int B, int H, int W, void* Yc, const float* gamma, const float* beta, double eps,
-                                       double momentum, float* running_mean, float* running_var, long long* num_batches,
-                                       double* stats, float* ab, float* mv, void* workspace, void* stream) {
+static int ct_fwd(const void* const* P, const int* const* maps, const float* const* a, const float* const* b, const int* strides, int k,
+                  const void* Wp, const void* ybg, const int* tile_list, int n_act, int B, int H, int W, void* Yc, const float* gamma,
+                  const float* beta, double eps, double momentum, float* running_mean, float* running_var, long long* num_batches,
+                  double* stats, float* ab, float* mv, const int* tile_class, const int* tile_order, const float* pre, void* workspace,
+                  void* stream) {
   GD_REQUIRE(k >= 1 && k <= CT_MAX_SRC, "conv3x3_tiles: 1..3 source stages");
   GD_REQUIRE(H >= 2 && W >= 2, "conv3x3_tiles: map too small");
   hipStream_t st = (hipStream_t)stream;
@@ -552,6 +728,9 @@
   A.n_act = n_act;
   A.H = H; A.W = W; A.TH = (H + 7) / 8; A.TW = (W + 7) / 8;
   A.Yc = (unsigned short*)Yc;
+  A.tile_class = CT_SKIP_OK ? tile_class : nullptr;
+  A.tile_order = CT_SKIP_OK ? tile_order : nullptr;
+  A.pre = CT_SKIP_OK ? pre : nullptr;
   GdArena ar(workspace, gdmae_conv3x3_tiles_workspace_bytes(n_act));
   float* part = ar.take<float>((size_t)(n_act > 0 ? n_act : 1) * 256);
   float* red = ar.take<float>((size_t)(CT_NRED + 2) * 256);
@@ -570,6 +749,27 @@
   GD_LAUNCH_CHECK();
   return gd_bn_fold_from_partials(st, red, CT_NRED + 2, CT_C, (double)B * H * W, gamma, beta, eps, momentum, running_mean,
                                   running_var, num_batches, stats, ab, mv);
+}
+
+extern "C" int gdmae_conv3x3_tiles_fwd(const void* const* P, const int* const* maps, const float* const* a, const float* const* b,
+                                       const int* strides, int k, const void* Wp, const void* ybg, const int* tile_list, int n_act,
+                                       int B, int H, int W, void* Yc, const float* gamma, const float* beta, double eps,
+                                       double momentum, float* running_mean, float* running_var, long long* num_batches,
+                                       double* stats, float* ab, float* mv, void* workspace, void* stream) {
+  return ct_fwd(P, maps, a, b, strides, k, Wp, ybg, tile_list, n_act, B, H, W, Yc, gamma, beta, eps, momentum, running_mean, running_var,
+                num_batches, stats, ab, mv, nullptr, nullptr, nullptr, workspace, stream);
+}
+
+extern "C" int gdmae_conv3x3_tiles_fwd_skip(const void* const* P, const int* const* maps, const float* const* a, const float* const* b,
+                                            const int* strides, int k, const void* Wp, const void* ybg, const int* tile_list, int n_act,
+                                            int B, int H, int W, void* Yc, const float* gamma, const float* beta, double eps,
+                                            double momentum, float* running_mean, float* running_var, long long* num_batches,
+                                            double* stats, float* ab, float* mv, const int* tile_class, const int* tile_order,
+                                            const float* pre, void* workspace, void* stream) {
+  const bool none = !tile_class && !tile_order && !pre;
+  GD_REQUIRE(none || (tile_class && tile_order && (pre || k < 2)), "conv3x3_tiles_fwd_skip: tile_class, tile_order and pre, or none of them");
+  return ct_fwd(P, maps, a, b, strides, k, Wp, ybg, tile_list, n_act, B, H, W, Yc, gamma, beta, eps, momentum, running_mean, running_var,
+                num_batches, stats, ab, mv, tile_class, tile_order, pre, workspace, stream);
 }
 
 template <int ES>
diff --git a/gd-mae_amd/csrc/plan.hip b/gd-mae_amd/csrc/plan.hip
--- a/gd-mae_amd/csrc/plan.hip
+++ b/gd-mae_amd/csrc/plan.hip
@@ -45,7 +45,8 @@
 };
 int gd_plan_windows_all(const GdWinStage* stages, int n_stages, hipStream_t st);
 size_t gd_decoder_tiles_lb_state_bytes(long long nt);
-int gd_decoder_tiles_lb(const int* const* maps, const int* strides, int k, int B, int H, int W, int* tile_slot, int* tile_list, int* n_act,
+int gd_decoder_tiles_lb(const int* const* maps, const int* strides, int k, int B, int H, int W, int* tile_slot, int* tile_list,
+                        int* tile_class, int* tile_order, int* n_act,
                         int* flag, void* lb_state, hipStream_t st);
 int gd_decoder_site_rulebook(const int* site, const int* n_dev, int sites_per_tok, long long cap_sites, const int* tile_slot, int H, int W,
                              int* nbr, hipStream_t st);
@@ -92,7 +93,7 @@
     long long tok_cell, map, nbr_subm, nbr_subm_t, nbr_down, nbr_down_t, up_sites, win_ws;
     long long w[2][7];
   } s[GDMAE_PLAN_MAX_STAGES];
-  long long dec_slot, dec_list, dec_flag, dec_nbr[3];
+  long long dec_slot, dec_list, dec_flag, dec_class, dec_order, dec_nbr[3];
   size_t lb_bytes, vox_ws_bytes;
   int n_counts;
   bool dec;
@@ -279,11 +280,13 @@
         O.s[i].w[sh][k] = L.add(nm, sizeof(int) * (k < 5 ? g.cap : wcap));
       }
   }
-  O.dec_slot = O.dec_list = O.dec_flag = -1;
+  O.dec_slot = O.dec_list = O.dec_flag = O.dec_class = O.dec_order = -1;
   if (O.dec) {
     O.dec_slot = L.add("dec.tile_slot", sizeof(int) * nt);
     O.dec_list = L.add("dec.tile_list", sizeof(int) * nt);
     O.dec_flag = L.add("dec.flag", sizeof(int) * nt);
+    O.dec_class = L.add("dec.tile_class", sizeof(int) * nt);
+    O.dec_order = L.add("dec.tile_order", sizeof(int) * nt);
     for (int g = 0; g < p->n_dec; ++g) {
       const StageGeo& sg = O.geo[p->dec_sources[g]];
       snprintf(nm, sizeof(nm), "dec.nbr%d", g);
@@ -410,7 +413,8 @@
       maps[g] = I(O.s[p->dec_sources[g]].map);
       ups[g] = O.geo[p->dec_sources[g]].up_s;
     }
-    int rc = gd_decoder_tiles_lb(maps, ups, p->n_dec, B, gy, gx, I(O.dec_slot), I(O.dec_list), n_act, I(O.dec_flag), lb, st);
+    int rc = gd_decoder_tiles_lb(maps, ups, p->n_dec, B, gy, gx, I(O.dec_slot), I(O.dec_list), I(O.dec_class), I(O.dec_order), n_act,
+                                 I(O.dec_flag), lb, st);
     if (rc) return rc;
     for (int g = 0; g < p->n_dec; ++g) {
       const int si = p->dec_sources[g];
diff --git a/gd-mae_amd/gdmae_hip/decoder.py b/gd-mae_amd/gdmae_hip/decoder.py
--- a/gd-mae_amd/gdmae_hip/decoder.py
+++ b/gd-mae_amd/gdmae_hip/decoder.py
@@ -19,6 +19,7 @@
 BLOCK_BWD = os.environ.get("GDMAE_DEC_BLOCK", "1")
 DY_ROWS = os.environ.get("GDMAE_DEC_DY_ROWS", "1") != "0"
 GATHER_FUSED = os.environ.get("GDMAE_DEC_GATHER_FUSED", "1") != "0"
+CT_SKIP = os.environ.get("GDMAE_CT_SKIP", "1")
 
 
 
@@ -81,6 +82,7 @@
     tiles: gplan.DecoderTiles
     maps: list
     ups: list
+    skip: str = "0"
 
 
 @dataclass(frozen=True, eq=False)
@@ -107,8 +109,16 @@
     bgz = torch.empty(Cin, dtype=cdt, device=dev)
     ybg = torch.empty(9, C2, dtype=cdt, device=dev)
     a_l, b_l = [ab[:w] for ab, w in zip(ab_l, widths)], [ab[w:] for ab, w in zip(ab_l, widths)]
-    L.call("gdmae_conv3x3_tiles_pack", L.ptr(conv_w), C2, Cin, L.host_ptrs(b_l), k, L.ptr(Wp), L.ptr(bgz), L.ptr(ybg),
-           L.stream())
+    skip = tc.skip != "0" and k >= 2 and dt.tile_class is not None and dt.tile_order is not None
+    pre = order = None
+    if skip:
+        pre = torch.empty(k - 1, C2, dtype=torch.float32, device=dev)
+        L.call("gdmae_conv3x3_tiles_pack_pre", L.ptr(conv_w), C2, Cin, L.host_ptrs(b_l), k, L.ptr(Wp), L.ptr(bgz), L.ptr(ybg), L.ptr(pre),
+               L.stream())
+        order = dt.tile_order if tc.skip != "ascending" else torch.arange(dt.n_act, dtype=torch.int32, device=dev)
+    else:
+        L.call("gdmae_conv3x3_tiles_pack", L.ptr(conv_w), C2, Cin, L.host_ptrs(b_l), k, L.ptr(Wp), L.ptr(bgz), L.ptr(ybg),
+               L.stream())
     y2 = torch.empty(max(dt.n_act, 1) * 64, C2, dtype=cdt, device=dev)
     stats2 = torch.empty(2 * C2, dtype=torch.float64, device=dev)
     ab2 = torch.empty(2 * C2, dtype=torch.float32, device=dev)
@@ -120,10 +130,10 @@
         pre_conv_hook()
     with timing.kernel("k_conv3x3_tiles", dt.n_act * 64 * (Cin + C2) * 2, flops,
                        {"dense_equivalent_TFLOPs_per_launch": round(2.0 * B * H * W * C2 * 9 * Cin / 1e12, 4), "active_tiles": dt.n_act}):
-        L.call("gdmae_conv3x3_tiles_fwd", L.host_ptrs([P.contiguous() for P in Ps]), L.host_ptrs(tc.maps), L.host_ptrs(a_l),
+        L.call("gdmae_conv3x3_tiles_fwd_skip", L.host_ptrs([P.contiguous() for P in Ps]), L.host_ptrs(tc.maps), L.host_ptrs(a_l),
                L.host_ptrs(b_l), L.host_i32(tc.ups), k, L.ptr(Wp), L.ptr(ybg), L.ptr(dt.tile_list), dt.n_act, B, H, W,
                L.ptr(y2), L.ptr(gamma2), L.ptr(beta2), float(geom.eps2), mom, L.ptr(rm), L.ptr(rv), L.ptr(nb), L.ptr(stats2),
-               L.ptr(ab2), L.ptr(mv2), L.ptr(ws), L.stream())
+               L.ptr(ab2), L.ptr(mv2), L.ptr(dt.tile_class) if skip else None, L.ptr(order), L.ptr(pre), L.ptr(ws), L.stream())
     M = pillar_cell.numel()
     yrows = torch.empty(M, C2, dtype=cdt, device=dev)
     out = None
@@ -560,7 +570,7 @@
     if cdt == torch.bfloat16 and conv_impl == 'tiles':
         ep = hidden[0]._plan
         tile_conv = TileConv(gplan.decoder_tiles(ep, src_idx, Y, X), [hidden[i].stage_plan.map for i in src_idx],
-                             [Y // hidden[i].stage_plan.Y for i in src_idx])
+                             [Y // hidden[i].stage_plan.Y for i in src_idx], CT_SKIP)
     for i, src in enumerate(model_cfg.FEATURES_SOURCE):
         h = hidden[int(src[-1]) - 1]
         sp = h.stage_plan
diff --git a/gd-mae_amd/gdmae_hip/lib.py b/gd-mae_amd/gdmae_hip/lib.py
--- a/gd-mae_amd/gdmae_hip/lib.py
+++ b/gd-mae_amd/gdmae_hip/lib.py
@@ -76,6 +76,10 @@
     "gdmae_conv3x3_tiles_workspace_bytes": (_Z, [_I]),
     "gdmae_conv3x3_tiles_fwd": (_I, [_P, _P, _P, _P, _P, _I, _P, _P, _P, _I, _I, _I, _I, _P, _P, _P, _D, _D, _P, _P, _P, _P, _P, _P,
                                      _P, _P]),
+    "gdmae_decoder_tiles_classes": (_I, [_P, _P, _I, _I, _I, _I, _P, _P, _P, _P, _P, _P, _P]),
+    "gdmae_conv3x3_tiles_pack_pre": (_I, [_P, _I, _I, _P, _I, _P, _P, _P, _P, _P]),
+    "gdmae_conv3x3_tiles_fwd_skip": (_I, [_P, _P, _P, _P, _P, _I, _P, _P, _P, _I, _I, _I, _I, _P, _P, _P, _D, _D, _P, _P, _P, _P, _P, _P,
+                                          _P, _P, _P, _P, _P]),
     "gdmae_tiles_gather_rows": (_I, [_P, _P, _P, _P, _L, _I, _I, _I, _I, _P, _P]),
     "gdmae_tiles_gather_rows_affine_relu": (_I, [_P, _P, _P, _P, _L, _I, _I, _I, _P, _P, _P, _P, _P]),
     "gdmae_tiles_to_dense": (_I, [_P, _P, _P, _I, _I, _I, _I, _I, _P, _P]),
diff --git a/gd-mae_amd/gdmae_hip/plan.py b/gd-mae_amd/gdmae_hip/plan.py
--- a/gd-mae_amd/gdmae_hip/plan.py
+++ b/gd-mae_amd/gdmae_hip/plan.py
@@ -130,6 +130,8 @@
     tile_slot: torch.Tensor
     tile_list: torch.Tensor
     nbr: Optional[list] = None
+    tile_class: Optional[torch.Tensor] = None
+    tile_order: Optional[torch.Tensor] = None
 
 
 @dataclass
@@ -175,10 +177,11 @@
 
 def _decoder_tiles_launch(maps, ups, B, H, W, dev) -> dict:
     nt = B * ((H + 7) // 8) * ((W + 7) // 8)
-    r = dict(tile_slot=_empty(nt, I32, dev), tile_list=_empty(nt, I32, dev), n_act=_empty(1, I32, dev), B=B, H=H, W=W)
+    r = dict(tile_slot=_empty(nt, I32, dev), tile_list=_empty(nt, I32, dev), tile_class=_empty(nt, I32, dev),
+             tile_order=_empty(nt, I32, dev), n_act=_empty(1, I32, dev), B=B, H=H, W=W)
     ws = _empty(L.load().gdmae_decoder_tiles_workspace_bytes(B, H, W), torch.uint8, dev)
-    L.call("gdmae_decoder_tiles", L.host_ptrs(maps), L.host_i32(ups), len(maps), B, H, W, L.ptr(r["tile_slot"]),
-           L.ptr(r["tile_list"]), L.ptr(r["n_act"]), L.ptr(ws), L.stream())
+    L.call("gdmae_decoder_tiles_classes", L.host_ptrs(maps), L.host_i32(ups), len(maps), B, H, W, L.ptr(r["tile_slot"]),
+           L.ptr(r["tile_list"]), L.ptr(r["tile_class"]), L.ptr(r["tile_order"]), L.ptr(r["n_act"]), L.ptr(ws), L.stream())
     r["_ws"] = ws
     return r
 
@@ -194,7 +197,7 @@
     assert all(sp.Y * u == H and sp.X * u == W for sp, u in zip(st, ups))
     r = _decoder_tiles_launch([sp.map for sp in st], ups, B, H, W, st[0].map.device)
     n = int(r["n_act"].item())
-    ep.dec_tiles = DecoderTiles(sources, B, H, W, n, r["tile_slot"], r["tile_list"][:n])
+    ep.dec_tiles = DecoderTiles(sources, B, H, W, n, r["tile_slot"], r["tile_list"][:n], None, r["tile_class"][:n], r["tile_order"][:n])
     ep.dec_tiles.nbr = _site_rulebooks(ep.dec_tiles, st, ups)
     return ep.dec_tiles
 
@@ -338,7 +341,8 @@
     dt = None
     if dec is not None:
         n_act = int(allc[ns + 16 * ns])
-        dt = DecoderTiles(dec["sources"], dec["B"], dec["H"], dec["W"], n_act, dec["tile_slot"], dec["tile_list"][:n_act])
+        dt = DecoderTiles(dec["sources"], dec["B"], dec["H"], dec["W"], n_act, dec["tile_slot"], dec["tile_list"][:n_act], None,
+                          dec["tile_class"][:n_act], dec["tile_order"][:n_act])
     return EncoderPlan(e["mask"][:M] if e["masked"] else None, e["tok_pillar"][:stages[0].n_tok], stages, dt)
 
 
@@ -541,7 +545,7 @@
             nt = B * ((gy + 7) // 8) * ((gx + 7) // 8)
             nbrs = [V(f"dec.nbr{g}", i32, stages[int(si)].n_tok * geo[int(si)]["up_s"] ** 2, 9) for g, si in enumerate(self.dec_sources)]
             dt = DecoderTiles(tuple(int(i) for i in self.dec_sources), B, gy, gx, n_act, V("dec.tile_slot", i32, nt), V("dec.tile_list", i32, n_act),
-                              nbrs)
+                              nbrs, V("dec.tile_class", i32, n_act), V("dec.tile_order", i32, n_act))
         ep = EncoderPlan(V("mask", f32, M) if self.masked else None, V("tok_pillar", i32, stages[0].n_tok if not geo[0]["strided"] else n_vis),
                          stages, dt)
         if self.masked and A.has("vfe.row_tok"):
diff --git a/include/gdmae_hip.h b/include/gdmae_hip.h
--- a/include/gdmae_hip.h
+++ b/include/gdmae_hip.h
@@ -162,6 +162,16 @@
                             int H, int W, void* Yc, const float* gamma, const float* beta, double eps, double momentum,
                             float* running_mean, float* running_var, long long* num_batches, double* stats, float* ab,
                             float* mv, void* workspace, void* stream);
+int gdmae_decoder_tiles_classes(const int* const* maps, const int* strides, int k, int B, int H, int W, int* tile_slot, int* tile_list,
+                                int* tile_class, int* tile_order, int* n_act, void* workspace, void* stream);
+int gdmae_conv3x3_tiles_pack_pre(const float* conv_w, int C2, int Cin, const float* const* b, int k, void* Wp, void* bgz, void* ybg,
+                                 float* pre, void* stream);
+int gdmae_conv3x3_tiles_fwd_skip(const void* const* P, const int* const* maps, const float* const* a, const float* const* b,
+                                 const int* strides, int k, const void* Wp, const void* ybg, const int* tile_list, int n_act, int B,
+                                 int H, int W, void* Yc, const float* gamma, const float* beta, double eps, double momentum,
+                                 float* running_mean, float* running_var, long long* num_batches, double* stats, float* ab,
+                                 float* mv, const int* tile_class, const int* tile_order, const float* pre, void* workspace,
+                                 void* stream);
 int gdmae_tiles_gather_rows(const void* Yc, const int* tile_slot, const void* ybg, const int* cell, long long n, int H, int W,
                             int C, int elem_bytes, void* out, void* stream);
 int gdmae_tiles_gather_rows_affine_relu(const void* Yc, const int* tile_slot, const void* ybg, const int* cell, long long n, int H, int W,
```

Measured after the change: 1142, median of 6. 1.01x the previous value.
